# kluonj/HelFEM

Measured on AMD Instinct MI355X. Metric: scf_iteration_wall_time_fock_plus_geneig_nbf4230, lower is better.
Workload: dtype f64; 1 GPU; diatomic Z1=7 Z2=7 R=2.068 PBE, nelem=5 nnodes=15 nquad=75 lmmax=[20,20] (Nbf=4230, Nang=61, Nrad=70), XC grid 92x13, symmetry blocks [1380, 1470, 1380]: J+XC Fock build + eig_gsym_sub + density per step; parallelism=shard1, density=occupied orbitals of the core Hamiltonian

## Files before the change

### helfem_amd/__init__.py

```python
import ctypes
import os

import numpy as np

_HERE = os.path.dirname(os.path.abspath(__file__))
_LIB_PATH = os.environ.get("HELFEM_AMD_LIB") or os.path.join(_HERE, "lib", "libhelfem_amd.so")
_lib = None

c_double_p = ctypes.POINTER(ctypes.c_double)
c_int_p = ctypes.POINTER(ctypes.c_int)
c_i64_p = ctypes.POINTER(ctypes.c_int64)


class hfg_diatomic_desc(ctypes.Structure):
    _fields_ = [("Z1", ctypes.c_int), ("Z2", ctypes.c_int), ("Rhalf", ctypes.c_double), ("primbas", ctypes.c_int),
                ("nnodes", ctypes.c_int), ("nquad", ctypes.c_int), ("bval", c_double_p), ("nbval", ctypes.c_int),
                ("lval", c_int_p), ("mval", c_int_p), ("nang", ctypes.c_int), ("lpad", ctypes.c_int)]


class hfg_model_pot(ctypes.Structure):
    _fields_ = [("kind", ctypes.c_int), ("Z", ctypes.c_int), ("d", ctypes.c_double), ("H", ctypes.c_double)]


class hfg_atomic_desc(ctypes.Structure):
# ... 53 lines not shown
        L.hfg_last_error.restype = ctypes.c_char_p
        L.hfg_version.restype = ctypes.c_char_p
        L.hfg_gaunt_coefficient.restype = ctypes.c_double
        L.hfg_gaunt_coefficient.argtypes = [ctypes.c_int] * 6
        L.hfg_modified_gaunt_coefficient.restype = ctypes.c_double
        L.hfg_modified_gaunt_coefficient.argtypes = [ctypes.c_int] * 6
        L.hfg_theta_lm.restype = ctypes.c_double
        L.hfg_theta_lm.argtypes = [ctypes.c_int, ctypes.c_int, ctypes.c_double]
        L.hfg_legendre_PQ.restype = None
        L.hfg_legendre_PQ.argtypes = [ctypes.c_int, ctypes.c_int, ctypes.c_double, c_double_p, c_double_p]
        for nm in ("hfg_bessel_il", "hfg_bessel_kl"):
            getattr(L, nm).restype = ctypes.c_double
            getattr(L, nm).argtypes = [ctypes.c_double, ctypes.c_int]
        L.hfg_erfc_phi.restype = ctypes.c_double
        L.hfg_erfc_phi.argtypes = [ctypes.c_int, ctypes.c_double, ctypes.c_double]
        L.hfg_compute_rs_tei.argtypes = [ctypes.c_void_p, ctypes.c_int, ctypes.c_double]
        L.hfg_compute_rs_tei_dev.argtypes = [ctypes.c_void_p, ctypes.c_void_p, ctypes.c_int, ctypes.c_double]
        L.hfg_rs_special_dev.argtypes = [ctypes.c_void_p, ctypes.c_int, ctypes.c_int, c_double_p, c_double_p, ctypes.c_int64, c_double_p]
        L.hfg_set_erfc_binomial_mode.restype = None
        L.hfg_set_erfc_binomial_mode.argtypes = [ctypes.c_int]
        L.hfg_model_potential.argtypes = [ctypes.c_void_p, ctypes.c_void_p, ctypes.POINTER(hfg_model_pot),
                                          ctypes.POINTER(hfg_model_pot), c_double_p]
        L.hfg_chebyshev_rule.restype = None
        L.hfg_chebyshev_rule.argtypes = [ctypes.c_int, c_double_p, c_double_p]
        L.hfg_lobatto_nodes.restype = None
        L.hfg_lobatto_nodes.argtypes = [ctypes.c_int, c_double_p]
        L.hfg_radial_grid.argtypes = [ctypes.c_double, ctypes.c_int, ctypes.c_int, ctypes.c_double, c_double_p]
        L.hfg_basis_confinement.argtypes = [ctypes.c_void_p, ctypes.c_int, ctypes.c_int, ctypes.c_double, ctypes.c_double,
                                            ctypes.c_double, c_double_p]
        L.hfg_atomic_grid.argtypes = [ctypes.c_int, ctypes.c_double, ctypes.c_int, ctypes.c_double, ctypes.c_int, ctypes.c_double,
                                      ctypes.c_int, ctypes.c_int, ctypes.c_double, ctypes.c_int, ctypes.c_int, ctypes.c_int,
                                      ctypes.c_double, ctypes.c_int, ctypes.c_double, c_double_p, c_int_p]
        L.hfg_scf_options_check_ex.argtypes = [ctypes.POINTER(hfg_scf_options), ctypes.POINTER(hfg_scf_atomic_extras)]
        L.hfg_scf_run_ex.argtypes = [ctypes.c_void_p, ctypes.POINTER(hfg_scf_options), ctypes.POINTER(hfg_scf_atomic_extras),
                                     ctypes.POINTER(hfg_scf_result), c_double_p, c_double_p]
        L.hfg_ctx_create.argtypes = [ctypes.POINTER(ctypes.c_void_p), ctypes.c_int, ctypes.c_void_p]
        L.hfg_xc_fock.argtypes = [ctypes.c_void_p, ctypes.c_void_p, ctypes.c_int, ctypes.c_int, c_double_p, c_double_p,
                                  c_double_p, c_double_p, c_double_p, ctypes.c_double]
        L.hfg_xc_fock_pol.argtypes = [ctypes.c_void_p, ctypes.c_void_p, ctypes.c_int, ctypes.c_int, c_double_p, c_double_p,
                                      c_double_p, c_double_p, c_double_p, c_double_p, c_double_p, ctypes.c_double]
        L.hfg_xc_fock_dev.argtypes = [ctypes.c_void_p, ctypes.c_void_p, ctypes.c_int, ctypes.c_int, ctypes.c_void_p,
                                      ctypes.c_void_p, ctypes.c_void_p, ctypes.c_double]
        L.hfg_coulomb_batch.argtypes = [ctypes.c_void_p, ctypes.c_void_p, ctypes.c_int64, c_double_p, c_double_p]
        L.hfg_coulomb_energy_matrix.argtypes = [ctypes.c_void_p, ctypes.c_void_p, ctypes.c_int64, c_double_p, c_double_p]
        L.hfg_coulomb_batch_devptr.argtypes = [ctypes.c_void_p, ctypes.c_void_p, ctypes.c_int64, ctypes.c_void_p, ctypes.c_void_p]
        for name in ("hfg_exchange_batch", "hfg_rs_exchange_batch"):
            getattr(L, name).argtypes = [ctypes.c_void_p, ctypes.c_void_p, ctypes.c_int64, c_double_p, c_double_p]
        for name in ("hfg_exchange_batch_devptr", "hfg_rs_exchange_batch_devptr"):
            getattr(L, name).argtypes = [ctypes.c_void_p, ctypes.c_void_p, ctypes.c_int64, ctypes.c_void_p, ctypes.c_void_p]
        L.hfg_exchange_occ_batch_devptr.argtypes = [ctypes.c_void_p, ctypes.c_void_p, ctypes.c_int64, ctypes.c_void_p, ctypes.c_void_p,
                                                    c_i64_p, ctypes.c_int64, ctypes.c_void_p]
        L.hfg_exchange_batch_plan.argtypes = [ctypes.c_int64, c_int_p, ctypes.c_int, c_int_p, c_int_p]
        L.hfg_fock_compact_pol_size.restype = ctypes.c_int64
        L.hfg_fock_compact_pol_size.argtypes = [ctypes.c_void_p]
        L.hfg_fock_compact_pol_devptr.argtypes = [ctypes.c_void_p, ctypes.c_void_p, ctypes.c_int, ctypes.c_int, ctypes.c_void_p,
                                                  ctypes.c_void_p, ctypes.c_void_p, ctypes.c_void_p, ctypes.c_double]
        L.hfg_fock_finish_pol_devptr.argtypes = [ctypes.c_void_p] * 7
        L.hfg_eig_gsym_sub_pair_devptr.argtypes = [ctypes.c_void_p, ctypes.c_int64, ctypes.c_void_p, ctypes.c_void_p, ctypes.c_void_p,
                                                   ctypes.c_int, c_i64_p, c_i64_p] + [ctypes.c_void_p] * 4
        L.hfg_profile_get.argtypes = [ctypes.c_void_p, ctypes.c_char_p, c_double_p, c_i64_p]
        L.hfg_measure_kernel.argtypes = [ctypes.c_void_p, ctypes.c_char_p, c_double_p, c_i64_p]
        L.hfg_profile_names.argtypes = [ctypes.c_void_p, ctypes.c_char_p, ctypes.c_size_t]
        L.hfg_diis_create.argtypes = [ctypes.c_void_p, ctypes.c_int64, ctypes.c_int, ctypes.c_int, ctypes.c_double, ctypes.c_double,
                                      ctypes.c_int, ctypes.POINTER(ctypes.c_void_p)]
        L.hfg_diis_destroy.argtypes = [ctypes.c_void_p]
        L.hfg_diis_set_metric_devptr.argtypes = [ctypes.c_void_p, ctypes.c_void_p, ctypes.c_void_p, ctypes.c_int64]
        L.hfg_diis_set_blocks.argtypes = [ctypes.c_void_p, ctypes.c_int, c_i64_p, c_i64_p]
        L.hfg_diis_update_devptr.argtypes = [ctypes.c_void_p, ctypes.c_double, ctypes.c_void_p, ctypes.c_void_p, ctypes.c_void_p,
                                             ctypes.c_int64, ctypes.c_void_p, ctypes.c_void_p, ctypes.c_void_p, ctypes.c_int64,
                                             c_double_p]
        L.hfg_diis_solve_devptr.argtypes = [ctypes.c_void_p, ctypes.c_void_p, ctypes.c_void_p, c_int_p]
        L.hfg_diis_size.argtypes = [ctypes.c_void_p]
        L.hfg_diis_get.argtypes = [ctypes.c_void_p, ctypes.c_int, c_double_p, ctypes.c_int64]
        L.hfg_coulomb_dev.argtypes = [ctypes.c_void_p] * 4
        L.hfg_fock_compact_size.restype = ctypes.c_int64
        L.hfg_eig_block_buf_size.restype = ctypes.c_int64
        L.hfg_fock_compact_dev.argtypes = [ctypes.c_void_p, ctypes.c_void_p, ctypes.c_int, ctypes.c_int, ctypes.c_void_p,
                                           ctypes.c_void_p, ctypes.c_void_p, ctypes.c_double]
        for name in ("hfg_exchange_dev", "hfg_rs_exchange_dev", "hfg_mix_exchange_devptr"):
            getattr(L, name).argtypes = [ctypes.c_void_p] * 4
        for name in ("hfg_exchange_occ_dev", "hfg_mix_exchange_occ_devptr"):
            getattr(L, name).argtypes = [ctypes.c_void_p] * 4 + [ctypes.c_int64, ctypes.c_void_p]
        L.hfg_mix_exchange_occ_batch_devptr.argtypes = L.hfg_exchange_occ_batch_devptr.argtypes
        _lib = L
    return _lib


def _check(rc):
    if rc != 0:
        raise RuntimeError(lib().hfg_last_error().decode())


def _f(a):
    return np.asfortranarray(a, dtype=np.float64)


def _p(a):
    return a.ctypes.data_as(c_double_p)


def device_count():
    return int(lib().hfg_device_count())


class Context(object):

    def __init__(self, device=0, stream=None):
        h = ctypes.c_void_p()
        if stream is None:
            sp = None
        elif int(stream) == 0:
            sp = ctypes.c_void_p(-1)
        else:
            sp = ctypes.c_void_p(int(stream))
        _check(lib().hfg_ctx_create(ctypes.byref(h), int(device), sp))
        self.h = h
        self.device = device

    def close(self):
        if self.h:
            lib().hfg_ctx_destroy(self.h)
            self.h = None

    def __del__(self):
        try:
            self.close()
        except Exception:
            pass

    def synchronize(self):
        _check(lib().hfg_ctx_synchronize(self.h))

    def set_shard(self, rank, nranks):
        _check(lib().hfg_ctx_set_shard(self.h, int(rank), int(nranks)))

    def set_fock_blocks(self, basis, blockid_ptr):
        f = lib().hfg_ctx_set_fock_blocks
        f.argtypes = [ctypes.c_void_p, ctypes.c_void_p, ctypes.c_void_p]
        _check(f(self.h, basis.h, ctypes.c_void_p(blockid_ptr or 0)))

    def fix_sinvh(self, device_ptr):
        _check(lib().hfg_ctx_fix_sinvh(self.h, ctypes.c_void_p(device_ptr or 0)))

    FOCK_BAND_STATES = ("none", "declared", "refused")

    def declare_fock_band(self, basis, H0_ptr=None, blockid_ptr=None):
        f = lib().hfg_ctx_declare_fock_band
        f.argtypes = [ctypes.c_void_p, ctypes.c_void_p, ctypes.c_void_p, ctypes.c_void_p, c_int_p]
        st = ctypes.c_int()
        _check(f(self.h, basis.h, ctypes.c_void_p(H0_ptr or 0), ctypes.c_void_p(blockid_ptr or 0), ctypes.byref(st)))
        return self.FOCK_BAND_STATES[st.value]

    def fock_band_state(self):
        f = lib().hfg_ctx_fock_band_state
        f.argtypes = [ctypes.c_void_p, c_int_p]
        st = ctypes.c_int()
        _check(f(self.h, ctypes.byref(st)))
        return self.FOCK_BAND_STATES[st.value]

    def profile(self, on=True):
        _check(lib().hfg_profile_enable(self.h, 1 if on else 0))

    def profile_reset(self):
        _check(lib().hfg_profile_reset(self.h))

    def measure_kernel(self, name):
# ... 973 lines not shown
            return [("hfg_mix_exchange_occ_batch_devptr", "K")]
        return [("hfg_mix_exchange_occ_devptr" if have_C else "hfg_mix_exchange_devptr", "K")]
    plain, occ, screened = (("hfg_exchange_batch_devptr", "hfg_exchange_occ_batch_devptr", "hfg_rs_exchange_batch_devptr") if batch
                            else ("hfg_exchange_dev", "hfg_exchange_occ_dev", "hfg_rs_exchange_dev"))
    route = []
    if kfrac != 0.0:
        route.append((occ if have_C else plain, "K"))
    if kshort != 0.0:
        route.append((screened, "Krs"))
    return route


class DeviceSCFStep(object):

    def __init__(self, basis, x_func, c_func, ldft, mdft, nocc, symmetry=1, device=0, rank=0, nranks=1,
                 dens_thr=1e-12, kfrac=0.0, device_tei=False, fock_shard="auto", kshort=0.0, omega=0.0, rs_kind=None):
        self.nocc = int(nocc)
        self._setup(basis, x_func, c_func, ldft, mdft, symmetry, device, rank, nranks, dens_thr, kfrac, device_tei, fock_shard,
                    kshort, omega, rs_kind)
        f64 = dict(dtype=self.torch.float64, device=self.dev)
        L, N = lib(), self.N
        self.Fc = self.torch.zeros(int(L.hfg_fock_compact_size(basis.h)), **f64)
        self.scal = self.torch.zeros(3, **f64)
        self.F = self.torch.zeros(N * N, **f64)
        self.E = self.torch.zeros(N, **f64)
        self.C = self.torch.zeros(N * N, **f64)
        self.P = self.torch.zeros(N * N, **f64)
        nb = int(L.hfg_eig_block_buf_size(len(self.blocks), self.blk_ptr.ctypes.data_as(c_i64_p)))
        self.blockbuf = self.torch.zeros(nb, **f64)
        if self.anyK:
            self.K = self.torch.zeros(N * N, **f64)
            self.Pa = self.torch.zeros(N * N, **f64)

    def _setup(self, basis, x_func, c_func, ldft, mdft, symmetry, device, rank, nranks, dens_thr, kfrac, device_tei, fock_shard,
               kshort=0.0, omega=0.0, rs_kind=None):
        self.kshort, self.omega = float(kshort), float(omega)
        self.rs_kind = 0
        self.mix = False
        self.Krs = None
        if self.kshort != 0.0:
            if not isinstance(basis, AtomicTwoDBasis):
                raise RuntimeError("Range separated functionals are not supported.")
            self.rs_kind = xc_rs_kind(x_func) if rs_kind is None else int(rs_kind)
            if self.rs_kind not in (1, 2) or self.omega == 0.0:
                raise ValueError("kshort != 0 needs a screened kernel (rs_kind 1 Yukawa or 2 erfc, from the exchange functional "
                                 "when None) and its range omega != 0")
        import torch
        self.torch = torch
        self.basis = basis
        self.x_func, self.c_func, self.thr = int(x_func), int(c_func), float(dens_thr)
        self.dev = torch.device("cuda", device)
        torch.cuda.set_device(self.dev)
        self.ctx = Context(device, stream=torch.cuda.current_stream(self.dev).cuda_stream)
        self.ctx.set_shard(rank, nranks)
        self.rank, self.nranks = int(rank), int(nranks)
        self.fock_shard = os.environ.get("HELFEM_FOCK_SHARD", fock_shard)
        if device_tei:
            basis.compute_tei(float(kfrac) != 0.0 or self.kshort != 0.0, device=True, ctx=self.ctx)
        if self.kshort != 0.0:
            switches = {r["name"]: r["value"] for r in tuning_table()}
            on_device = bool(device_tei) or switches["HELFEM_RS_TEI"] == "dev"
            basis._compute_rs(self.rs_kind, self.omega, on_device, self.ctx)
        basis.upload(ldft, mdft, ctx=self.ctx)
        if self.kshort != 0.0:
            want = int(switches["HELFEM_EXL_MIX"])
            if want > 0 or (want < 0 and MIX_BY_DEFAULT[self.rs_kind]):
                self.mix = basis.mix_exchange_tables(float(kfrac), self.kshort, ctx=self.ctx)
        N = basis.Nbf()
        self.N = N
        self.blocks = basis.get_sym_idx(symmetry)
        self.blk_ptr, self.blk_idx = scf._blocks(self.blocks)
        blockid = np.zeros(N, dtype=np.int32)
        for ib, b in enumerate(self.blocks):
            blockid[b] = ib
        self.blockid = torch.from_numpy(blockid).to(self.dev)
        self.ctx.set_fock_blocks(basis, self.blockid.data_ptr())
        self.H0 = None
        self.Sinvh = None
        self.kfrac = float(kfrac)
        self.anyK = self.kfrac != 0.0 or self.kshort != 0.0
        self.kscale = self.kfrac if self.kshort == 0.0 else 1.0
        self.have_C = False
        self.have_density = False
        if self.kshort != 0.0 and not self.mix:
            self.Krs = torch.zeros(N * N, dtype=torch.float64, device=self.dev)

    def _ptr(self, t):
        return ctypes.c_void_p(t.data_ptr())

    def set_matrices(self, H0, Sinvh):
        t = self.torch
        self.H0 = t.from_numpy(np.asfortranarray(H0).ravel(order="F").copy()).to(self.dev)
        self.ctx.fix_sinvh(None)
        self.Sinvh = t.from_numpy(np.asfortranarray(Sinvh).ravel(order="F").copy()).to(self.dev)
        self.ctx.fix_sinvh(self.Sinvh.data_ptr())
        if not self.anyK and not self._applies_cuhf:
            self.ctx.declare_fock_band(self.basis, self.H0.data_ptr(), self.blockid.data_ptr())

    def set_density(self, P, C=None):
        self.P.copy_(self.torch.from_numpy(np.asfortranarray(P).ravel(order="F").copy()))
        self.have_density = True
        self.have_C = C is not None
        if C is not None:
            self.C[:self.N * self.nocc].copy_(self.torch.from_numpy(np.asfortranarray(C[:, :self.nocc]).ravel(order="F").copy()))

    def exchange(self):
        self.torch.mul(self.P, 0.5, out=self.Pa)
        self._build_K(self.Pa, self.C, ctypes.c_int64(self.nocc), self.K)

    def _build_K(self, P, C, nocc, K, batch=0):
        L = lib()
        head = (self.ctx.h, self.basis.h, batch) if batch else (self.ctx.h, self.basis.h)
        for name, dest in _exchange_route(self.mix, self.kfrac, self.kshort, self.have_C, bool(batch)):
            args = [self._ptr(P)]
            if "_occ_" in name:
                args += [self._ptr(C), nocc] if self.have_C else [None, None]
                if batch:
                    args.append(self.N)
            _check(getattr(L, name)(*head, *args, self._ptr(K if dest == "K" else self.Krs)))
        if self.kshort != 0.0 and not self.mix:
            if self.kfrac != 0.0:
                K.mul_(self.kfrac).add_(self.Krs, alpha=self.kshort)
            else:
                self.torch.mul(self.Krs, self.kshort, out=K)

    def fock_partial(self):
        _check(lib().hfg_fock_compact_dev(self.ctx.h, self.basis.h, self.x_func, self.c_func, self._ptr(self.P),
                                          self._ptr(self.Fc), self._ptr(self.scal), self.thr))

    def fock_finish(self):
        _check(lib().hfg_fock_finish_dev(self.ctx.h, self.basis.h, self._ptr(self.Fc), self._ptr(self.H0),
                                         self._ptr(self.blockid), self._ptr(self.F)))

    def _spins(self):
        return ((self.P, self.F, self.E, self.C, self.nocc),)

    def _blockbufs(self):
        return (self.blockbuf,)

    def _spin_K(self):
        return (self.K,)

    def eig_partial(self):
        for (_, F, _, _, _), buf in zip(self._spins(), self._blockbufs()):
            _check(lib().hfg_eig_blocks_dev(self.ctx.h, ctypes.c_int64(self.N), self._ptr(F), self._ptr(self.Sinvh),
                                            len(self.blocks), self.blk_ptr.ctypes.data_as(c_i64_p),
                                            self.blk_idx.ctypes.data_as(c_i64_p), self._ptr(buf)))

    def eig_finish(self):
        for (_, _, E, C, _), buf in zip(self._spins(), self._blockbufs()):
            _check(lib().hfg_eig_assemble_dev(self.ctx.h, ctypes.c_int64(self.N), len(self.blocks),
                                              self.blk_ptr.ctypes.data_as(c_i64_p), self.blk_idx.ctypes.data_as(c_i64_p),
                                              self._ptr(buf), self._ptr(E), self._ptr(C)))

    def eig_whole(self):
        _check(lib().hfg_eig_gsym_sub_dev(self.ctx.h, ctypes.c_int64(self.N), self._ptr(self.F), self._ptr(self.Sinvh),
                                          len(self.blocks), self.blk_ptr.ctypes.data_as(c_i64_p),
                                          self.blk_idx.ctypes.data_as(c_i64_p), self._ptr(self.E), self._ptr(self.C)))

    def density(self):
        for P, _, _, C, nocc in self._spins():
            if nocc == 0:
                P.zero_()
                continue
            _check(lib().hfg_form_density_dev(self.ctx.h, ctypes.c_int64(self.N), ctypes.c_int64(self.N), self._ptr(C),
                                              ctypes.c_int64(nocc), self._ptr(P)))
        self.have_density = True

    def step(self, allreduce=None, exchange_blocks=None):
        self._fock_stage(allreduce)
        self._constrain()
        self._eig_stage(allreduce, exchange_blocks)
        self.density()
        self.have_C = True

    def _whole_shard(self, fn):
        if self.nranks > 1:
            self.ctx.set_shard(0, 1)
        try:
            fn()
        finally:
            if self.nranks > 1:
                self.ctx.set_shard(self.rank, self.nranks)

    def _fock_stage(self, allreduce):
        shard_fock = self.nranks > 1 and self.fock_shard == "always"
        if shard_fock or self.nranks == 1:
            self.fock_partial()
            if allreduce is not None:
                allreduce(self.Fc)
                allreduce(self.scal)
        else:
            self._whole_shard(self.fock_partial)
        self.fock_finish()
        if self.anyK:
            self.exchange()
            if allreduce is not None:
                allreduce(self.K)
            self._add_exchange()

    def _add_exchange(self):
        for (_, F, _, _, _), K in zip(self._spins(), self._spin_K()):
            F.add_(K, alpha=self.kscale)

    def _eig_in_one_call(self, allreduce, exchange_blocks):
        return self.nranks == 1 and allreduce is None and exchange_blocks is None

    def _eig_stage(self, allreduce, exchange_blocks):
        if self._eig_in_one_call(allreduce, exchange_blocks):
            self.eig_whole()
            return
        self.eig_partial()
        for buf in self._blockbufs():
            if exchange_blocks is not None:
                exchange_blocks(buf, len(self.blocks))
            elif allreduce is not None:
                allreduce(buf)
        self.eig_finish()

    def _nn_buffer(self, name):
        buf = getattr(self, name, None)
        if buf is None:
            buf = self.torch.zeros(self.N * self.N, dtype=self.torch.float64, device=self.dev)
            setattr(self, name, buf)
        return buf

    def _coulomb_energy_matrix(self, P):
        J = self._nn_buffer("J")
        self._whole_shard(lambda: _check(lib().hfg_coulomb_dev(self.ctx.h, self.basis.h, self._ptr(P), self._ptr(J))))
        return J

    def _energy_terms(self):
        t = self.torch
        J = self._coulomb_energy_matrix(self.P)
        terms = [t.dot(self.P, self.H0), t.dot(self.P, J)]
        terms.append(t.dot(self.Pa, self.K) if self.anyK else t.zeros((), dtype=t.float64, device=self.dev))
        return terms

    def energy(self, Enucr=0.0):
        t = self.torch
        v = t.stack(self._energy_terms() + [self.scal[0]]).cpu().numpy()
        r = dict(E1=float(v[0]), Ecoul=0.5 * float(v[1]), Exx=self._exx_factor() * float(v[2]), Exc=float(v[3]), Enucr=float(Enucr))
        r["Etot"] = r["E1"] + r["Ecoul"] + r["Exx"] + r["Exc"] + r["Enucr"]
        return r

    def _exx_factor(self):
        return self.kscale

    def _nspin(self):
        return 1

    def _density_stage(self):
        self.density()
        self.P.mul_(2.0)
        self.have_C = True

    def _core_guess(self, allreduce, exchange_blocks):
        for _, F, _, _, _ in self._spins():
            F.copy_(self.H0)
        self._eig_stage(allreduce, exchange_blocks)
        self._density_stage()

    def _diis_update(self, diis, E):
        Pa = self.torch.mul(self.P, 0.5, out=self._nn_buffer("Pa"))
        if self.have_C:
            return diis.update(E, self.F, Pa, self.C, self.nocc)
        return diis.update(E, self.F, Pa)

    def _diis_solve(self, diis):
        diis.solve(self.F)

    _applies_cuhf = False

    def _constraint_begin(self, S):
        pass

    def _constrain(self):
        pass

    def run(self, S, maxit=50, convthr=1e-7, Enucr=0.0, allreduce=None, exchange_blocks=None, diis=None, callback=None,
            rohf=False, cuhf=False, readocc=None, maverage=False, dampfock=1.0):
        _refuse_out_of_scope(type(self).__name__, rohf and not self._applies_cuhf, cuhf and not self._applies_cuhf, readocc, maverage,
                             dampfock)
        if self.H0 is None:
            raise RuntimeError("run: set_matrices first")
        self._constraint_begin(S)
        t = self.torch
        if diis is None:
            diis = DeviceDIIS(self.ctx, self.N, self._nspin())
            dS = t.from_numpy(np.asfortranarray(S, dtype=np.float64).ravel(order="F").copy()).to(self.dev)
            diis.set_metric(dS, self.Sinvh)
            if len(self.blocks) > 1:
                diis.set_blocks(self.blocks)
        if not self.have_density:
            self._core_guess(allreduce, exchange_blocks)
        trace, Eold, res, converged, it = [], 0.0, None, False, 0
        for it in range(1, int(maxit) + 1):
            self._fock_stage(allreduce)
            res = self.energy(Enucr)
            self._constrain()
            maxerr = self._diis_update(diis, res["Etot"])
            dE = res["Etot"] - Eold
            Eold = res["Etot"]
            trace.append((res["Etot"], maxerr))
            if callback is not None:
                callback(it, res["Etot"], maxerr)
            if maxerr < convthr and abs(dE) < convthr:
                converged = True
                break
            self._diis_solve(diis)
            self._eig_stage(allreduce, exchange_blocks)
            self._density_stage()
        res = dict(res or {})
        res.update(iterations=it, converged=converged, trace=trace)
        return res

    def numpy(self, t, shape):
        return t.cpu().numpy().reshape(shape, order="F")


class DeviceUSCFStep(DeviceSCFStep):

    def __init__(self, basis, x_func, c_func, ldft, mdft, nocc, symmetry=1, device=0, rank=0, nranks=1,
                 dens_thr=1e-12, kfrac=0.0, device_tei=False, fock_shard="auto", kshort=0.0, omega=0.0, rs_kind=None):
        self.nela, self.nelb = int(nocc[0]), int(nocc[1])
        if self.nela < 1 or self.nelb < 0:
            raise ValueError("DeviceUSCFStep: nocc = (nela >= 1, nelb >= 0)")
        self._setup(basis, x_func, c_func, ldft, mdft, symmetry, device, rank, nranks, dens_thr, kfrac, device_tei, fock_shard,
                    kshort, omega, rs_kind)
        t, N, L = self.torch, self.N, lib()
        f64 = dict(dtype=t.float64, device=self.dev)
        self.nc = int(L.hfg_fock_compact_size(basis.h))
        self.Fc = t.zeros(int(L.hfg_fock_compact_pol_size(basis.h)), **f64)
        self.scal = t.zeros(3, **f64)
        for name in ("Pa", "Pb", "Fa", "Fb", "Ca", "Cb"):
            setattr(self, name, t.zeros(N * N, **f64))
        self.Ea, self.Eb = t.zeros(N, **f64), t.zeros(N, **f64)
        if self.nranks > 1:
            nb = int(L.hfg_eig_block_buf_size(len(self.blocks), self.blk_ptr.ctypes.data_as(c_i64_p)))
            self.blockbuf_a, self.blockbuf_b = t.zeros(nb, **f64), t.zeros(nb, **f64)
        self.kbatch = False
        if self.anyK:
            self.K = t.zeros(2 * N * N, **f64)
            self.Ka, self.Kb = self.K[:N * N], self.K[N * N:]
            self.kbatch = {r["name"]: r["value"] for r in tuning_table()}["HELFEM_USCF_KBATCH"] == "on"
            if self.kbatch:
                self.Pab, self.Cab = t.zeros(2 * N * N, **f64), t.zeros(2 * N * N, **f64)
                self._nocc = np.array([self.nela, self.nelb], dtype=np.int64)
                if self.Krs is not None:
                    self.Krs = t.zeros(2 * N * N, **f64)

    def _spins(self):
        return ((self.Pa, self.Fa, self.Ea, self.Ca, self.nela), (self.Pb, self.Fb, self.Eb, self.Cb, self.nelb))

    def _blockbufs(self):
        return (self.blockbuf_a, self.blockbuf_b)

    def _spin_K(self):
        return (self.Ka, self.Kb)

    def set_density(self, Pa, Pb, Ca=None, Cb=None):
        as_dev = lambda M: self.torch.from_numpy(np.asfortranarray(M).ravel(order="F").copy())
        self.Pa.copy_(as_dev(Pa))
        self.Pb.copy_(as_dev(Pb))
        self.have_density = True
        self.have_C = Ca is not None and (Cb is not None or self.nelb == 0)
        if self.have_C:
            self.Ca[:self.N * self.nela].copy_(as_dev(Ca[:, :self.nela]))
            if self.nelb:
                self.Cb[:self.N * self.nelb].copy_(as_dev(Cb[:, :self.nelb]))

    def exchange(self):
        if self.kbatch:
            N2 = self.N * self.N
            self.Pab[:N2].copy_(self.Pa)
            self.Pab[N2:].copy_(self.Pb)
            if self.have_C:
                self.Cab[:N2].copy_(self.Ca)
                self.Cab[N2:].copy_(self.Cb)
            self._build_K(self.Pab, self.Cab, self._nocc.ctypes.data_as(c_i64_p), self.K, batch=2)
            return
        for (P, _, _, C, nocc), K in zip(self._spins(), self._spin_K()):
            if nocc == 0:
                K.zero_()
            else:
                self._build_K(P, C, ctypes.c_int64(nocc), K)

    def fock_partial(self):
        _check(lib().hfg_fock_compact_pol_devptr(self.ctx.h, self.basis.h, self.x_func, self.c_func, self._ptr(self.Pa),
                                                 self._ptr(self.Pb), self._ptr(self.Fc), self._ptr(self.scal), self.thr))

    def fock_finish(self):
        _check(lib().hfg_fock_finish_pol_devptr(self.ctx.h, self.basis.h, self._ptr(self.Fc), self._ptr(self.H0),
                                                self._ptr(self.blockid), self._ptr(self.Fa), self._ptr(self.Fb)))

    def eig_pair(self):
        _check(lib().hfg_eig_gsym_sub_pair_devptr(self.ctx.h, ctypes.c_int64(self.N), self._ptr(self.Fa), self._ptr(self.Fb),
                                                  self._ptr(self.Sinvh), len(self.blocks), self.blk_ptr.ctypes.data_as(c_i64_p),
                                                  self.blk_idx.ctypes.data_as(c_i64_p), self._ptr(self.Ea), self._ptr(self.Ca),
                                                  self._ptr(self.Eb), self._ptr(self.Cb)))

    eig_whole = eig_pair

    def _eig_in_one_call(self, allreduce, exchange_blocks):
        return self.nranks == 1

    def _energy_terms(self):
        t = self.torch
        Pt = t.add(self.Pa, self.Pb, out=self._nn_buffer("Pt"))
        J = self._coulomb_energy_matrix(Pt)
        terms = [t.dot(Pt, self.H0), t.dot(Pt, J)]
        terms.append(t.dot(self.Pa, self.Ka) + t.dot(self.Pb, self.Kb) if self.anyK
                     else t.zeros((), dtype=t.float64, device=self.dev))
        return terms

    def _exx_factor(self):
        return 0.5 * self.kscale

    def _nspin(self):
        return 2

    def _density_stage(self):
        self.density()
        self.have_C = True

    def _diis_update(self, diis, E):
        if self.have_C:
            return diis.update(E, self.Fa, self.Pa, self.Ca, self.nela, self.Fb, self.Pb, self.Cb if self.nelb else None, self.nelb)
        return diis.update(E, self.Fa, self.Pa, Fb=self.Fb, Pb=self.Pb)

    def _diis_solve(self, diis):
        diis.solve(self.Fa, self.Fb)


class DeviceROHFStep(DeviceUSCFStep):

    _applies_cuhf = True

    def __init__(self, *args, **kw):
        super(DeviceROHFStep, self).__init__(*args, **kw)
        self.S = None

    def set_overlap(self, S):
        S = np.asfortranarray(S, dtype=np.float64)
        if S.shape != (self.N, self.N):
            raise ValueError("DeviceROHFStep.set_overlap: S is N x N")
        self.S = self.torch.from_numpy(S.ravel(order="F").copy()).to(self.dev)

    def _constraint_begin(self, S):
        if S is not None:
            self.set_overlap(S)

    def _constrain(self):
        if self.S is None:
            raise RuntimeError("DeviceROHFStep: set_overlap first")
        if not self.have_C:
            raise RuntimeError("DeviceROHFStep: the constraint needs the orbitals the densities were formed from "
                               "(set_density with Ca and Cb, or start from the core guess)")
        self.ctx.cuhf_update(self.S, self.Ca, self.nela, self.Cb, self.nelb, self.Fa, self.Fb)
```

### helfem_amd/csrc/hip/capi.cpp

```cpp
#include "internal.h"
#include "../host/checkpoint.h"
#include "../host/diis.h"
#include "../host/dftfuncs.h"
#include "../host/exchange_batch_plan.h"
#include "../host/eig_band_plan.h"
#include "../host/fock_need.h"
#include <cstring>
#include <memory>
#include <mutex>

namespace hfg {
static thread_local std::string g_err;
void set_error(const std::string &msg) { g_err = msg; }

}

using namespace hfg;

#define HFG_TRY try {
#define HFG_CATCH                       \
  }                                     \
  catch (const std::logic_error &e) {   \
    hfg::set_error(e.what());           \
    return 1;                           \
// ... 807 lines not shown
int hfg_exchange_batch_plan(int64_t nP, const int *ranks, int max_members, int *chunk_of, int *nchunks) {
  HFG_TRY
  if (nP < 0) throw std::logic_error("hfg_exchange_batch_plan: negative number of densities\n");
  if (nP > 0 && (!ranks || !chunk_of)) throw std::logic_error("hfg_exchange_batch_plan: null pointer\n");
  if (max_members < 0) throw std::logic_error("hfg_exchange_batch_plan: negative chunk size\n");
  const int n = helfem::exchange_batch_plan((long)nP, ranks, max_members ? max_members : helfem::tuning_live().exchange_batch_chunk, chunk_of);
  if (nchunks) *nchunks = n;
  HFG_CATCH
}
int hfg_xc_fock_dev(hfg_ctx *ctx, hfg_basis *b, int x_func, int c_func, const double *dP, double *dH, double *dScal,
                    double thr) {
  HFG_TRY xc_fock_dev(ctx, b, x_func, c_func, dP, dH, dScal, thr);
  HFG_CATCH
}
int hfg_xc_fock_pol_dev(hfg_ctx *ctx, hfg_basis *b, int x_func, int c_func, const double *dPa, const double *dPb,
                        double *dHa, double *dHb, double *dScal, double thr) {
  HFG_TRY xc_fock_pol_dev(ctx, b, x_func, c_func, dPa, dPb, dHa, dHb, dScal, thr);
  HFG_CATCH
}
int hfg_eig_gsym_sub_dev(hfg_ctx *ctx, int64_t N, const double *dF, const double *dS, int nblk, const int64_t *blk_ptr,
                         const int64_t *blk_idx, double *dE, double *dC) {
  HFG_TRY eig_gsym_sub_dev(ctx, (int)N, dF, dS, nblk, blk_ptr, blk_idx, dE, dC);
  HFG_CATCH
}
int64_t hfg_eig_block_buf_size(int nblk, const int64_t *blk_ptr) { return (int64_t)eig_block_buf_size(nblk, blk_ptr); }
int hfg_eig_blocks_dev(hfg_ctx *ctx, int64_t N, const double *dF, const double *dS, int nblk, const int64_t *blk_ptr,
                       const int64_t *blk_idx, double *dBlockBuf) {
  HFG_TRY eig_blocks_dev(ctx, (int)N, dF, dS, nblk, blk_ptr, blk_idx, dBlockBuf);
  HFG_CATCH
}
int hfg_eig_assemble_dev(hfg_ctx *ctx, int64_t N, int nblk, const int64_t *blk_ptr, const int64_t *blk_idx,
                         const double *dBlockBuf, double *dE, double *dC) {
  HFG_TRY eig_assemble_dev(ctx, (int)N, nblk, blk_ptr, blk_idx, dBlockBuf, dE, dC);
  HFG_CATCH
}
int hfg_form_density_dev(hfg_ctx *ctx, int64_t N, int64_t ncols, const double *dC, int64_t nocc, double *dP) {
  HFG_TRY form_density_dev(ctx, (int)N, (int)ncols, dC, (int)nocc, dP);
  HFG_CATCH
}
int hfg_gemm_dev(hfg_ctx *ctx, int tA, int tB, int64_t m, int64_t n, int64_t k, const double *dA, int64_t lda,
                 const double *dB, int64_t ldb, double *dC, int64_t ldc) {
  HFG_TRY gemm_dev(ctx, tA != 0, tB != 0, (int)m, (int)n, (int)k, 1.0, dA, (int)lda, dB, (int)ldb, 0.0, dC, (int)ldc);
  HFG_CATCH
}

int64_t hfg_fock_compact_size(hfg_basis *b) { return (int64_t)fock_compact_size(b); }
int hfg_fock_compact_dev(hfg_ctx *ctx, hfg_basis *b, int x_func, int c_func, const double *dP, double *dFc,
                         double *dScal, double thr) {
  HFG_TRY fock_compact_dev(ctx, b, x_func, c_func, dP, dFc, dScal, thr);
  HFG_CATCH
}
int hfg_fock_finish_dev(hfg_ctx *ctx, hfg_basis *b, const double *dFc, const double *dH0, const int *dBlockId,
                        double *dF) {
  HFG_TRY fock_finish_dev(ctx, b, dFc, dH0, dBlockId, dF);
  HFG_CATCH
}
int64_t hfg_fock_compact_pol_size(hfg_basis *b) { return 2 * (int64_t)fock_compact_size(b); }
int hfg_fock_compact_pol_devptr(hfg_ctx *ctx, hfg_basis *b, int x_func, int c_func, const double *dPa, const double *dPb,
                                double *dFc, double *dScal, double thr) {
  HFG_TRY
  if (!ctx || !b) throw std::logic_error("hfg_fock_compact_pol_devptr: null context or basis\n");
  if (!dPa || !dPb || !dFc || !dScal) throw std::logic_error("hfg_fock_compact_pol_devptr: null device pointer\n");
  fock_compact_pol_dev(ctx, b, x_func, c_func, dPa, dPb, dFc, dScal, thr);
  HFG_CATCH
}
int hfg_fock_finish_pol_devptr(hfg_ctx *ctx, hfg_basis *b, const double *dFc, const double *dH0, const int *dBlockId,
                               double *dFa, double *dFb) {
  HFG_TRY
  if (!ctx || !b) throw std::logic_error("hfg_fock_finish_pol_devptr: null context or basis\n");
  if (!dFc || !dFa || !dFb) throw std::logic_error("hfg_fock_finish_pol_devptr: null device pointer\n");
  fock_finish_pol_dev(ctx, b, dFc, dH0, dBlockId, dFa, dFb);
  HFG_CATCH
}
int hfg_eig_gsym_sub_pair_devptr(hfg_ctx *ctx, int64_t N, const double *dFa, const double *dFb, const double *dSinvh, int nblk,
                                 const int64_t *blk_ptr, const int64_t *blk_idx, double *dEa, double *dCa, double *dEb,
                                 double *dCb) {
  HFG_TRY
  if (!ctx) throw std::logic_error("hfg_eig_gsym_sub_pair_devptr: null context\n");
  if (!dFa || !dFb || !dSinvh || !blk_ptr || !blk_idx || !dEa || !dCa || !dEb || !dCb)
    throw std::logic_error("hfg_eig_gsym_sub_pair_devptr: null pointer\n");
  eig_gsym_sub_pair_dev(ctx, (int)N, dFa, dFb, dSinvh, nblk, blk_ptr, blk_idx, dEa, dCa, dEb, dCb);
  HFG_CATCH
}
int hfg_ctx_set_fock_blocks(hfg_ctx *ctx, hfg_basis *b, const int *blockid_dev) {
  HFG_TRY
  if (!ctx || !b) throw std::logic_error("hfg_ctx_set_fock_blocks: null context or basis");
  set_fock_blocks(ctx, b, blockid_dev);
  HFG_CATCH
}
int hfg_fock_need_pairs(int nshell, const int *nfunc, const int *blockid, int *need) {
  HFG_TRY
  if (nshell < 0 || !nfunc || !blockid || !need) throw std::logic_error("hfg_fock_need_pairs: invalid arguments");
  helfem::fock_need_pairs(nshell, nfunc, blockid, need);
  HFG_CATCH
}

namespace {
struct FullShard {
  hfg_ctx *c;
  int r, n;
  explicit FullShard(hfg_ctx *ctx) : c(ctx), r(ctx->shard_rank), n(ctx->shard_n) {
    c->shard_rank = 0;
    c->shard_n = 1;
  }
  ~FullShard() {
    c->shard_rank = r;
    c->shard_n = n;
  }
};
}
int hfg_coulomb(hfg_ctx *ctx, hfg_basis *b, const double *P, double *J) {
  HFG_TRY
  FullShard full(ctx);
  size_t N = b->Nbf();
  Stage st(ctx);
  double *dP = st.up(P, N * N), *dJ = st.alloc(N * N);
  coulomb_dev(ctx, b, dP, dJ);
  st.down(J, dJ, N * N);
  st.sync();
  HFG_CATCH
}
int hfg_coulomb_batch(hfg_ctx *ctx, hfg_basis *b, int64_t nP, const double *P, double *J) {
  HFG_TRY
  if (!coulomb_batch_args("hfg_coulomb_batch", ctx, b, nP, P, J)) return 0;
  FullShard full(ctx);
  size_t n = b->Nbf() * b->Nbf() * (size_t)nP;
  Stage st(ctx);
  double *dP = st.up(P, n), *dJ = st.alloc(n);
  coulomb_batch_dev(ctx, b, nP, dP, dJ);
  st.down(J, dJ, n);
  st.sync();
  HFG_CATCH
}
int hfg_coulomb_energy_matrix(hfg_ctx *ctx, hfg_basis *b, int64_t nP, const double *P, double *W) {
  HFG_TRY
  if (!coulomb_batch_args("hfg_coulomb_energy_matrix", ctx, b, nP, P, W)) return 0;
  FullShard full(ctx);
  Stage st(ctx);
  double *dP = st.up(P, b->Nbf() * b->Nbf() * (size_t)nP), *dW = st.alloc((size_t)nP * nP);
  coulomb_energy_matrix_dev(ctx, b, nP, dP, dW);
  st.down(W, dW, (size_t)nP * nP);
  st.sync();
  HFG_CATCH
}
int hfg_exchange(hfg_ctx *ctx, hfg_basis *b, const double *P, double *K) {
  HFG_TRY
  FullShard full(ctx);
  size_t N = b->Nbf();
  Stage st(ctx);
  double *dP = st.up(P, N * N), *dK = st.alloc(N * N);
  exchange_dev(ctx, b, dP, dK);
  st.down(K, dK, N * N);
  st.sync();
  HFG_CATCH
}
int hfg_rs_exchange(hfg_ctx *ctx, hfg_basis *b, const double *P, double *K) {
  HFG_TRY
  FullShard full(ctx);
  size_t N = b->Nbf();
  Stage st(ctx);
  double *dP = st.up(P, N * N), *dK = st.alloc(N * N);
  exchange_dev(ctx, b, dP, dK, ExTables::screened);
  st.down(K, dK, N * N);
  st.sync();
  HFG_CATCH
}
// ... 366 lines not shown
```

### helfem_amd/csrc/hip/common.h

```cpp
#pragma once
#include <hip/hip_runtime.h>
#include <cstdint>
#include <cstring>
#include <map>
#include <stdexcept>
#include <string>
#include <vector>

#include "../../../include/helfem_gpu.h"
#include "../host/atomic_basis.h"
#include "../host/diatomic_basis.h"
#include "../host/tuning.h"
#include "workspace_owner.h"

namespace hfg {
using helfem::TrdMode, helfem::tuning;

void set_error(const std::string &msg);

#define HFG_HIP_CHECK(expr)                                                                          \
  do {                                                                                               \
    hipError_t _e = (expr);                                                                          \
    if (_e != hipSuccess)                                                                            \
      throw std::runtime_error(std::string("HIP error: ") + hipGetErrorString(_e) + " in " + #expr + \
                               " (" + __FILE__ + ":" + std::to_string(__LINE__) + ")");              \
  } while (0)

template <typename T>
struct DevBuf {
  T *p = nullptr;
  size_t n = 0;
  DevBuf() {}
  DevBuf(const DevBuf &) = delete;
  DevBuf &operator=(const DevBuf &) = delete;
  ~DevBuf() { release(); }
  void release() {
    if (p) (void)hipFree(p);
    p = nullptr;
    n = 0;
  }
  void resize(size_t count) {
    if (count <= n) return;
    release();
    HFG_HIP_CHECK(hipMalloc((void **)&p, count * sizeof(T)));
    n = count;
  }
  void upload(const std::vector<T> &h, hipStream_t s) {
    resize(h.size() ? h.size() : 1);
    if (h.size()) HFG_HIP_CHECK(hipMemcpyAsync(p, h.data(), h.size() * sizeof(T), hipMemcpyHostToDevice, s));
  }
};

template <typename T>
bool upload_cached(DevBuf<T> &buf, std::vector<T> &cache, const std::vector<T> &h, hipStream_t s) {
  if (buf.p && cache.size() == h.size() && buf.n >= h.size() &&
      (h.empty() || memcmp((const void *)cache.data(), (const void *)h.data(), h.size() * sizeof(T)) == 0))
    return false;
  HFG_HIP_CHECK(hipStreamSynchronize(s));
  cache = h;
  buf.upload(cache, s);
  return true;
}

struct ProfEntry {
  double ms = 0.0;
  int64_t launches = 0;
  std::vector<std::pair<hipEvent_t, hipEvent_t> > pending;
};

}

struct hfg_dev_tables;

struct hfg_ctx {
  int device = 0;
  hipStream_t stream = nullptr;
  bool own_stream = false;
  hipStream_t side_stream = nullptr;
  hipEvent_t side_ev[2] = {nullptr, nullptr};
  hipStream_t side();
  bool avoid_side = false;
  void drop_side();
  int shard_rank = 0, shard_n = 1;
  const double *fixed_sinvh = nullptr;
  unsigned long fixed_gen = 0;
  void fix_sinvh(const double *p) {
    fixed_sinvh = p;
    fixed_gen++;
    band_node.clear();
    band_state = 0;
  }
  std::vector<int> band_node;
  int band_pm = 0, band_E = 0;
  int band_state = 0;
  hfg::DevBuf<int> fock_need, fock_gneed;
  const hfg_dev_tables *fock_need_tables = nullptr;
  int fock_need_A = 0, fock_need_G = 0;
  bool profiling = false;
  std::map<std::string, hfg::ProfEntry> prof;
  std::vector<hipEvent_t> event_pool;
  hfg::DevBuf<double> ws[8];
  double *pinned = nullptr;
  size_t pinned_bytes = 0;
  hfg::WorkspaceOwner<hfg::WS_CTX_SLOTS> work;

  void *pinned_buf(size_t bytes);
  hipEvent_t get_event();
  void prof_begin(const char *name);
  void prof_end(const char *name);
  void prof_collect();
};

struct hfg_basis {
  int kind = 0;
  helfem::diatomic::TwoDBasis b;
  helfem::atomic::TwoDBasis ab;
  hfg_dev_tables *dev = nullptr;
  hfg_dev_tables *dev_rs = nullptr;
  hfg_dev_tables *dev_mix = nullptr;
  double mix_alpha = 0.0, mix_beta = 0.0, mix_omega = 0.0;
  int mix_kind = 0;
  int dev_device = -1;
  hfg::DevBuf<double> dev_tei;
  bool tei_on_device = false;
  hfg::DevBuf<double> dev_rs_tei, dev_rs_disj;
  bool rs_on_device = false;

  size_t Nbf() const { return kind ? ab.Nbf() : b.Nbf(); }
  size_t Ndummy() const { return kind ? ab.Nbf() : b.Ndummy(); }
  size_t Nrad() const { return kind ? ab.Nrad() : b.Nrad(); }
  size_t Nang() const { return kind ? ab.Nang() : b.Nang(); }
  size_t Nel() const { return kind ? ab.Nel() : b.Nel(); }
  size_t max_Nprim() const { return kind ? ab.max_Nprim() : b.max_Nprim(); }
  bool have_tei() const { return tei_on_device || (kind ? ab.have_tei : b.have_tei); }
};

namespace hfg {
struct GemmTask {
  const double *A;
  const double *B;
  double *C;
  int M, N, K, lda, ldb, ldc;
  int tA = 0, tB = 0;
  double alpha = 1.0, beta = 0.0;
  int sym = 0;
  int over = 0;
  const int *amap = nullptr, *cmap = nullptr;
  const int64_t *rmap = nullptr;
  const int *kstart = nullptr;
  int nk = 0;
  int kpad = 0;
};
static_assert(sizeof(GemmTask) == 120, "GemmTask is compared bytewise: keep it free of padding");

struct ProfScope {
  hfg_ctx *c;
  const char *n;
  ProfScope(hfg_ctx *ctx, const char *name) : c(ctx), n(name) {
    if (c->profiling) c->prof_begin(n);
  }
  ~ProfScope() {
    if (c->profiling) c->prof_end(n);
  }
};
}
```

### helfem_amd/csrc/hip/eig.hip

```cpp
#include "internal.h"
#include "wave.h"
#include "../host/eigsel_count.h"
#include "../host/eig_band_plan.h"
#include <cstdlib>
#include <cstring>
#include <functional>

namespace hfg {

constexpr int MAXB = 8;
struct EigBatch {
  int nblk;
  int n[MAXB];
  double *A[MAXB];
  double *d[MAXB];
  double *e[MAXB];
  double *tau[MAXB];
  double *v[MAXB];
  double *pp[MAXB];
  double *dots[MAXB];
  double *Z[MAXB];
  int nz[MAXB];
  double *rot[MAXB];
  int *sweeps[MAXB];
// ... 512 lines not shown
  __shared__ double sT[BT_KB][BT_KB + 1];
  __shared__ double sG[BT_KB][BT_KB + 1];
  __shared__ double sg[BT_KB];
  const int blk = blockIdx.y, p = blockIdx.x;
  const int n = b.n[blk];
  const int j0 = p * BT_KB;
  if (j0 > n - 3) return;
  const int kb = min(BT_KB, n - 2 - j0);
  double *Tp = T[blk] + (size_t)p * BT_KB * BT_KB;
  const int t = threadIdx.x;
  for (int c0 = 0; c0 < BT_KB; c0 += 16) {
    double g[16];
#pragma unroll
    for (int u = 0; u < 16; u++) g[u] = 0.0;
#pragma unroll
    for (int sl = 0; sl < BT_GS; sl++) {
      const double *src = G[blk] + ((size_t)sl * P + p) * BT_KB * BT_KB + (size_t)c0 * BT_KB + t;
#pragma unroll
      for (int u = 0; u < 16; u++) g[u] += src[(size_t)u * BT_KB];
    }
#pragma unroll
    for (int u = 0; u < 16; u++) {
      sG[c0 + u][t] = g[u];
      sT[t][c0 + u] = 0.0;
    }
  }
  __shared__ double stau[BT_KB];
  stau[t] = (t < kb) ? b.tau[blk][j0 + t] : 0.0;
  __syncthreads();
  for (int i = 0; i < kb; i++) {
    const double ti = stau[i];
    sg[t] = (t < i) ? sG[i][t] : 0.0;
    __syncthreads();
    if (t < i) {
      double acc0 = 0.0, acc1 = 0.0, acc2 = 0.0, acc3 = 0.0;
#pragma unroll
      for (int k = 0; k < BT_KB; k += 4) {
        acc0 += sT[t][k] * sg[k];
        acc1 += sT[t][k + 1] * sg[k + 1];
        acc2 += sT[t][k + 2] * sg[k + 2];
        acc3 += sT[t][k + 3] * sg[k + 3];
      }
      sT[t][i] = -ti * ((acc0 + acc1) + (acc2 + acc3));
    }
    if (t == i) sT[i][i] = ti;
    __syncthreads();
  }
  for (int c = 0; c < BT_KB; c++) Tp[(size_t)c * BT_KB + t] = sT[t][c];
}

struct EigWork : Workspace {
  GemmHow full_how;
  std::vector<int64_t> asm_rows;
  DevBuf<long long> asm_rows_dev;
  bool folded = false;
  DevBuf<double> Y[MAXB];
  DevBuf<GemmTask> btslabR, btupdR;
  std::vector<GemmTask> h_btslabR, h_btupdR;
  DevBuf<double> A[MAXB], d[MAXB], e[MAXB], tau[MAXB], v[MAXB], pp[MAXB], dots[MAXB], Z[MAXB], rot[MAXB];
  DevBuf<double> Zs[MAXB], Ws[MAXB];
  DevBuf<int> selrank;
  DevBuf<int> sweeps[MAXB];
  DevBuf<int> ibuf1, ibuf2;
  DevBuf<GemmTask> gtasks, bttasks, btslab, btgram, btcpl, btupd;
  std::vector<GemmTask> h_gtasks, h_bttasks, h_btslab, h_btgram, h_btcpl, h_btupd;
  std::vector<double *> h_btptr;
  DevBuf<double> Vx[MAXB], G[MAXB], T[MAXB], VT[MAXB], Wb[MAXB], Wp[MAXB], Cc[MAXB];
  DevBuf<double *> btptr;
  bool used_dc = true;
  DevBuf<double> idx;
  const double *sup_S = nullptr;
  unsigned long sup_gen = 0;
  int sup_N = 0;
  std::vector<int64_t> sup_ptr, sup_idx;
  DevBuf<double> Xc;
  std::vector<char> xc_have;
  std::vector<int64_t> band_rows, band_pos;
  std::vector<int> band_ks, band_koff, band_toff;
  bool band_any = false;
  DevBuf<long long> band_rows_dev, band_pos_dev;
  DevBuf<int> band_ks_dev, band_iota_dev;
  DevBuf<GemmTask> fxtasks;
  std::vector<GemmTask> h_fxtasks;
  int *h_status = nullptr;
  hipEvent_t status_ev = nullptr;
  ~EigWork() {
    if (h_status) (void)hipHostFree(h_status);
    if (status_ev) (void)hipEventDestroy(status_ev);
  }
};
static EigWork &work_for(hfg_ctx *ctx) { return ctx->work.get<EigWork>(WS_EIG); }

struct CopySlices {
  const double *src[16];
  double *dst[16];
  int n[16];
};
__global__ void k_copy_slices(CopySlices c) {
  const int q = blockIdx.y;
  for (int i = blockIdx.x * blockDim.x + threadIdx.x; i < c.n[q]; i += gridDim.x * blockDim.x) c.dst[q][i] = c.src[q][i];
}
static void copy_slices(hipStream_t s, const std::vector<const double *> &src, const std::vector<double *> &dst, const std::vector<int> &n) {
  for (size_t q0 = 0; q0 < src.size(); q0 += 16) {
    CopySlices c{};
    const int m = (int)std::min<size_t>(16, src.size() - q0);
    int nmax = 0;
    for (int q = 0; q < m; q++) {
      c.src[q] = src[q0 + q];
      c.dst[q] = dst[q0 + q];
      c.n[q] = n[q0 + q];
      nmax = std::max(nmax, n[q0 + q]);
    }
    if (nmax > 0) hipLaunchKernelGGL(k_copy_slices, dim3((nmax + 255) / 256, m), dim3(256), 0, s, c);
  }
}

struct TrPtrs {
  const double *src[MAXB];
  double *dst[MAXB];
  int n[MAXB];
};
__global__ __launch_bounds__(256) void k_transpose_batch(TrPtrs t) {
  __shared__ double tile[64][65];
  const int blk = blockIdx.z, n = t.n[blk];
  const int bi = blockIdx.x * 64, bj = blockIdx.y * 64;
  if (bi >= n || bj >= n) return;
  const int tx = threadIdx.x & 63, ty = threadIdx.x >> 6;
  for (int c = ty; c < 64; c += 4) {
    const int gm = bi + tx, gn = bj + c;
    tile[c][tx] = (gm < n && gn < n) ? t.src[blk][(size_t)gn * n + gm] : 0.0;
  }
  __syncthreads();
  for (int c = ty; c < 64; c += 4) {
    const int gm = bj + tx, gn = bi + c;
    if (gm < n && gn < n) t.dst[blk][(size_t)gn * n + gm] = tile[tx][c];
  }
}

static void bt_wy_setup(hfg_ctx *ctx, EigWork &w, const EigBatch &b, int nblk, const int *ns, int nmax, bool fold = false) {
  hipStream_t s = ctx->stream;
  const int P = (nmax - 3) / BT_KB + 1;
  const int NP = (P + 1) / 2;
  constexpr int BT_S = 6;
  std::vector<double *> ptrs(6 * (size_t)nblk);
  for (int k = 0; k < nblk; k++) {
    const int n = ns[k];
    w.Vx[k].resize((size_t)n * n);
    w.G[k].resize((size_t)BT_GS * P * BT_KB * BT_KB);
    w.T[k].resize((size_t)P * BT_KB * BT_KB);
    w.VT[k].resize((size_t)n * P * BT_KB);
    w.Wb[k].resize((size_t)BT_PW * n);
    w.Wp[k].resize((size_t)BT_S * BT_PW * n);
    w.Cc[k].resize((size_t)BT_GS * NP * BT_KB * BT_KB);
    ptrs[k] = w.Vx[k].p;
    ptrs[nblk + k] = w.G[k].p;
    ptrs[2 * nblk + k] = w.T[k].p;
    ptrs[3 * nblk + k] = w.Wp[k].p;
    ptrs[4 * nblk + k] = w.Wb[k].p;
    ptrs[5 * nblk + k] = w.Cc[k].p;
  }
  upload_cached(w.btptr, w.h_btptr, ptrs, s);
  GemmTask none;
  none.A = none.B = nullptr;
  none.C = nullptr;
  none.M = none.N = none.K = 0;
  none.lda = none.ldb = none.ldc = 1;
// ... 359 lines not shown
      if (shb > 64 * 1024)
        HFG_HIP_CHECK(
            hipFuncSetAttribute((const void *)k_backtransform_lds, hipFuncAttributeMaxDynamicSharedMemorySize, (int)shb));
      hipLaunchKernelGGL(k_backtransform_lds, grid, dim3(256), shb, s, bz);
    }
    }
  }
  HFG_HIP_CHECK(hipGetLastError());
}

static void check_status(hfg_ctx *ctx, EigWork &w, int nblk) {
  if (w.used_dc) {
    if (dc_status(ctx) != 0) throw std::logic_error("Eigendecomposition failed!\n");
    trdp_check_status(ctx);
    return;
  }
  for (int i = 0; i < nblk; i++) {
    int st[2];
    HFG_HIP_CHECK(hipMemcpyAsync(st, w.sweeps[i].p, 2 * sizeof(int), hipMemcpyDeviceToHost, ctx->stream));
    HFG_HIP_CHECK(hipStreamSynchronize(ctx->stream));
    if (st[1] != 0) throw std::logic_error("Eigendecomposition failed!\n");
  }
}

void eig_sym_dev(hfg_ctx *ctx, int n, const double *dA, double *dE, double *dC) {
  EigWork &w = work_for(ctx);
  w.A[0].resize((size_t)n * n + 2);
  HFG_HIP_CHECK(hipMemcpyAsync(w.A[0].p, dA, sizeof(double) * n * n, hipMemcpyDeviceToDevice, ctx->stream));
  eig_sym_batch(ctx, w, 1, &n);
  DevBuf<int> &rank = w.ibuf1;
  rank.resize(n + 8);
  launch_rank(ctx, w.d[0].p, n, rank.p);
  hipLaunchKernelGGL(k_scatter_cols, dim3((n + 255) / 256, n), dim3(256), 0, ctx->stream, w.Z[0].p, n, n,
                     (const int64_t *)nullptr, rank.p, 0, w.d[0].p, n, dC, dE);
  check_status(ctx, w, 1);
}

void eig_sym_sel_dev(hfg_ctx *ctx, int n, const double *dA, int nev, double *dE, double *dC) {
  if (nev < 1) throw std::logic_error("eig_sym_sel: nev must be at least 1\n");
  if (n < 1) throw std::logic_error("eig_sym_sel: empty matrix\n");
  nev = std::min(nev, n);
  EigWork &w = work_for(ctx);
  w.A[0].resize((size_t)n * n + 2);
  HFG_HIP_CHECK(hipMemcpyAsync(w.A[0].p, dA, sizeof(double) * n * n, hipMemcpyDeviceToDevice, ctx->stream));
  eig_sym_batch(ctx, w, 1, &n, nullptr, &nev);
  HFG_HIP_CHECK(hipMemcpyAsync(dC, w.Zs[0].p, sizeof(double) * (size_t)n * nev, hipMemcpyDeviceToDevice, ctx->stream));
  HFG_HIP_CHECK(hipMemcpyAsync(dE, w.Ws[0].p, sizeof(double) * nev, hipMemcpyDeviceToDevice, ctx->stream));
  check_status(ctx, w, 1);
}

void eig_gsym_dev(hfg_ctx *ctx, int N, int n, const double *dF, const double *dS, double *dE, double *dC) {
  EigWork &w = work_for(ctx);
  w.A[0].resize((size_t)n * n + 2);
  DevBuf<double> &T1 = ctx->ws[0];
  DevBuf<double> &Ctmp = ctx->ws[1];
  T1.resize((size_t)N * n);
  Ctmp.resize((size_t)N * n);
  {
    ProfScope ps(ctx, "eig_reduce");
    gemm_dev(ctx, false, false, N, n, N, 1.0, dF, N, dS, N, 0.0, T1.p, N);
    gemm_dev(ctx, true, false, n, n, N, 1.0, dS, N, T1.p, N, 0.0, w.A[0].p, n);
  }
  eig_sym_batch(ctx, w, 1, &n);
  {
    ProfScope ps(ctx, "eig_backtransform");
    gemm_dev(ctx, false, false, N, n, n, 1.0, dS, N, w.Z[0].p, n, 0.0, Ctmp.p, N);
  }
  DevBuf<int> &rank = w.ibuf1;
  rank.resize(n + 8);
  launch_rank(ctx, w.d[0].p, n, rank.p);
  hipLaunchKernelGGL(k_scatter_cols, dim3((N + 255) / 256, n), dim3(256), 0, ctx->stream, Ctmp.p, N, n,
                     (const int64_t *)nullptr, rank.p, 0, w.d[0].p, N, dC, dE);
  check_status(ctx, w, 1);
}

size_t eig_block_buf_size(int nblk, const int64_t *blk_ptr) {
  size_t nmax = 0;
  for (int ib = 0; ib < nblk; ib++) nmax = std::max<size_t>(nmax, blk_ptr[ib + 1] - blk_ptr[ib]);
  return (size_t)nblk * (nmax * nmax + nmax);
}

static void eig_blocks_multi_dev(hfg_ctx *ctx, int N, int nF, const double *const *dFs, const double *dS, int nblk, const int64_t *blk_ptr,
                                 const int64_t *blk_idx, double *const *dBlockBufs, int nev = 0, double *const *dEs = nullptr,
                                 double *const *dCs = nullptr);
static int eig_num_cus(hfg_ctx *ctx) {
  static const int ncu = [&] {
    hipDeviceProp_t prop;
    return (hipGetDeviceProperties(&prop, ctx->device) == hipSuccess && prop.multiProcessorCount > 0) ? prop.multiProcessorCount : 256;
  }();
  return ncu;
}
void eig_blocks_dev(hfg_ctx *ctx, int N, const double *dF, const double *dS, int nblk, const int64_t *blk_ptr,
                    const int64_t *blk_idx, double *dBlockBuf) {
  eig_blocks_multi_dev(ctx, N, 1, &dF, dS, nblk, blk_ptr, blk_idx, &dBlockBuf);
}
static void eig_blocks_multi_dev(hfg_ctx *ctx, int N, int nF, const double *const *dFs, const double *dS, int nblk, const int64_t *blk_ptr,
                                 const int64_t *blk_idx, double *const *dBlockBufs, int nev, double *const *dEs, double *const *dCs) {
  EigWork &w = work_for(ctx);
  hipStream_t s = ctx->stream;
  const bool direct = dEs != nullptr;
  if (direct && (ctx->shard_n != 1 || nF * nblk > MAXB)) throw std::logic_error("eig_blocks_multi_dev: direct path needs one rank and one batch\n");
  if (blk_ptr[nblk] != N) throw std::logic_error("Symmetry mismatch in eig_gsym_sub\n");
  DevBuf<double> &idxbuf = w.idx;
  idxbuf.resize(2 * (size_t)N + 16);
  int64_t *drows = (int64_t *)idxbuf.p;
  int64_t *dcols = drows + N;
  for (int ib = 0; ib < nblk; ib++)
    if (blk_ptr[ib + 1] == blk_ptr[ib]) throw std::logic_error("eig_gsym_sub: empty symmetry block\n");
  const bool want_band = ctx->fixed_sinvh && ctx->fixed_sinvh == dS && ctx->band_state == 1 && ctx->band_node.size() == (size_t)N &&
                         helfem::tuning_live().eig_band;
  const bool cached = ctx->fixed_sinvh && ctx->fixed_sinvh == dS && w.sup_S == dS && w.sup_gen == ctx->fixed_gen &&
                      w.sup_N == N && want_band == !w.band_rows.empty() &&
                      w.sup_ptr.size() == (size_t)nblk + 1 && std::equal(w.sup_ptr.begin(), w.sup_ptr.end(), blk_ptr) &&
                      w.sup_idx.size() == (size_t)N && std::equal(w.sup_idx.begin(), w.sup_idx.end(), blk_idx);
  if (!cached) {
    w.sup_S = nullptr;
    w.xc_have.clear();
    HFG_HIP_CHECK(hipStreamSynchronize(s));
    w.band_rows.clear();
    w.band_pos.clear();
    w.band_ks.clear();
    w.band_koff.assign(1, 0);
    w.band_toff.assign(1, 0);
    w.band_any = false;
    if (want_band) {
      w.band_rows.resize(N);
      w.band_pos.resize(N);
      std::vector<int> nd, ks, toff;
      int64_t nbig = 0;
      for (int ib = 0; ib < nblk; ib++) {
        const int64_t o = blk_ptr[ib], n = blk_ptr[ib + 1] - o;
        nbig = std::max(nbig, n);
        nd.resize(n);
        for (int64_t i = 0; i < n; i++) {
          if (blk_idx[o + i] < 0 || blk_idx[o + i] >= N) throw std::logic_error("eig_gsym_sub: block index out of range\n");
          nd[i] = ctx->band_node[blk_idx[o + i]];
        }
        helfem::eig_band_order(n, nd.data(), w.band_pos.data() + o);
        for (int64_t i = 0; i < n; i++) w.band_rows[o + i] = blk_idx[o + w.band_pos[o + i]];
        if (helfem::eig_band_plan(n, nd.data(), w.band_pos.data() + o, ctx->band_pm, ctx->band_E, ks, toff)) w.band_any = true;
        for (size_t t = 0; t + 1 < toff.size(); t++) w.band_koff.push_back((int)w.band_ks.size() + toff[t + 1]);
        w.band_ks.insert(w.band_ks.end(), ks.begin(), ks.end());
        w.band_toff.push_back((int)w.band_koff.size() - 1);
      }
      std::vector<int> iota(nbig);
      for (int64_t i = 0; i < nbig; i++) iota[i] = (int)i;
      w.band_rows_dev.resize(N);
      w.band_pos_dev.resize(N);
      w.band_ks_dev.resize(w.band_ks.size() + 1);
      w.band_iota_dev.resize(nbig);
      HFG_HIP_CHECK(hipMemcpyAsync(w.band_rows_dev.p, w.band_rows.data(), sizeof(int64_t) * N, hipMemcpyHostToDevice, s));
      HFG_HIP_CHECK(hipMemcpyAsync(w.band_pos_dev.p, w.band_pos.data(), sizeof(int64_t) * N, hipMemcpyHostToDevice, s));
      HFG_HIP_CHECK(hipMemcpyAsync(w.band_ks_dev.p, w.band_ks.data(), sizeof(int) * w.band_ks.size(), hipMemcpyHostToDevice, s));
      HFG_HIP_CHECK(hipMemcpyAsync(w.band_iota_dev.p, iota.data(), sizeof(int) * nbig, hipMemcpyHostToDevice, s));
      HFG_HIP_CHECK(hipStreamSynchronize(s));
    }
    HFG_HIP_CHECK(hipMemcpyAsync(drows, blk_idx, sizeof(int64_t) * N, hipMemcpyHostToDevice, s));
    DevBuf<int> &flag = w.ibuf2;
    flag.resize((size_t)N * nblk + 8);
    for (int ib = 0; ib < nblk; ib++) {
      int n = (int)(blk_ptr[ib + 1] - blk_ptr[ib]);
      hipLaunchKernelGGL(k_col_support, dim3(N), dim3(256), 0, s, dS, N, drows + blk_ptr[ib], n, flag.p + (size_t)ib * N);
    }
    std::vector<int> hflag((size_t)N * nblk);
    HFG_HIP_CHECK(hipMemcpyAsync(hflag.data(), flag.p, sizeof(int) * hflag.size(), hipMemcpyDeviceToHost, s));
    HFG_HIP_CHECK(hipStreamSynchronize(s));
    std::vector<int64_t> allcols;
    for (int ib = 0; ib < nblk; ib++) {
      int cnt = 0;
      for (int c = 0; c < N; c++)
        if (hflag[(size_t)ib * N + c]) {
          allcols.push_back(c);
          cnt++;
        }
      if (cnt != (int)(blk_ptr[ib + 1] - blk_ptr[ib]))
        throw std::logic_error("eig_gsym_sub: Sinvh is not block structured (columns with support != block size)\n");
    }
    HFG_HIP_CHECK(hipMemcpyAsync(dcols, allcols.data(), sizeof(int64_t) * N, hipMemcpyHostToDevice, s));
    HFG_HIP_CHECK(hipStreamSynchronize(s));
    if (ctx->fixed_sinvh == dS) {
      w.sup_S = dS;
      w.sup_gen = ctx->fixed_gen;
      w.sup_N = N;
      w.sup_ptr.assign(blk_ptr, blk_ptr + nblk + 1);
      w.sup_idx.assign(blk_idx, blk_idx + N);
    }
  }

  size_t nmax = 0;
  for (int ib = 0; ib < nblk; ib++) nmax = std::max<size_t>(nmax, blk_ptr[ib + 1] - blk_ptr[ib]);
  const size_t slot = nmax * nmax + nmax;
  if (!direct && ctx->shard_n > 1)
    for (int f = 0; f < nF; f++) HFG_HIP_CHECK(hipMemsetAsync(dBlockBufs[f], 0, sizeof(double) * slot * nblk, s));
  const bool keep_x = w.sup_S == dS && w.sup_S != nullptr;
  std::vector<size_t> xoff(nblk + 1, 0);
  for (int ib = 0; ib < nblk; ib++) xoff[ib + 1] = xoff[ib] + (size_t)(blk_ptr[ib + 1] - blk_ptr[ib]) * (size_t)(blk_ptr[ib + 1] - blk_ptr[ib]);
  if (keep_x) {
    if (w.xc_have.size() != (size_t)nblk || w.Xc.n < xoff[nblk]) {
      w.Xc.resize(xoff[nblk]);
      w.xc_have.assign(nblk, 0);
    }
  }
  std::vector<int64_t> koff(nblk + 1, 0);
  for (int ib = 0; ib < nblk; ib++) {
    const int64_t n = blk_ptr[ib + 1] - blk_ptr[ib];
    koff[ib + 1] = koff[ib] + (nev > 0 ? std::min<int64_t>(nev, n) : n);
  }
  const int K = (int)koff[nblk];
  DevBuf<int> &rank = w.ibuf1;
  DevBuf<double> &Etmp = ctx->ws[3];
  if (direct) {
    rank.resize((size_t)nF * (N + 8));
    Etmp.resize((size_t)nF * N);
  }

  std::vector<int> mine;
  for (int f = 0; f < nF; f++)
    for (int ib = 0; ib < nblk; ib++)
      if (ib % ctx->shard_n == ctx->shard_rank) mine.push_back(f * nblk + ib);
  DevBuf<double> &Fb = ctx->ws[5];
  DevBuf<double> &T1 = ctx->ws[0];
  DevBuf<double> &Xall = ctx->ws[4];
  Fb.resize(nmax * nmax * MAXB);
  T1.resize(nmax * nmax * MAXB);
  Xall.resize(nmax * nmax * MAXB);
  for (size_t c0 = 0; c0 < mine.size(); c0 += MAXB) {
    int nb = (int)std::min<size_t>(MAXB, mine.size() - c0);
    std::vector<int> ns(nb), nevs(nb);
    std::vector<GemmTask> gt(4 * (size_t)nb);
    const double *Xptr[MAXB];
    int nm = 0;
    for (int k = 0; k < nb; k++) {
      const int ib = mine[c0 + k] % nblk;
      double *dBlockBuf = direct ? nullptr : dBlockBufs[mine[c0 + k] / nblk];
      int n = (int)(blk_ptr[ib + 1] - blk_ptr[ib]);
      ns[k] = n;
      nevs[k] = nev > 0 ? std::min(nev, n) : n;
      nm = std::max(nm, n);
      w.A[k].resize((size_t)n * n + 2);
      if (nev > 0) w.Zs[k].resize((size_t)n * nevs[k]);
      else w.Z[k].resize((size_t)n * n);
      w.Y[k].resize((size_t)n * n);
      double *Xb = keep_x ? w.Xc.p + xoff[ib] : Xall.p + (size_t)k * nmax * nmax;
      double *Fk = Fb.p + (size_t)k * nmax * nmax, *Tk = T1.p + (size_t)k * nmax * nmax;
      Xptr[k] = Xb;
      GemmTask g;
      g.M = g.N = g.K = n;
      g.lda = g.ldb = g.ldc = n;
      g.A = Fk;
      g.B = Xb;
      g.C = Tk;
      gt[k] = g;
      g.A = Xb;
      g.tA = 1;
      g.B = Tk;
      g.C = w.A[k].p;
      g.sym = 1;
      gt[nb + k] = g;
      g.sym = 0;
      g.tA = 0;
      g.A = Xb;
      g.B = nev > 0 ? w.Zs[k].p : w.Z[k].p;
      g.N = nevs[k];
      if (direct) {
        const int f = mine[c0 + k] / nblk;
        g.C = dCs[f];
        g.ldc = N;
        g.rmap = drows + blk_ptr[ib];
        g.cmap = rank.p + (size_t)f * (N + 8) + koff[ib];
      } else
        g.C = dBlockBuf + (size_t)ib * slot;
      gt[2 * nb + k] = g;
      g.A = w.Y[k].p;
      g.tA = 1;
      gt[3 * nb + k] = g;
    }
    upload_cached(w.gtasks, w.h_gtasks, gt, s);
    std::vector<GemmTask> fx;
    if (w.band_any && !w.band_rows.empty()) {
      for (int k = 0; k < nb; k++) {
        const int ib = mine[c0 + k] % nblk;
        const int n = ns[k], nt = w.band_toff[ib + 1] - w.band_toff[ib];
        for (int t = 0; t < nt; t++) {
          const int i0 = t * helfem::EIG_BAND_TILE, q = w.band_toff[ib] + t;
          GemmTask g = gt[k];
          g.A = gt[k].A + i0;
          g.M = std::min(helfem::EIG_BAND_TILE, n - i0);
          g.rmap = (const int64_t *)w.band_pos_dev.p + blk_ptr[ib] + i0;
          g.cmap = w.band_iota_dev.p;
          g.kstart = w.band_ks_dev.p + w.band_koff[q];
          g.nk = w.band_koff[q + 1] - w.band_koff[q];
          fx.push_back(g);
        }
      }
      std::stable_sort(fx.begin(), fx.end(), [](const GemmTask &a, const GemmTask &b) { return a.nk > b.nk; });
      upload_cached(w.fxtasks, w.h_fxtasks, fx, s);
    }
    {
      ProfScope ps(ctx, "eig_reduce");
      const int force_split = tuning().gemm_splitk;
      long full_tiles = 0, low_tiles = 0;
      for (int k = 0; k < nb; k++) {
        const long t1 = (ns[k] + 127) / 128;
        full_tiles += t1 * t1;
        low_tiles += t1 * (t1 + 1) / 2;
      }
      const bool band_fx = !fx.empty() && force_split < 0 && !gemm_prefers_128(ctx, full_tiles) && !tuning().mfma_4x4x4;
      for (int k = 0; k < nb; k++) {
        const int ib = mine[c0 + k] % nblk;
        const double *dF = dFs[mine[c0 + k] / nblk];
        int n = ns[k];
        double *Fk = Fb.p + (size_t)k * nmax * nmax;
        if (!(keep_x && w.xc_have[ib]))
          hipLaunchKernelGGL(k_gather_block, dim3((n + 255) / 256, n), dim3(256), 0, s, dF, dS, N, drows + blk_ptr[ib],
                             dcols + blk_ptr[ib], n, Fk, const_cast<double *>(Xptr[k]));
        else if (!band_fx)
          hipLaunchKernelGGL(k_gather_f, dim3((n + 255) / 256, n), dim3(256), 0, s, dF, N, drows + blk_ptr[ib], n, Fk);
        if (band_fx)
          hipLaunchKernelGGL(k_gather_f2, dim3((n + 255) / 256, n), dim3(256), 0, s, dF, N, (const int64_t *)w.band_rows_dev.p + blk_ptr[ib],
                             drows + blk_ptr[ib], n, Fk);
        if (keep_x) w.xc_have[ib] = 1;
      }
      const int slots = 2 * eig_num_cus(ctx);
      const bool split_full = force_split >= 0 ? force_split != 0 : (full_tiles < slots && nm >= 256);
      const bool split_low = force_split >= 0 ? force_split != 0 : (low_tiles < slots && nm >= 256);
      ProfScope pp3(ctx, "eig_products");
      const bool tile64 = force_split < 0 && !gemm_prefers_128(ctx, full_tiles);
      GemmHow full, low;
      if (tile64) full.tile = low.tile = GemmTile::T64;
      else {
        if (split_full) full.tile = GemmTile::T128, full.split2 = true;
        else if (tuning().gemm_rect) full.tile = GemmTile::T128x64;
        if (split_low) low.tile = GemmTile::T128, low.split2 = true;
      }
      w.full_how = full;
      if (full.split2)
        for (int k = 0; k < nb; k++) HFG_HIP_CHECK(hipMemsetAsync(T1.p + (size_t)k * nmax * nmax, 0, sizeof(double) * (size_t)ns[k] * ns[k], s));
      if (band_fx) {
        GemmHow how;
        how.tile = GemmTile::T64;
        how.scatter = how.klist = true;
        gemm_tasklist_dev(ctx, w.fxtasks.p, (int)fx.size(), helfem::EIG_BAND_TILE, nm, how);
      } else
        gemm_tasklist_dev(ctx, w.gtasks.p, nb, nm, nm, full);
      if (low.split2)
        for (int k = 0; k < nb; k++) HFG_HIP_CHECK(hipMemsetAsync(w.A[k].p, 0, sizeof(double) * (size_t)ns[k] * ns[k], s));
      gemm_tasklist_dev(ctx, w.gtasks.p + nb, nb, nm, nm, low);
      gemm_mirror_lower_dev(ctx, w.gtasks.p + nb, nb, nm);
    }
    std::function<void()> after_solve;
    if (direct)
      after_solve = [&] {
        if (w.used_dc) {
          if (!w.h_status) HFG_HIP_CHECK(hipHostMalloc((void **)&w.h_status, sizeof(int), hipHostMallocDefault));
          if (!w.status_ev) HFG_HIP_CHECK(hipEventCreateWithFlags(&w.status_ev, hipEventDisableTiming));
          HFG_HIP_CHECK(hipMemcpyAsync(w.h_status, dc_status_word(ctx), sizeof(int), hipMemcpyDeviceToHost, s));
          HFG_HIP_CHECK(hipEventRecord(w.status_ev, s));
        }
        ProfScope ps(ctx, "scatter");
        std::vector<const double *> csrc;
        std::vector<double *> cdst;
        std::vector<int> cn;
        for (int k = 0; k < nb; k++) {
          const int ib = mine[c0 + k] % nblk, f = mine[c0 + k] / nblk;
          csrc.push_back(nev > 0 ? w.Ws[k].p : w.d[k].p);
          cdst.push_back(Etmp.p + (size_t)f * N + koff[ib]);
          cn.push_back(nevs[k]);
        }
        copy_slices(s, csrc, cdst, cn);
        for (int f = 0; f < nF; f++) {
          int *rk = rank.p + (size_t)f * (N + 8);
          launch_rank(ctx, Etmp.p + (size_t)f * N, K, rk);
          hipLaunchKernelGGL(k_place_values, dim3((K + 255) / 256), dim3(256), 0, s, Etmp.p + (size_t)f * N, K, rk, dEs[f]);
          HFG_HIP_CHECK(hipMemsetAsync(dCs[f], 0, sizeof(double) * (size_t)N * K, s));
        }
      };
    eig_sym_batch(ctx, w, nb, ns.data(), Xptr, nev > 0 ? nevs.data() : nullptr, after_solve);
    {
      ProfScope ps(ctx, "eig_backtransform");
      if (!direct) {
        std::vector<const double *> csrc;
        std::vector<double *> cdst;
        std::vector<int> cn;
        for (int k = 0; k < nb; k++) {
          const int ib = mine[c0 + k] % nblk;
          double *slotp = dBlockBufs[mine[c0 + k] / nblk] + (size_t)ib * slot;
          csrc.push_back(nev > 0 ? w.Ws[k].p : w.d[k].p);
          cdst.push_back(slotp + nmax * nmax);
          cn.push_back(nevs[k]);
          if (nev <= 0 && w.full_how.split2 && ctx->shard_n == 1)
            HFG_HIP_CHECK(hipMemsetAsync(slotp, 0, sizeof(double) * (size_t)ns[k] * ns[k], s));
        }
        copy_slices(s, csrc, cdst, cn);
      }
      {
        ProfScope pp3(ctx, "eig_products");
        const GemmTask *last = w.gtasks.p + (w.folded ? 3 : 2) * (size_t)nb;
        GemmHow how = nev > 0 ? GemmHow{GemmTile::T64} : w.full_how;
        how.scatter = direct;
        gemm_tasklist_dev(ctx, last, nb, nm, nev > 0 ? *std::max_element(nevs.begin(), nevs.end()) : nm, how);
      }
    }
    if (direct && w.used_dc) {
      HFG_HIP_CHECK(hipEventSynchronize(w.status_ev));
      if (*w.h_status != 0) throw std::logic_error("Eigendecomposition failed!\n");
      trdp_check_status(ctx);
    } else
    check_status(ctx, w, nb);
  }
  HFG_HIP_CHECK(hipGetLastError());
}

static void eig_assemble_sel_dev(hfg_ctx *ctx, int N, int nblk, const int64_t *blk_ptr, const int64_t *blk_idx, const double *dBlockBuf,
                                 double *dE, double *dC, int nev);
void eig_assemble_dev(hfg_ctx *ctx, int N, int nblk, const int64_t *blk_ptr, const int64_t *blk_idx,
                      const double *dBlockBuf, double *dE, double *dC) {
  eig_assemble_sel_dev(ctx, N, nblk, blk_ptr, blk_idx, dBlockBuf, dE, dC, 0);
}
int64_t eig_sel_count(int nblk, const int64_t *blk_ptr, int64_t nev) { return helfem::eig_sel_count(nblk, blk_ptr, nev); }
static void eig_assemble_sel_dev(hfg_ctx *ctx, int N, int nblk, const int64_t *blk_ptr, const int64_t *blk_idx, const double *dBlockBuf,
                                 double *dE, double *dC, int nev) {
  EigWork &w = work_for(ctx);
  hipStream_t s = ctx->stream;
  ProfScope ps(ctx, "scatter");
  if (w.asm_rows.size() != (size_t)N || !std::equal(w.asm_rows.begin(), w.asm_rows.end(), blk_idx)) {
    w.asm_rows.assign(blk_idx, blk_idx + N);
    w.asm_rows_dev.resize((size_t)N + 2);
    HFG_HIP_CHECK(hipMemcpyAsync(w.asm_rows_dev.p, w.asm_rows.data(), sizeof(int64_t) * N, hipMemcpyHostToDevice, s));
  }
  int64_t *drows = (int64_t *)w.asm_rows_dev.p;
  size_t nmax = 0;
  for (int ib = 0; ib < nblk; ib++) nmax = std::max<size_t>(nmax, blk_ptr[ib + 1] - blk_ptr[ib]);
  const size_t slot = nmax * nmax + nmax;
  DevBuf<double> &Etmp = ctx->ws[3];
  Etmp.resize(N);
  std::vector<int64_t> koff(nblk + 1, 0);
  for (int ib = 0; ib < nblk; ib++) {
    const int64_t n = blk_ptr[ib + 1] - blk_ptr[ib];
    koff[ib + 1] = koff[ib] + (nev > 0 ? std::min<int64_t>(nev, n) : n);
  }
  const int K = (int)koff[nblk];
  {
    std::vector<const double *> csrc;
    std::vector<double *> cdst;
    std::vector<int> cn;
    for (int ib = 0; ib < nblk; ib++) {
      csrc.push_back(dBlockBuf + (size_t)ib * slot + nmax * nmax);
      cdst.push_back(Etmp.p + koff[ib]);
      cn.push_back((int)(koff[ib + 1] - koff[ib]));
    }
    copy_slices(s, csrc, cdst, cn);
  }
  DevBuf<int> &rank = w.ibuf1;
  rank.resize(N + 8);
  HFG_HIP_CHECK(hipMemsetAsync(dC, 0, sizeof(double) * (size_t)N * K, s));
  launch_rank(ctx, Etmp.p, K, rank.p);
  for (int ib = 0; ib < nblk; ib++) {
    int n = (int)(blk_ptr[ib + 1] - blk_ptr[ib]), nc = (int)(koff[ib + 1] - koff[ib]);
    hipLaunchKernelGGL(k_scatter_cols, dim3((n + 255) / 256, nc), dim3(256), 0, s, dBlockBuf + (size_t)ib * slot, n, nc,
                       drows + blk_ptr[ib], rank.p, (int)koff[ib], Etmp.p + koff[ib], N, dC, dE);
  }
  HFG_HIP_CHECK(hipGetLastError());
}

static void eig_gsym_sub_multi_dev(hfg_ctx *ctx, int N, int nF, const double *const *dFs, const double *dS, int nblk, const int64_t *blk_ptr,
                                   const int64_t *blk_idx, int nev, double *const *dEs, double *const *dCs) {
  int save_rank = ctx->shard_rank, save_n = ctx->shard_n;
  ctx->shard_rank = 0;
  ctx->shard_n = 1;
  try {
    if (helfem::tuning_live().eig_direct && nF * nblk <= MAXB) {
      eig_blocks_multi_dev(ctx, N, nF, dFs, dS, nblk, blk_ptr, blk_idx, nullptr, nev, dEs, dCs);
    } else {
      const size_t sz = eig_block_buf_size(nblk, blk_ptr);
      DevBuf<double> &buf = ctx->ws[6];
      buf.resize(nF * sz);
      double *bufs[MAXB];
      if (nF > MAXB) throw std::logic_error("eig_gsym_sub: too many matrices in one call\n");
      for (int f = 0; f < nF; f++) bufs[f] = buf.p + f * sz;
      eig_blocks_multi_dev(ctx, N, nF, dFs, dS, nblk, blk_ptr, blk_idx, bufs, nev);
      for (int f = 0; f < nF; f++) eig_assemble_sel_dev(ctx, N, nblk, blk_ptr, blk_idx, bufs[f], dEs[f], dCs[f], nev);
    }
  } catch (...) {
    ctx->shard_rank = save_rank;
    ctx->shard_n = save_n;
    throw;
  }
  ctx->shard_rank = save_rank;
  ctx->shard_n = save_n;
}

void eig_gsym_sub_dev(hfg_ctx *ctx, int N, const double *dF, const double *dS, int nblk, const int64_t *blk_ptr,
                      const int64_t *blk_idx, double *dE, double *dC) {
  eig_gsym_sub_multi_dev(ctx, N, 1, &dF, dS, nblk, blk_ptr, blk_idx, 0, &dE, &dC);
}

void eig_gsym_sub_sel_dev(hfg_ctx *ctx, int N, const double *dF, const double *dS, int nblk, const int64_t *blk_ptr,
                          const int64_t *blk_idx, int nev, double *dE, double *dC) {
  if (nev < 1) throw std::logic_error("eig_gsym_sub_sel: nev must be at least 1\n");
  eig_gsym_sub_multi_dev(ctx, N, 1, &dF, dS, nblk, blk_ptr, blk_idx, nev, &dE, &dC);
}

void eig_block_supports(hfg_ctx *ctx, int N, const double *dS, int nblk, const int64_t *blk_ptr, const int64_t *blk_idx,
                        std::vector<int64_t> &cols) {
  hipStream_t s = ctx->stream;
  DevBuf<int64_t> drows;
  DevBuf<int> flag;
  drows.resize(N);
  flag.resize((size_t)N * nblk + 8);
  HFG_HIP_CHECK(hipMemcpyAsync(drows.p, blk_idx, sizeof(int64_t) * N, hipMemcpyHostToDevice, s));
  for (int ib = 0; ib < nblk; ib++) {
    const int n = (int)(blk_ptr[ib + 1] - blk_ptr[ib]);
    hipLaunchKernelGGL(k_col_support, dim3(N), dim3(256), 0, s, dS, N, drows.p + blk_ptr[ib], n, flag.p + (size_t)ib * N);
  }
  std::vector<int> hflag((size_t)N * nblk);
  HFG_HIP_CHECK(hipMemcpyAsync(hflag.data(), flag.p, sizeof(int) * hflag.size(), hipMemcpyDeviceToHost, s));
  HFG_HIP_CHECK(hipStreamSynchronize(s));
  cols.clear();
  for (int ib = 0; ib < nblk; ib++) {
    int cnt = 0;
    for (int c = 0; c < N; c++)
      if (hflag[(size_t)ib * N + c]) {
        cols.push_back(c);
        cnt++;
      }
    if (cnt != (int)(blk_ptr[ib + 1] - blk_ptr[ib]))
      throw std::logic_error("eig_gsym_sub: Sinvh is not block structured (columns with support != block size)\n");
  }
}

__global__ void k_band_outside(const double *__restrict__ H, int N, const int *__restrict__ node, const int *__restrict__ blockid,
                               int pm, int E, int *__restrict__ flag) {
  const int row = blockIdx.x * blockDim.x + threadIdx.x, col = blockIdx.y;
  int bad = 0;
  if (row < N && (!blockid || blockid[row] == blockid[col]) && !helfem::eig_band_share(node[row], node[col], pm, E))
    bad = H[(size_t)col * N + row] != 0.0;
  bad = __syncthreads_or(bad);
  if (bad && threadIdx.x == 0) atomicOr(flag, 1);
}

int eig_declare_band(hfg_ctx *ctx, int N, const int *node, int pm, int E, const double *dH0, const int *dBlockId) {
  if (!ctx->fixed_sinvh) throw std::logic_error("hfg_ctx_declare_fock_band: no Sinvh is declared fixed (hfg_ctx_fix_sinvh)\n");
  if (N < 1 || pm < 1 || E < 1 || !node) throw std::logic_error("hfg_ctx_declare_fock_band: invalid pattern\n");
  for (int i = 0; i < N; i++)
    if (node[i] < 0 || node[i] > pm * E) throw std::logic_error("hfg_ctx_declare_fock_band: radial node outside the elements\n");
  ctx->band_node.clear();
  ctx->band_state = 0;
  EigWork &w = work_for(ctx);
  w.sup_S = nullptr;
  if (dH0) {
    hipStream_t s = ctx->stream;
    DevBuf<int> &buf = w.ibuf2;
    buf.resize((size_t)N + 8);
    int flag = 0;
    HFG_HIP_CHECK(hipMemcpyAsync(buf.p + 1, node, sizeof(int) * N, hipMemcpyHostToDevice, s));
    HFG_HIP_CHECK(hipMemsetAsync(buf.p, 0, sizeof(int), s));
    hipLaunchKernelGGL(k_band_outside, dim3((N + 255) / 256, N), dim3(256), 0, s, dH0, N, buf.p + 1, dBlockId, pm, E, buf.p);
    HFG_HIP_CHECK(hipMemcpyAsync(&flag, buf.p, sizeof(int), hipMemcpyDeviceToHost, s));
    HFG_HIP_CHECK(hipStreamSynchronize(s));
    if (flag) {
      ctx->band_state = 2;
      return 2;
    }
  }
  ctx->band_node.assign(node, node + N);
  ctx->band_pm = pm;
  ctx->band_E = E;
  ctx->band_state = 1;
  return 1;
}

void eig_gsym_sub_pair_dev(hfg_ctx *ctx, int N, const double *dFa, const double *dFb, const double *dS, int nblk, const int64_t *blk_ptr,
                           const int64_t *blk_idx, double *dEa, double *dCa, double *dEb, double *dCb) {
  const double *Fs[2] = {dFa, dFb};
  double *Es[2] = {dEa, dEb}, *Cs[2] = {dCa, dCb};
  eig_gsym_sub_multi_dev(ctx, N, 2, Fs, dS, nblk, blk_ptr, blk_idx, 0, Es, Cs);
}
// ... 3 lines not shown
```

### helfem_amd/csrc/hip/fock.hip

```cpp
#include "internal.h"
#include "xc_device.h"
#include "../host/dftfuncs.h"
#include "../host/fock_need.h"
#include <algorithm>
#include <cstring>

namespace hfg {

__global__ void k_gather_compact(const double *__restrict__ P, int N, int A, int R, int E, int p,
                                 const int *__restrict__ shell_off, const int *__restrict__ shell_skip,
                                 double *__restrict__ Xc, int *__restrict__ on) {
  int blk = blockIdx.x;
  int e = blk % E;
  int xy = blk / E;
  int y = xy % A, x = xy / A;
  int pp = p * p;
  int live = 0;
  for (int t = threadIdx.x; t < pp; t += blockDim.x) {
    int i = t % p, j = t / p;
    int ni = e * (p - 1) + i, nj = e * (p - 1) + j;
    double v = 0.0;
    bool ok = (ni < R) && (nj < R) && !(shell_skip[x] && ni == 0) && !(shell_skip[y] && nj == 0);
    if (ok) v = P[(size_t)(shell_off[y] + nj) * N + (shell_off[x] + ni)];
    Xc[(size_t)blk * pp + t] = v;
// ... 86 lines not shown
  size_t stride = (size_t)gridDim.x * blockDim.x;
  for (; i < n; i += stride) a[i] += b[i];
}

__global__ void k_gather_compact_pol(const double *__restrict__ Pa, const double *__restrict__ Pb, int N, int A, int R, int E,
                                     int p, const int *__restrict__ shell_off, const int *__restrict__ shell_skip,
                                     double *__restrict__ Xa, double *__restrict__ Xb, double *__restrict__ Xt,
                                     int *__restrict__ on) {
  int blk = blockIdx.x;
  int e = blk % E;
  int xy = blk / E;
  int y = xy % A, x = xy / A;
  int pp = p * p;
  int live = 0;
  for (int t = threadIdx.x; t < pp; t += blockDim.x) {
    int i = t % p, j = t / p;
    int ni = e * (p - 1) + i, nj = e * (p - 1) + j;
    double va = 0.0, vb = 0.0;
    bool ok = (ni < R) && (nj < R) && !(shell_skip[x] && ni == 0) && !(shell_skip[y] && nj == 0);
    if (ok) {
      size_t o = (size_t)(shell_off[y] + nj) * N + (shell_off[x] + ni);
      va = Pa[o];
      vb = Pb[o];
    }
    size_t c = (size_t)blk * pp + t;
    Xa[c] = va;
    Xb[c] = vb;
    Xt[c] = va + vb;
    live |= (va != 0.0) | (vb != 0.0);
  }
  if (on) {
    live = __syncthreads_or(live);
    if (threadIdx.x == 0) on[blk] = live;
  }
}

__global__ void k_fock_combine_pol(double *__restrict__ Fc, const double *__restrict__ Xa, const double *__restrict__ Xb,
                                   size_t nc) {
  size_t i = (size_t)blockIdx.x * blockDim.x + threadIdx.x;
  size_t stride = (size_t)gridDim.x * blockDim.x;
  for (; i < nc; i += stride) {
    double j = Fc[nc + i];
    Fc[i] = j + Xa[i];
    Fc[nc + i] = j + Xb[i];
  }
}

__global__ void k_fock_finish_pol(const double *__restrict__ Xc, size_t nc, const double *__restrict__ H0,
                                  const int *__restrict__ blockid, int N, int A, int R, int E, int p,
                                  const int *__restrict__ pure_shell, const int *__restrict__ pure_n,
                                  double *__restrict__ outa, double *__restrict__ outb) {
  int row = blockIdx.x * 64 + (threadIdx.x & 63);
  int col = blockIdx.y * 4 + (threadIdx.x >> 6);
  if (row >= N || col >= N) return;
  size_t o = (size_t)col * N + row;
  if (blockid && blockid[row] != blockid[col]) {
    outa[o] = 0.0;
    outb[o] = 0.0;
    return;
  }
  int x = pure_shell[row], n = pure_n[row];
  int y = pure_shell[col], m = pure_n[col];
  int pm = p - 1, pp = p * p;
  int e1 = n / pm, f1 = m / pm;
  double va = H0 ? H0[o] : 0.0, vb = va;
  const double *base = Xc + (size_t)(x * A + y) * E * pp;
  for (int ce = 0; ce < 2; ce++) {
    int e = e1 - ce;
    if (e < 0 || e >= E) continue;
    int i = n - e * pm;
    if (i < 0 || i > pm) continue;
    for (int cf = 0; cf < 2; cf++) {
      int f = f1 - cf;
      if (f != e) continue;
      int j = m - f * pm;
      if (j < 0 || j > pm) continue;
      size_t c = (size_t)e * pp + j * p + i;
      va += base[c];
      vb += base[nc + c];
    }
  }
  outa[o] = va;
  outb[o] = vb;
}

__global__ void k_coulomb_ket(const double *__restrict__ Pc, int A, int E, int pp, const int *__restrict__ lm_off,
                              const int *__restrict__ lm_x, const int *__restrict__ lm_y,
                              const double *__restrict__ lm_c0, const double *__restrict__ lm_c2, int NLM,
                              const int *__restrict__ LM_ilm, int rank, int nranks, double *__restrict__ Paux,
                              const int *__restrict__ on, int *__restrict__ chan) {
  int iLM = blockIdx.x, e = blockIdx.y;
  if (LM_ilm[iLM] % nranks != rank) return;
  int beg = lm_off[iLM], end = lm_off[iLM + 1];
  if (on) {
    int live = 0;
    for (int k = beg + threadIdx.x; k < end; k += blockDim.x) live |= on[((size_t)lm_x[k] * A + lm_y[k]) * E + e];
    live = __syncthreads_or(live);
    if (threadIdx.x == 0) chan[(size_t)iLM * E + e] = live;
    if (!live) {
      for (int t = threadIdx.x; t < pp; t += blockDim.x) {
        Paux[((size_t)(0 * NLM + iLM) * E + e) * pp + t] = 0.0;
        Paux[((size_t)(1 * NLM + iLM) * E + e) * pp + t] = 0.0;
      }
      return;
    }
  }
  for (int t = threadIdx.x; t < pp; t += blockDim.x) {
    double a0 = 0.0, a2 = 0.0;
    int k = beg;
    for (; k + 8 <= end; k += 8) {
      double v[8];
#pragma unroll
      for (int u = 0; u < 8; u++) v[u] = Pc[((size_t)(lm_x[k + u] * A + lm_y[k + u]) * E + e) * pp + t];
#pragma unroll
      for (int u = 0; u < 8; u++) {
        a0 += lm_c0[k + u] * v[u];
        a2 += lm_c2[k + u] * v[u];
      }
    }
    for (; k < end; k++) {
      double v = Pc[((size_t)(lm_x[k] * A + lm_y[k]) * E + e) * pp + t];
      a0 += lm_c0[k] * v;
      a2 += lm_c2[k] * v;
    }
    Paux[((size_t)(0 * NLM + iLM) * E + e) * pp + t] = a0;
    Paux[((size_t)(1 * NLM + iLM) * E + e) * pp + t] = a2;
  }
}

__global__ void k_coulomb_tei(const double *__restrict__ tei, const double *__restrict__ Paux, int Ntab, int NLM,
                              int E, int pp, const int *__restrict__ lmpos ,
                              const int *__restrict__ lm_tab, int rank, int nranks, double *__restrict__ Y,
                              const int *__restrict__ chan) {
  extern __shared__ double sh[];
  int ilm = blockIdx.x / E, e = blockIdx.x % E;
  if (ilm % nranks != rank) return;
  int tt = blockIdx.y;
  int iLMp = lmpos[2 * ilm], iLMm = lmpos[2 * ilm + 1];
  if (chan && !(iLMp >= 0 && chan[(size_t)iLMp * E + e]) && !(iLMm >= 0 && chan[(size_t)iLMm * E + e])) {
    for (int r = threadIdx.x; r < pp; r += blockDim.x) {
      if (iLMp >= 0) Y[((size_t)(tt * NLM + iLMp) * E + e) * pp + r] = 0.0;
      if (iLMm >= 0) Y[((size_t)(tt * NLM + iLMm) * E + e) * pp + r] = 0.0;
    }
    return;
  }
  int which = (tt & 1);
  double *xp = sh, *xm = sh + pp;
  for (int t = threadIdx.x; t < pp; t += blockDim.x) {
    xp[t] = (iLMp >= 0) ? Paux[((size_t)(which * NLM + iLMp) * E + e) * pp + t] : 0.0;
    xm[t] = (iLMm >= 0) ? Paux[((size_t)(which * NLM + iLMm) * E + e) * pp + t] : 0.0;
  }
  __syncthreads();
  const double *T = tei + (((size_t)tt * Ntab + lm_tab[ilm]) * E + e) * (size_t)pp * pp;
  for (int r = threadIdx.x; r < pp; r += blockDim.x) {
    double yp = 0.0, ym = 0.0;
#pragma unroll 5
    for (int c = 0; c < pp; c++) {
      double v = T[(size_t)c * pp + r];
      yp += v * xp[c];
      ym += v * xm[c];
    }
    if (iLMp >= 0) Y[((size_t)(tt * NLM + iLMp) * E + e) * pp + r] = yp;
    if (iLMm >= 0) Y[((size_t)(tt * NLM + iLMm) * E + e) * pp + r] = ym;
  }
}

// ... 1157 lines not shown
__global__ void k_mp_fill(const double *__restrict__ rad_w, const double *__restrict__ rad_sh,
                          const double *__restrict__ th_c, const double *__restrict__ th_s,
                          const double *__restrict__ th_w, int G, int nth, int nphi, double Rh, int geom, DevModelPot p1,
                          DevModelPot p2, double *__restrict__ Fo) {
  const size_t Q = blockIdx.x;
  const double shm = rad_sh[Q], wr = rad_w[Q];
  const double dphi = 2.0 * HFG_PI / nphi;
  for (int t = threadIdx.x; t < G * G * nth; t += blockDim.x) {
    const int i = t % nth, gab = t / nth, ga = gab / G, gb = gab % G;
    double f = 0.0;
    if (ga == gb) {
      const double sth = th_s[i], cth = th_c[i];
      double w, v;
      if (geom == 0) {
        const double chm = sqrt(1.0 + shm * shm);
        w = th_w[i] * dphi * wr * Rh * Rh * Rh * shm * (shm * shm + sth * sth);
        v = mp_potential(p1, Rh * (chm + cth)) + mp_potential(p2, Rh * (chm - cth));
      } else {
        w = th_w[i] * dphi * wr * shm * shm;
        v = mp_potential(p1, shm);
      }
      f = 0.5 * nphi * w * v;
    }
    Fo[((Q * G + ga) * G + gb) * nth + i] = f;
  }
}

static int round_up64(int n) { return ((n + 63) / 64) * 64; }
static size_t xc_fock_radial_lds(int p, int nq, int do_lapl = 0) {
  const size_t shb = (size_t)(4 * nq + (do_lapl ? 6 : 4) * nq * p) * sizeof(double);
  if (shb > 150 * 1024) throw std::runtime_error("radial quadrature too large for the XC Fock kernel's LDS tables");
  if (shb > 64 * 1024)
    HFG_HIP_CHECK(hipFuncSetAttribute((const void *)k_xc_fock_radial, hipFuncAttributeMaxDynamicSharedMemorySize, (int)shb));
  return shb;
}
static size_t xc_fock_theta_lds(int nth, int maxgrp, int do_lapl) {
  size_t shb = (size_t)((do_lapl ? 6 : 5) * nth + 4 * nth * maxgrp) * sizeof(double);
  if (shb > 160 * 1024) throw std::runtime_error("angular grid too large for the XC Fock kernel's LDS tables");
  if (shb > 64 * 1024)
    HFG_HIP_CHECK(hipFuncSetAttribute((const void *)k_xc_fock_theta, hipFuncAttributeMaxDynamicSharedMemorySize, (int)shb));
  return shb;
}
static void launch_xc_fock_theta(hfg_ctx *ctx, size_t NQ, int G, int nth, int maxgrp, const double *Fo, const double *Th, const double *dTh,
                                 int A, const int *grp_off, const int *grp_shell, int do_grad, int do_tau, int rank, int nranks,
                                 double *GA, double *GB, double *GC, int do_lapl = 0, double *GL = nullptr, const int *gneed = nullptr) {
  const int nf = do_lapl ? 6 : 5;
  const size_t need = (size_t)(nf * nth + 4 * nth * maxgrp) * sizeof(double);
  if (need <= tuning().xc_lds_limit) {
    hipLaunchKernelGGL(k_xc_fock_theta, dim3((unsigned)NQ, G * G), dim3(256), xc_fock_theta_lds(nth, maxgrp, do_lapl), ctx->stream, Fo, Th, dTh, A,
                       nth, G, grp_off, grp_shell, do_grad, do_tau, do_lapl, NQ, rank, nranks, GA, GB, GC, GL, gneed);
    return;
  }
  if (maxgrp * maxgrp > XC_FT_MAXPP * 256) throw std::runtime_error("angular basis too large for the XC Fock kernels (more than 64 shells of one m)");
  int nthc = (int)(tuning().xc_lds_limit / sizeof(double) / (nf + 4 * maxgrp));
  if (nthc < 4) throw std::runtime_error("angular basis too large for the XC Fock kernels' LDS tables");
  nthc = std::min(nthc, nth);
  const size_t shb = (size_t)(nf * nthc + 4 * nthc * maxgrp) * sizeof(double);
  if (do_lapl) {
    if (shb > 64 * 1024)
      HFG_HIP_CHECK(hipFuncSetAttribute((const void *)k_xc_fock_theta_chunked<true>, hipFuncAttributeMaxDynamicSharedMemorySize, (int)shb));
    hipLaunchKernelGGL(k_xc_fock_theta_chunked<true>, dim3((unsigned)NQ, G * G), dim3(256), shb, ctx->stream, Fo, Th, dTh, A, nth, G, grp_off,
                       grp_shell, do_grad, do_tau, NQ, rank, nranks, GA, GB, GC, GL, nthc, gneed);
    return;
  }
  if (shb > 64 * 1024)
    HFG_HIP_CHECK(hipFuncSetAttribute((const void *)k_xc_fock_theta_chunked<false>, hipFuncAttributeMaxDynamicSharedMemorySize, (int)shb));
  hipLaunchKernelGGL(k_xc_fock_theta_chunked<false>, dim3((unsigned)NQ, G * G), dim3(256), shb, ctx->stream, Fo, Th, dTh, A, nth, G, grp_off,
                     grp_shell, do_grad, do_tau, NQ, rank, nranks, GA, GB, GC, (double *)nullptr, nthc, gneed);
}

static size_t xc_density_radial_lds(int p, int nq, int do_lapl = 0) {
  const int NJ = (256 / nq > 0) ? std::min(256 / nq, p) : 1;
  size_t shb = (size_t)(p * p + 2 * p * nq + 3 * NJ * nq + (do_lapl ? NJ * nq + p * nq : 0)) * sizeof(double);
  if (shb > 150 * 1024) throw std::runtime_error("radial quadrature too large for the XC density kernel's LDS tables");
  if (shb > 64 * 1024)
    HFG_HIP_CHECK(hipFuncSetAttribute((const void *)k_xc_density_radial, hipFuncAttributeMaxDynamicSharedMemorySize, (int)shb));
  return shb;
}

struct FockAux : Workspace {
  DevBuf<int> pure_shell, pure_n, lmpos;
  DevBuf<double> Pc, Jc, Pc2, Jc2, Pc3, Paux, Y, Jaux, D0, D1, D2, D3, V, Fo, GA, GB, GC, GL, partial, scal;
  DevBuf<int> on, gon, chan;
};

struct FockSkip {
  const int *on = nullptr, *gon = nullptr;
  int *chan = nullptr;
  const int *need = nullptr, *gneed = nullptr;
};

static void aux_setup(hfg_ctx *ctx, const hfg_dev_tables *t, FockAux *a) {
  std::vector<int> ps(t->N), pn(t->N);
  {
    size_t k = 0;
    for (int s = 0; s < t->A; s++)
      for (int n = (t->h_shell_skip[s] ? 1 : 0); n < t->R; n++, k++) {
        ps[k] = s;
        pn[k] = n;
      }
  }
  a->pure_shell.upload(ps, ctx->stream);
  a->pure_n.upload(pn, ctx->stream);
  std::vector<int> lmpos(2 * t->Nlm, -1);
  for (int i = 0; i < t->NLM; i++) {
    int M = t->h_LM_M[i];
    int ilm = t->h_LM_ilm[i];
    if (M >= 0) lmpos[2 * ilm] = i;
    if (M < 0) lmpos[2 * ilm + 1] = i;
  }
  a->lmpos.upload(lmpos, ctx->stream);
  HFG_HIP_CHECK(hipStreamSynchronize(ctx->stream));
}
static FockAux &aux_for(hfg_ctx *ctx, hfg_basis *basis) {
  hfg_dev_tables *t = basis->dev;
  return t->work.get<FockAux>(WS_FOCK, [&](FockAux &a) { aux_setup(ctx, t, &a); });
}

static hfg_dev_tables *tables_of(hfg_ctx *ctx, hfg_basis *basis) {
  if (!basis->dev || !basis->dev->have_tei) throw std::logic_error("Primitive teis have not been computed!\n");
  if (basis->dev_device != ctx->device) throw std::logic_error("basis tables live on a different device\n");
  return basis->dev;
}

static void gather_compact(hfg_ctx *ctx, hfg_basis *basis, const double *dP, double *dPc) {
  hfg_dev_tables *t = basis->dev;
  hipLaunchKernelGGL(k_gather_compact, dim3(t->A * t->A * t->E), dim3(256), 0, ctx->stream, dP, t->N, t->A, t->R, t->E,
                     t->p, t->shell_off.p, t->shell_skip.p, dPc, (int *)nullptr);
}

static void skip_flags_behind_on(hfg_ctx *ctx, hfg_dev_tables *t, FockAux &a, bool with_need, FockSkip &sk) {
  sk.on = a.on.p;
  sk.chan = a.chan.p;
  if (t->have_xc) {
    a.gon.resize((size_t)t->E * t->G * t->G);
    hipLaunchKernelGGL(k_skip_groups, dim3(t->E, t->G * t->G), dim3(256), 0, ctx->stream, a.on.p, t->A, t->E, t->G, t->grp_off.p,
                       t->grp_shell.p, a.gon.p);
    sk.gon = a.gon.p;
  }
  if (with_need && ctx->fock_need_tables == t && ctx->fock_need_A == t->A) {
    sk.need = ctx->fock_need.p;
    if (t->have_xc && ctx->fock_need_G == t->G) sk.gneed = ctx->fock_gneed.p;
  }
}

static FockSkip gather_compact_flagged(hfg_ctx *ctx, hfg_basis *basis, const double *dP, double *dPc, bool with_need) {
  hfg_dev_tables *t = basis->dev;
  FockSkip sk;
  if (!helfem::tuning_live().fock_skip) {
    gather_compact(ctx, basis, dP, dPc);
    return sk;
  }
  FockAux &a = aux_for(ctx, basis);
  a.on.resize((size_t)t->A * t->A * t->E);
  a.chan.resize((size_t)t->NLM * t->E);
  hipLaunchKernelGGL(k_gather_compact, dim3(t->A * t->A * t->E), dim3(256), 0, ctx->stream, dP, t->N, t->A, t->R, t->E,
                     t->p, t->shell_off.p, t->shell_skip.p, dPc, a.on.p);
  skip_flags_behind_on(ctx, t, a, with_need, sk);
  return sk;
}

static FockSkip gather_compact_pol_flagged(hfg_ctx *ctx, hfg_basis *basis, const double *dPa, const double *dPb, bool with_need) {
  hfg_dev_tables *t = basis->dev;
  FockAux &a = aux_for(ctx, basis);
  FockSkip sk;
  const bool skip = helfem::tuning_live().fock_skip;
// ... 368 lines not shown
  const FockSkip sk = gather_compact_flagged(ctx, basis, dP, a.Pc.p, false);
  xc_compact(ctx, basis, x_func, c_func, a.Pc.p, a.Jc.p, dScal, thr, sk);
  scatter_dense(ctx, basis, a.Jc.p, dH);
  HFG_HIP_CHECK(hipGetLastError());
}

static size_t xc_grid_pol_lds(const hfg_dev_tables *t, const XCPlan &pl, int *rowc) {
  const int npot2 = pl.do_lapl ? 12 : (pl.do_tau ? 10 : 8);
  *rowc = t->ntheta;
  while ((size_t)(npot2 * *rowc * t->nphi + 3 * 4) * sizeof(double) > tuning().xc_lds_limit && *rowc > 1) *rowc = (*rowc + 1) / 2;
  const size_t shb = (size_t)(npot2 * *rowc * t->nphi + 3 * 4) * sizeof(double);
  if (shb > 150 * 1024) throw std::runtime_error("XC angular grid too large for the polarised grid kernel's LDS tile");
  return shb;
}

static void xc_compact_pol(hfg_ctx *ctx, hfg_basis *basis, int x_func, int c_func, const double *dPca, const double *dPcb,
                           double *dHca, double *dHcb, double *dScal, double thr, const FockSkip &sk = FockSkip()) {
  hfg_dev_tables *t = tables_of(ctx, basis);
  const XCPlan pl = xc_plan(t, x_func, c_func, thr);
  FockAux &a = aux_for(ctx, basis);
  const int npl = pl.do_lapl ? 6 : (pl.do_tau ? 5 : 3);
  xc_buffers(a, pl, 2 * npl);
  for (int sp = 0; sp < 2; sp++) xc_density_stage(ctx, t, a, pl, sp ? dPcb : dPca, a.V.p + (size_t)sp * npl * pl.nv, sk);
  int rowc;
  const size_t shb = xc_grid_pol_lds(t, pl, &rowc);
  launch_xc_grid(ctx, t, a, pl, k_xc_grid_pol<true>, k_xc_grid_pol<false>, shb, x_func, c_func, rowc);
  for (int sp = 0; sp < 2; sp++) xc_fock_stage(ctx, t, a, pl, a.Fo.p + (size_t)sp * npl * pl.nv, sp ? dHcb : dHca, sk);
  hipLaunchKernelGGL(k_xc_sum_partials, dim3(1), dim3(64), 0, ctx->stream, a.partial.p, pl.NQ, dScal);
  HFG_HIP_CHECK(hipGetLastError());
}

void xc_fock_pol_dev(hfg_ctx *ctx, hfg_basis *basis, int x_func, int c_func, const double *dPa, const double *dPb,
                     double *dHa, double *dHb, double *dScal, double thr) {
  hfg_dev_tables *t = tables_of(ctx, basis);
  FockAux &a = aux_for(ctx, basis);
  const size_t nc = (size_t)t->A * t->A * t->E * t->p * t->p;
  a.Pc.resize(nc);
  a.Jc.resize(nc);
  a.Pc2.resize(nc);
  a.Jc2.resize(nc);
  ProfScope ps(ctx, "xc");
  gather_compact(ctx, basis, dPa, a.Pc.p);
  gather_compact(ctx, basis, dPb, a.Pc2.p);
  xc_compact_pol(ctx, basis, x_func, c_func, a.Pc.p, a.Pc2.p, a.Jc.p, a.Jc2.p, dScal, thr);
  scatter_dense(ctx, basis, a.Jc.p, dHa);
  scatter_dense(ctx, basis, a.Jc2.p, dHb);
  HFG_HIP_CHECK(hipGetLastError());
}

void model_potential_dev(hfg_ctx *ctx, hfg_basis *basis, int kind1, int Z1, double d1, double H1, int kind2, int Z2,
                         double d2, double H2, double *dH) {
  hfg_dev_tables *t = tables_of(ctx, basis);
  if (!t->have_xc) throw std::runtime_error("XC grid tables were not uploaded (hfg_basis_upload with ldft,mdft > 0)\n");
  for (int k : {kind1, kind2})
    if (k != 0 && k != 1 && k != 3) throw std::logic_error("Unsupported guess\n");
  if ((kind1 == 1 && !(d1 > 0.0)) || (kind2 == 1 && !(d2 > 0.0)))
    throw std::logic_error("GSZ guess: the screening length d_Z must be given\n");
  FockAux &a = aux_for(ctx, basis);
  const int A = t->A, E = t->E, p = t->p, nq = t->nq, G = t->G, nth = t->ntheta, nphi = t->nphi;
  const size_t NQ = (size_t)E * nq, AA = (size_t)A * A;
  const size_t nc = (size_t)A * A * E * p * p;
  a.Jc.resize(nc);
  a.GA.resize(NQ * AA);
  a.GB.resize(NQ * AA);
  a.Fo.resize(5 * NQ * G * G * nth);
  int maxgrp = 0;
  for (int g = 0; g < G; g++) maxgrp = std::max(maxgrp, t->h_grp_off[g + 1] - t->h_grp_off[g]);
  DevModelPot p1{kind1, Z1, d1, H1}, p2{kind2, Z2, d2, H2};
  hipLaunchKernelGGL(k_mp_fill, dim3((unsigned)NQ), dim3(256), 0, ctx->stream, t->rad_w.p, t->rad_sh.p, t->th_c.p, t->th_s.p,
                     t->th_w.p, G, nth, nphi, t->Rhalf, t->geom, p1, p2, a.Fo.p);
  launch_xc_fock_theta(ctx, NQ, G, nth, maxgrp, a.Fo.p, t->Th.p, t->dTh.p, A, t->grp_off.p, t->grp_shell.p, 0, 0, 0, 1, a.GA.p, a.GB.p,
                       (double *)nullptr);
  hipLaunchKernelGGL(k_xc_fock_radial, dim3(A * A, E), dim3(std::min(256, round_up64(p * p))),
                     xc_fock_radial_lds(p, nq), ctx->stream, a.GA.p, a.GB.p, (const double *)nullptr, (const double *)nullptr, t->rad_B.p,
                     t->rad_dB.p, (const double *)nullptr, t->shell_l.p, t->rad_sh.p, A, E, p, nq, 0, 0, 0, 0, 1, a.Jc.p, (const int *)nullptr);
  scatter_dense(ctx, basis, a.Jc.p, dH);
  HFG_HIP_CHECK(hipGetLastError());
}

size_t fock_compact_size(hfg_basis *basis) {
  return (size_t)basis->Nang() * basis->Nang() * basis->Nel() * basis->max_Nprim() * basis->max_Nprim();
}

void set_fock_blocks(hfg_ctx *ctx, hfg_basis *basis, const int *dBlockId) {
  ctx->fock_need_tables = nullptr;
  if (!dBlockId) return;
  if (!basis->dev || basis->dev_device != ctx->device) throw std::logic_error("hfg_ctx_set_fock_blocks: the basis tables are not on this context's device\n");
  const hfg_dev_tables *t = basis->dev;
  const int A = t->A;
  std::vector<int> blockid(t->N), nfunc(A), need((size_t)A * A);
  HFG_HIP_CHECK(hipDeviceSynchronize());
  HFG_HIP_CHECK(hipMemcpy(blockid.data(), dBlockId, sizeof(int) * t->N, hipMemcpyDeviceToHost));
  for (int x = 0; x < A; x++) nfunc[x] = t->R - (t->h_shell_skip[x] ? 1 : 0);
  helfem::fock_need_pairs(A, nfunc.data(), blockid.data(), need.data());
  ctx->fock_need.upload(need, ctx->stream);
  ctx->fock_need_A = A;
  ctx->fock_need_G = 0;
  if (t->have_xc) {
    std::vector<int> ms(t->h_shell_m.begin(), t->h_shell_m.begin() + A);
    std::sort(ms.begin(), ms.end());
    ms.erase(std::unique(ms.begin(), ms.end()), ms.end());
    const int G = (int)ms.size();
    if (G != t->G) throw std::logic_error("hfg_ctx_set_fock_blocks: m groups do not match the XC tables\n");
    std::vector<int> gneed((size_t)G * G, 0);
    auto grp = [&](int x) { return (int)(std::lower_bound(ms.begin(), ms.end(), t->h_shell_m[x]) - ms.begin()); };
    for (int x = 0; x < A; x++)
      for (int y = 0; y < A; y++)
        if (need[(size_t)x * A + y]) gneed[(size_t)grp(x) * G + grp(y)] = 1;
    ctx->fock_gneed.upload(gneed, ctx->stream);
    ctx->fock_need_G = G;
  }
  HFG_HIP_CHECK(hipStreamSynchronize(ctx->stream));
  ctx->fock_need_tables = t;
}

void fock_compact_dev(hfg_ctx *ctx, hfg_basis *basis, int x_func, int c_func, const double *dP, double *dFc,
                      double *dScal, double thr) {
  hfg_dev_tables *t = tables_of(ctx, basis);
  FockAux &a = aux_for(ctx, basis);
  const size_t nc = fock_compact_size(basis);
  a.Pc.resize(nc);
  a.Jc.resize(nc);
  if ((x_func > 0 || c_func > 0) && tuning().fock_overlap && !ctx->avoid_side) {
    hipStream_t main = ctx->stream, q = ctx->side();
    const FockSkip sk = gather_compact_flagged(ctx, basis, dP, a.Pc.p, true);
    HFG_HIP_CHECK(hipEventRecord(ctx->side_ev[0], main));
    HFG_HIP_CHECK(hipStreamWaitEvent(q, ctx->side_ev[0], 0));
    ctx->stream = q;
    try {
      ProfScope ps(ctx, "coulomb");
      coulomb_compact(ctx, basis, a.Pc.p, dFc, sk);
    } catch (...) {
      ctx->stream = main;
      throw;
    }
    ctx->stream = main;
    HFG_HIP_CHECK(hipEventRecord(ctx->side_ev[1], q));
    ProfScope ps(ctx, "xc");
    xc_compact(ctx, basis, x_func, c_func, a.Pc.p, a.Jc.p, dScal, thr, sk);
    HFG_HIP_CHECK(hipStreamWaitEvent(main, ctx->side_ev[1], 0));
    hipLaunchKernelGGL(k_add_inplace, dim3(2048), dim3(256), 0, ctx->stream, dFc, a.Jc.p, nc);
    HFG_HIP_CHECK(hipGetLastError());
    return;
  }
  FockSkip sk;
  {
    ProfScope ps(ctx, "coulomb");
    sk = gather_compact_flagged(ctx, basis, dP, a.Pc.p, true);
    coulomb_compact(ctx, basis, a.Pc.p, dFc, sk);
  }
  if (x_func > 0 || c_func > 0) {
    ProfScope ps(ctx, "xc");
    xc_compact(ctx, basis, x_func, c_func, a.Pc.p, a.Jc.p, dScal, thr, sk);
    hipLaunchKernelGGL(k_add_inplace, dim3(2048), dim3(256), 0, ctx->stream, dFc, a.Jc.p, nc);
  } else {
    HFG_HIP_CHECK(hipMemsetAsync(dScal, 0, 3 * sizeof(double), ctx->stream));
  }
  (void)t;
  HFG_HIP_CHECK(hipGetLastError());
}

void fock_finish_dev(hfg_ctx *ctx, hfg_basis *basis, const double *dFc, const double *dH0, const int *dBlockId,
                     double *dF) {
  hfg_dev_tables *t = tables_of(ctx, basis);
  FockAux &a = aux_for(ctx, basis);
  ProfScope ps(ctx, "scatter");
  dim3 grid((t->N + 63) / 64, (t->N + 3) / 4);
  hipLaunchKernelGGL(k_fock_finish, grid, dim3(256), 0, ctx->stream, dFc, dH0, dBlockId, t->N, t->A, t->R, t->E, t->p,
                     a.pure_shell.p, a.pure_n.p, dF);
  HFG_HIP_CHECK(hipGetLastError());
}

void fock_compact_pol_dev(hfg_ctx *ctx, hfg_basis *basis, int x_func, int c_func, const double *dPa, const double *dPb,
                          double *dFc, double *dScal, double thr) {
  hfg_dev_tables *t = tables_of(ctx, basis);
  const bool with_xc = x_func > 0 || c_func > 0;
  if (with_xc) {
    int rowc;
    (void)xc_grid_pol_lds(t, xc_plan(t, x_func, c_func, thr), &rowc);
  }
  FockAux &a = aux_for(ctx, basis);
  const size_t nc = fock_compact_size(basis);
  a.Pc.resize(nc);
  a.Pc2.resize(nc);
  a.Pc3.resize(nc);
  double *dJc = dFc + nc;
  if (!with_xc) {
    ProfScope ps(ctx, "coulomb");
    const FockSkip sk = gather_compact_pol_flagged(ctx, basis, dPa, dPb, true);
    coulomb_compact(ctx, basis, a.Pc3.p, dJc, sk);
    HFG_HIP_CHECK(hipMemcpyAsync(dFc, dJc, nc * sizeof(double), hipMemcpyDeviceToDevice, ctx->stream));
    HFG_HIP_CHECK(hipMemsetAsync(dScal, 0, 3 * sizeof(double), ctx->stream));
    return;
  }
  a.Jc.resize(nc);
  a.Jc2.resize(nc);
  if (tuning().fock_overlap && !ctx->avoid_side) {
    hipStream_t main = ctx->stream, q = ctx->side();
    const FockSkip sk = gather_compact_pol_flagged(ctx, basis, dPa, dPb, true);
    HFG_HIP_CHECK(hipEventRecord(ctx->side_ev[0], main));
    HFG_HIP_CHECK(hipStreamWaitEvent(q, ctx->side_ev[0], 0));
    ctx->stream = q;
    try {
      ProfScope ps(ctx, "coulomb");
      coulomb_compact(ctx, basis, a.Pc3.p, dJc, sk);
    } catch (...) {
      ctx->stream = main;
      throw;
    }
    ctx->stream = main;
    HFG_HIP_CHECK(hipEventRecord(ctx->side_ev[1], q));
    ProfScope ps(ctx, "xc");
    try {
      xc_compact_pol(ctx, basis, x_func, c_func, a.Pc.p, a.Pc2.p, a.Jc.p, a.Jc2.p, dScal, thr, sk);
    } catch (...) {
      (void)hipStreamWaitEvent(main, ctx->side_ev[1], 0);
      throw;
    }
    HFG_HIP_CHECK(hipStreamWaitEvent(main, ctx->side_ev[1], 0));
    hipLaunchKernelGGL(k_fock_combine_pol, dim3(2048), dim3(256), 0, ctx->stream, dFc, a.Jc.p, a.Jc2.p, nc);
    HFG_HIP_CHECK(hipGetLastError());
    return;
  }
  FockSkip sk;
  {
    ProfScope ps(ctx, "coulomb");
    sk = gather_compact_pol_flagged(ctx, basis, dPa, dPb, true);
    coulomb_compact(ctx, basis, a.Pc3.p, dJc, sk);
  }
  ProfScope ps(ctx, "xc");
  xc_compact_pol(ctx, basis, x_func, c_func, a.Pc.p, a.Pc2.p, a.Jc.p, a.Jc2.p, dScal, thr, sk);
  hipLaunchKernelGGL(k_fock_combine_pol, dim3(2048), dim3(256), 0, ctx->stream, dFc, a.Jc.p, a.Jc2.p, nc);
  HFG_HIP_CHECK(hipGetLastError());
}

void fock_finish_pol_dev(hfg_ctx *ctx, hfg_basis *basis, const double *dFc, const double *dH0, const int *dBlockId,
                         double *dFa, double *dFb) {
  hfg_dev_tables *t = tables_of(ctx, basis);
  FockAux &a = aux_for(ctx, basis);
  ProfScope ps(ctx, "scatter");
  dim3 grid((t->N + 63) / 64, (t->N + 3) / 4);
  hipLaunchKernelGGL(k_fock_finish_pol, grid, dim3(256), 0, ctx->stream, dFc, fock_compact_size(basis), dH0, dBlockId, t->N, t->A,
                     t->R, t->E, t->p, a.pure_shell.p, a.pure_n.p, dFa, dFb);
  HFG_HIP_CHECK(hipGetLastError());
}

}
```

### helfem_amd/csrc/hip/internal.h

```cpp
#pragma once
#include "common.h"
#include "tables.h"
#include "../host/scf.h"

namespace hfg {

enum class GemmTile { Auto, T64, T128, T128x64 };
struct GemmHow {
  GemmTile tile = GemmTile::Auto;
  bool acc = false, split2 = false, map = false, scatter = false, klist = false;
};
void gemm_tasklist_dev(hfg_ctx *ctx, const GemmTask *dtasks, int ntasks, int maxM, int maxN, GemmHow how = {});
void gemm_worklist_dev(hfg_ctx *ctx, const GemmTask *dtasks, const int2 *dwl, int nwg, GemmTile tile, bool split2 = false);
void gemm_worklist(const std::vector<GemmTask> &tasks, GemmTile tile, bool split2, std::vector<int2> &out);
void gemm_mirror_lower_dev(hfg_ctx *ctx, const GemmTask *dtasks, int ntasks, int maxN);
bool gemm_prefers_128(hfg_ctx *ctx, long tiles128);
void gemm_dev(hfg_ctx *ctx, bool tA, bool tB, int M, int N, int K, double alpha, const double *A, int lda, const double *B, int ldb,
              double beta, double *C, int ldc);

void coulomb_dev(hfg_ctx *ctx, hfg_basis *basis, const double *dP, double *dJ);
void coulomb_batch_dev(hfg_ctx *ctx, hfg_basis *basis, int64_t nP, const double *dP, double *dJ);
void coulomb_energy_matrix_dev(hfg_ctx *ctx, hfg_basis *basis, int64_t nP, const double *dP, double *dW);
void set_xc_params(hfg_ctx *ctx, int x_func, const double *x_pars, int nx, int c_func, const double *c_pars, int nc);
void xc_eval_host(int id, int nspin, size_t np, const double *rho, const double *sigma, const double *lapl, const double *tau,
                  double *exc, double *vrho, double *vsigma, double *vlapl, double *vtau, double thr);
void xc_eval_host_ext(int id, const double *pars, int npars, int nspin, size_t np, const double *rho, const double *sigma,
                      const double *lapl, const double *tau, double *exc, double *vrho, double *vsigma, double *vlapl, double *vtau,
                      double thr);
void xc_fock_dev(hfg_ctx *ctx, hfg_basis *basis, int x_func, int c_func, const double *dP, double *dH, double *dScal,
                 double thr);
void xc_fock_pol_dev(hfg_ctx *ctx, hfg_basis *basis, int x_func, int c_func, const double *dPa, const double *dPb, double *dHa,
                     double *dHb, double *dScal, double thr);
void model_potential_dev(hfg_ctx *ctx, hfg_basis *basis, int kind1, int Z1, double d1, double H1, int kind2, int Z2, double d2,
                         double H2, double *dH);
void set_fock_blocks(hfg_ctx *ctx, hfg_basis *basis, const int *dBlockId);
size_t fock_compact_size(hfg_basis *basis);
void fock_compact_dev(hfg_ctx *ctx, hfg_basis *basis, int x_func, int c_func, const double *dP, double *dFc, double *dScal,
                      double thr);
void fock_finish_dev(hfg_ctx *ctx, hfg_basis *basis, const double *dFc, const double *dH0, const int *dBlockId,
                     double *dF);
void fock_compact_pol_dev(hfg_ctx *ctx, hfg_basis *basis, int x_func, int c_func, const double *dPa, const double *dPb,
                          double *dFc, double *dScal, double thr);
void fock_finish_pol_dev(hfg_ctx *ctx, hfg_basis *basis, const double *dFc, const double *dH0, const int *dBlockId,
                         double *dFa, double *dFb);

enum class ExTables { coulomb, screened, mix };
hfg_dev_tables *exchange_tables(hfg_basis *basis, ExTables which);
void exchange_dev(hfg_ctx *ctx, hfg_basis *basis, const double *dP, double *dK, ExTables which = ExTables::coulomb,
                  const double *Lknown = nullptr, int rknown = 0);
bool exchange_lowrank_dev(hfg_ctx *ctx, hfg_dev_tables *t, const double *dP, double *dK, const double *Lknown,
                          int rknown);
void exchange_batch_dev(hfg_ctx *ctx, hfg_basis *basis, int64_t nP, const double *dP, double *dK, ExTables which = ExTables::coulomb,
                        const double *dC = nullptr, const int64_t *nocc = nullptr, int64_t ldc = 0);

constexpr double EXL_PAIR_MAX_BYTES = 32e9;
int mix_exchange_tables_dev(hfg_ctx *ctx, hfg_basis *basis, double alpha, double beta);

void compute_tei_dev(hfg_ctx *ctx, hfg_basis *basis);

void compute_rs_tei_dev(hfg_ctx *ctx, hfg_basis *basis, int rs_kind, double omega);
void rs_special_dev(hfg_ctx *ctx, int which, int L, const double *a, const double *b, size_t n, double *out);

void eig_sym_dev(hfg_ctx *ctx, int n, const double *dA, double *dE, double *dC);
void eig_gsym_dev(hfg_ctx *ctx, int N, int n, const double *dF, const double *dS, double *dE, double *dC);
void eig_gsym_sub_dev(hfg_ctx *ctx, int N, const double *dF, const double *dS, int nblk, const int64_t *blk_ptr,
                      const int64_t *blk_idx, double *dE, double *dC);
void eig_gsym_sub_pair_dev(hfg_ctx *ctx, int N, const double *dFa, const double *dFb, const double *dS, int nblk,
                           const int64_t *blk_ptr, const int64_t *blk_idx, double *dEa, double *dCa, double *dEb,
                           double *dCb);
size_t eig_block_buf_size(int nblk, const int64_t *blk_ptr);
void eig_blocks_dev(hfg_ctx *ctx, int N, const double *dF, const double *dS, int nblk, const int64_t *blk_ptr,
                    const int64_t *blk_idx, double *dBlockBuf);
void eig_assemble_dev(hfg_ctx *ctx, int N, int nblk, const int64_t *blk_ptr, const int64_t *blk_idx, const double *dBlockBuf,
                      double *dE, double *dC);
void eig_block_supports(hfg_ctx *ctx, int N, const double *dS, int nblk, const int64_t *blk_ptr, const int64_t *blk_idx,
                        std::vector<int64_t> &cols);
int64_t eig_sel_count(int nblk, const int64_t *blk_ptr, int64_t nev);
void eig_sym_sel_dev(hfg_ctx *ctx, int n, const double *dA, int nev, double *dE, double *dC);
void eig_gsym_sub_sel_dev(hfg_ctx *ctx, int N, const double *dF, const double *dS, int nblk, const int64_t *blk_ptr,
                          const int64_t *blk_idx, int nev, double *dE, double *dC);

int eig_declare_band(hfg_ctx *ctx, int N, const int *node, int pm, int E, const double *dH0, const int *dBlockId);

void tridiag_dc_batch(hfg_ctx *ctx, int nblk, const int *ns, double *const *d, double *const *e, double *const *Z);
int dc_status(hfg_ctx *ctx);
int *dc_status_word(hfg_ctx *ctx);
void tridiag_sel_batch(hfg_ctx *ctx, int nblk, const int *ns, const int *nev, double *const *d, double *const *e, double *const *W,
                       double *const *Z);
void tridiagonalize_batch(hfg_ctx *ctx, int nblk, const int *ns, double *const *A, double *const *d, double *const *e,
                          double *const *tau);
void trd_measure_gemv(hfg_ctx *ctx, double *ms, int64_t *launches);
bool tridiagonalize_takes_chain(int nblk, const int *ns);
void tridiagonalize_persistent(hfg_ctx *ctx, int nblk, const int *ns, double *const *A, double *const *d, double *const *e,
                               double *const *tau, std::vector<char> &done);
void trdp_check_status(hfg_ctx *ctx);

void form_sinvh_dev(hfg_ctx *ctx, int N, const double *dS, bool chol, int nblk, const int64_t *blk_ptr, const int64_t *blk_idx,
                    double *dSinvh);
void form_density_dev(hfg_ctx *ctx, int N, int ncols, const double *dC, int nocc, double *dP);

constexpr int DIIS_LR_MAXCOLS = 64;
constexpr int DIIS_HIST_CHUNK = 8;
struct DiisErrTask {
  const double *A, *B;
  double *out;
  int n, k, ld, ldo;
};
struct DiisHistory {
  const double *E[DIIS_HIST_CHUNK], *P[DIIS_HIST_CHUNK], *F[DIIS_HIST_CHUNK];
  int n;
};
struct DiisComb {
  const double *F[16];
  double w[16];
  int n;
};
size_t diis_lowrank_partials(int ntasks, int nmax);
void diis_lowrank_error_dev(hfg_ctx *ctx, const DiisErrTask *dtasks, int ntasks, int nmax, double *dPartialMax,
                            double *dMax);
void diis_history_dev(hfg_ctx *ctx, const DiisHistory &h, int j0, int nhtot, const double *dEnew, size_t elen, const double *dPnew,
                      const double *dFnew, size_t flen, bool want_max, double *dPartial, double *dRes);
void diis_extrapolate_dev(hfg_ctx *ctx, const DiisComb &c, size_t NN, int nspin, double *dFa, double *dFb);

constexpr int CUHF_LR_MAXCOLS = 128;
void cuhf_lowrank_dev(hfg_ctx *ctx, int N, const double *dS, const double *dCa, int nocca, const double *dCb, int noccb, double *dFa,
                      double *dFb);
void cuhf_dense_dev(hfg_ctx *ctx, int N, int n, const double *dP, const double *dSh, const double *dSinvh, int nocca, int noccb,
                    double *dFa, double *dFb);

helfem::scf::Result scf_device_loop(hfg_ctx *ctx, hfg_basis *hb, const helfem::scf::Options &opt, int nel, double Enucr, int symm,
                                    const std::vector<std::vector<size_t> > &dsym, int ldft, int mdft,
                                    const std::vector<std::vector<std::vector<size_t> > > &avg_idx =
                                        std::vector<std::vector<std::vector<size_t> > >());

}
```

### helfem_amd/csrc/host/tuning.h

```cpp
#pragma once
#include <string>

namespace helfem {
constexpr int EXL_GMAX = 16;
enum class TrdMode { persistent, chain, twokernel, unblocked };
enum class EigSel { crossover, stein, dc };
enum class RsTei { host, dev };
#define HELFEM_TUNING(X) \
  X(scf_host, bool, false, "HELFEM_SCF", true, "=host", !strcmp(e, "host"), "SCF loop driven from the host through the per-stage entry points (checker of the device-resident loop)") \
  X(tei_host, bool, false, "HELFEM_TEI", false, "=host", !strcmp(e, "host"), "in-element tables built by the threaded host code and uploaded (checker of tei_dev.hip)") \
  X(rs_tei, RsTei, RsTei::host, "HELFEM_RS_TEI", false, "word", !strcmp(e, "dev") ? RsTei::dev : RsTei::host, "range-separated exchange tables of the SCF drivers: dev = built on the device (rs_tei_dev.hip); unset or any other word = built by the threaded host code and uploaded") \
  X(exchange_general, bool, false, "HELFEM_EXCHANGE", true, "=general", !strcmp(e, "general"), "general exchange kernels always, not only where the low-rank fast path declines") \
  X(exl_rb, int, 0, "HELFEM_EXL_RB", false, "int", atoi(e), "RB kernel of the low-rank exchange: 4 the 4 x 4 vector kernel, 1 the one-pair vector kernel (checkers), else the matrix-core kernel k_exl_RBm") \
  X(exl_mgroups, bool, true, "HELFEM_EXL_MGROUPS", false, "off if 0", atoi(e) != 0, "cross-element products by blocks of equal m; off: the full products") \
  X(exl_rect, int, -1, "HELFEM_EXL_RECT", false, "int", atoi(e), "tiles of the element GEMM: 0 / 1 / 2 = 128 x 128 / 128 x 64 / 64 x 64 always; negative: 64 x 64 when the tasks average fewer than 1500 pairs, else 128 x 128") \
  X(exl_wl, bool, true, "HELFEM_EXL_WL", false, "off if 0", atoi(e) != 0, "XCD-contiguous workgroup lists for the element GEMM and the cross products; off: plain task-list grids") \
  X(exl_splitk, bool, true, "HELFEM_EXL_SPLITK", false, "off if 0", atoi(e) != 0, "two half-K workgroups per tile for the cross products; off: one workgroup per tile") \
  X(exl_crect, bool, true, "HELFEM_EXL_CRECT", false, "off if 0", atoi(e) != 0, "128 x 64 tiles for the split cross products; off: 128 x 128") \
  X(exl_groups, int, 4, "HELFEM_EXL_GROUPS", false, "int", std::max(1, std::min(EXL_GMAX, atoi(e))), "groups of 64 factors tried before the general kernels take over, clamped to 1 ... 16") \
  X(exl_hint, bool, true, "HELFEM_EXL_HINT", false, "off if 0", atoi(e) != 0, "the SCF loop's occupied orbitals taken as the factors of P; off: always factorise and verify P (checker)") \
  X(exl_pair, bool, true, "HELFEM_EXL_PAIR", false, "off if 0", atoi(e) != 0, "low-rank fast path for the pair (erfc) tables; off: general kernels") \
  X(exl_mix, int, -1, "HELFEM_EXL_MIX", true, "int", atoi(e), "range-separated hybrids in the step objects: 0 = K from two builds, hfg_exchange_occ_dev and hfg_rs_exchange_dev, added on the device (checker); other non-negative = one build on the mixed-kernel table set (hfg_mix_exchange_tables); negative: by kernel kind as measured, the mixed set for both Yukawa and erfc") \
  X(fock_overlap, bool, true, "HELFEM_FOCK_OVERLAP", false, "off if 0", atoi(e) != 0, "Coulomb kernels on the side stream beside the XC kernels; off: one after the other on the main stream") \
  X(fock_skip, bool, true, "HELFEM_FOCK_SKIP", true, "off if 0", atoi(e) != 0, "Fock build skips shell pairs whose density block is zero and, after hfg_ctx_set_fock_blocks, pairs the caller does not read; off: every pair is computed (checker)") \
  X(xc_lds_limit, size_t, 150 * 1024, "HELFEM_XC_LDS_LIMIT", false, "int", (size_t)atol(e), "bytes of LDS the angular XC kernels plan with; smaller forces the chunked kernels (tests)") \
  X(coulomb_batch_chunk, int, 0, "HELFEM_COULOMB_BATCH_CHUNK", true, "int", std::max(0, atoi(e)), "densities per pass over the tables of the batched Coulomb build forced smaller than the LDS rule allows (tests; 0: the rule's own)") \
  X(exchange_batch_chunk, int, 0, "HELFEM_EXCHANGE_BATCH_CHUNK", true, "int", std::max(0, atoi(e)), "densities per pass over the tables of the batched exchange build at most (tests; 0: as many as fit the 64 factor columns of a pass)") \
  X(uscf_kbatch, bool, false, "HELFEM_USCF_KBATCH", true, "=1", atoi(e) == 1, "DeviceUSCFStep: K[Pa] and K[Pb] through one call of hfg_exchange_occ_batch_devptr; off: one call per spin") \
  X(diis_blocks, bool, true, "HELFEM_DIIS_BLOCKS", false, "off if 0", atoi(e) != 0, "DIIS error per symmetry block; off: the four dense N^3 products (checker)") \
  X(diis_lowrank, bool, true, "HELFEM_DIIS_LOWRANK", false, "off if 0", atoi(e) != 0, "blocked DIIS error from the occupied orbitals; off: per-block n^3 products from F and P (checker)") \
  X(cuhf_lowrank, bool, true, "HELFEM_CUHF_LOWRANK", true, "off if 0", atoi(e) != 0, "hfg_cuhf_update_devptr: the constraint from the occupied orbitals (rank na + nb, up to 128 columns); off: the dense natural-orbital sequence always (checker)") \
  X(eig_pair, bool, true, "HELFEM_EIG_PAIR", false, "off if 0", atoi(e) != 0, "both spins' Fock matrices in one batched eigensolve; off: two calls") \
  X(eig_direct, bool, true, "HELFEM_EIG_DIRECT", true, "off if 0", atoi(e) != 0, "one-call blocked eigensolve (hfg_eig_gsym_sub_dev, _sel_dev, _pair_devptr) ranks before its last product and stores that product straight into C; off: block slots, then hfg_eig_assemble_dev (checker)") \
  X(eig_band, bool, true, "HELFEM_EIG_BAND", true, "off if 0", atoi(e) != 0, "blocked eigensolve under a declared radial-element pattern of F (hfg_ctx_declare_fock_band): rows of F radial-major, F X as row-tile tasks over the k steps that meet their non-zero columns, bit for bit the dense product; off: the declaration is ignored (checker)") \
  X(trd_mode, TrdMode, TrdMode::persistent, "HELFEM_TRD", false, "word", !strcmp(e, "persistent") ? TrdMode::persistent : !strcmp(e, "twokernel") ? TrdMode::twokernel : !strcmp(e, "unblocked") ? TrdMode::unblocked : TrdMode::chain, "tridiagonalisation: persistent = k_trdp where the batch fits, else the chain; chain (and any unknown word) = one k_trdf launch per column always (checker); twokernel = k_trdb_gemv + k_trdb_w; unblocked = the first-generation kernels") \
  X(trdp_min, int, 256, "HELFEM_TRDP_MIN", false, "int", atoi(e), "smallest order the persistent kernel takes") \
  X(trdp_r, int, 0, "HELFEM_TRDP_R", false, "int", atoi(e), "rows per thread of the persistent kernel forced (0: the first that fits)") \
  X(trdp_u, int, 0, "HELFEM_TRDP_U", false, "int", atoi(e), "column chunks per thread of the persistent kernel forced wider than needed (measurement; 0: narrowest)") \
  X(trdp_limit_ms, long long, 200, "HELFEM_TRDP_LIMIT_MS", false, "int", atoll(e), "wall-clock bound of every spin of the persistent kernel, ms") \
  X(trdp_phases, bool, true, "HELFEM_TRDP_PHASES", false, "off if 0", atoi(e) != 0, "one cooperative launch per phase; off: the whole matrix in one launch (checker)") \
  X(trdp_step, int, 96, "HELFEM_TRDP_STEP", false, "int", std::max(1, atoi(e)), "fewest columns of a phase (at least 1)") \
  X(trdp_coop, bool, true, "HELFEM_TRDP_COOP", false, "off if 0", atoi(e) != 0, "hipLaunchCooperativeKernel for the phases; off: plain launches (A/B of the launch overhead)") \
  X(trdp_stamps, int, 0, "HELFEM_TRDP_STAMPS", false, "int", atoi(e), "non-zero: the stamping kernels, one launch per eigensolve, phase summary on stderr; 2 and more: also per-column stamps of one workgroup") \
  X(trdp_stamps_file, std::string, "", "HELFEM_TRDP_STAMPS_FILE", false, "path", e, "with stamps: file for the stamps of every workgroup over 64 columns (tools/trdp_window.py)") \
  X(trd_tail, int, 2, "HELFEM_TRD_TAIL", false, "int", atoi(e), "last columns of the chain in one launch: 0 none, 1 the LDS-resident kernel (order 128), else the register-resident kernel (order 192)") \
  X(trdf_sym, int, -1, "HELFEM_TRDF_SYM", false, "int", atoi(e), "symmetric sweep of k_trdf: 0 never, other non-negative always, negative by HELFEM_TRDF_SYM_MIN") \
  X(trdf_sym_min, int, 0, "HELFEM_TRDF_SYM_MIN", false, "int", atoi(e), "panels whose full grid has more tiles than this sweep one triangle only") \
  X(trd_band_update, bool, true, "HELFEM_TRD_BAND_UPDATE", false, "off if 0", atoi(e) != 0, "band-limited trailing updates when every sweep is symmetric; off: full updates") \
  X(trdf_nth, int, 0, "HELFEM_TRDF_NTH", false, "int", atoi(e), "512: k_trdf with 512 threads; anything else 1024 (A/B runs)") \
  X(acc_tile, int, 0, "HELFEM_ACC_TILE", false, "int", atoi(e), "128: 128 x 128 tiles for the accumulating updates (and full, not band-limited ones); anything else 64 x 64") \
  X(trdf_dbg, int, 0, "HELFEM_TRDF_DBG", false, "int", atoi(e), "measurement replay of k_trdf only: bits 0-2 go to the kernel's debug field, bit 2 also prints the per-wave stamps (tools/trdf_probe.py)") \
  X(trdf_c, int, -1, "HELFEM_TRDF_C", false, "int", atoi(e), "measurement replay of k_trdf only: column-in-panel index forced for every launch (negative: each launch's own)") \
  X(tridiag_ql, bool, false, "HELFEM_TRIDIAG", false, "=ql", !strcmp(e, "ql"), "one-lane implicit QL for the tridiagonal problem instead of divide and conquer (checker)") \
  X(dc_gemm_small, bool, false, "HELFEM_DC_GEMM", false, "=small", !strcmp(e, "small"), "Q U of the divide-and-conquer merges by the first 64 x 64 kernel instead of the tile engine (checker)") \
  X(dc_levels, bool, false, "HELFEM_DC", false, "=levels", !strcmp(e, "levels"), "divide-and-conquer merges with the gather, scatter and copy-back passes over Q and ten launches per level (checker of the column-mapped product)") \
  X(eigsel, EigSel, EigSel::crossover, "HELFEM_EIGSEL", false, "word", !strcmp(e, "stein") ? EigSel::stein : !strcmp(e, "dc") ? EigSel::dc : EigSel::crossover, "selected eigenpairs (hfg_eig_*_sel): stein = multisection and inverse iteration always; dc = the full divide and conquer, then the lowest columns (checker); unset or any other word = the crossover, which sends every wanted fraction to dc (measured: stein is slower down to 1/64 of the columns)") \
  X(dc_dbg, bool, false, "HELFEM_DC_DBG", false, "present", true, "merge statistics of divide and conquer on stderr") \
  X(bt_column, bool, false, "HELFEM_BT", false, "=column", !strcmp(e, "column"), "back-transformation reflector by reflector instead of compact WY (checker)") \
  X(bt_fold, bool, true, "HELFEM_BT_FOLD", false, "off if 0", atoi(e) != 0, "X Q formed on the side stream beside divide and conquer; off: Z <- Q Z on the main stream behind it") \
  X(bt_side, bool, false, "HELFEM_BT_SIDE", false, "=1", atoi(e) == 1, "without the fold: the compact-WY set-up on the side stream") \
  X(gemm_tile, int, 0, "HELFEM_GEMM_TILE", false, "int", atoi(e), "128: 128 x 128 tiles always; other non-zero: 64 x 64 always; 0: the large tiles where they fill whole rounds of the chip") \
  X(gemm_splitk, int, -1, "HELFEM_GEMM_SPLITK", false, "int", atoi(e), "eigensolve's products: 0 / other non-negative = large tiles without / with two half-K workgroups each; negative: chosen by tile count") \
  X(gemm_rect, bool, false, "HELFEM_GEMM_RECT", false, "on if not 0", atoi(e) != 0, "128 x 64 tiles for the eigensolve's large-tile products") \
  X(mfma_4x4x4, bool, false, "HELFEM_MFMA", false, "=4x4x4", !strcmp(e, "4x4x4"), "v_mfma_f64_4x4x4_4b_f64 in the tile engine instead of v_mfma_f64_16x16x4_f64 (A/B runs)") \
  X(num_threads, int, 0, "HELFEM_NUM_THREADS", true, "int", std::max(0, atoi(e)), "host threads of the set-up code (0: one per core, 64 at most)") \
  X(hdf5_lib, std::string, "", "HELFEM_HDF5_LIB", true, "path", e, "HDF5 library tried before the usual names")

struct Tuning {
#define X(field, type, def, ...) type field = def;
  HELFEM_TUNING(X)
#undef X
};
const Tuning &tuning();
Tuning tuning_live();
std::string tuning_table();
}
```

### include/helfem_gpu.h

```cpp
#ifndef HELFEM_GPU_H
#define HELFEM_GPU_H

#include <stddef.h>
#include <stdint.h>

#ifdef __cplusplus
extern "C" {
#endif

typedef struct hfg_ctx hfg_ctx;
typedef struct hfg_basis hfg_basis;

#define HFG_NULL_STREAM ((void *)(intptr_t)-1)
int hfg_ctx_create(hfg_ctx **ctx, int device, void *stream);
int hfg_ctx_destroy(hfg_ctx *ctx);
int hfg_ctx_synchronize(hfg_ctx *ctx);
const char *hfg_last_error(void);
const char *hfg_version(void);
int hfg_device_count(void);

int hfg_ctx_set_shard(hfg_ctx *ctx, int rank, int nranks);

int hfg_ctx_fix_sinvh(hfg_ctx *ctx, const double *dSinvh);

// ... 102 lines not shown
int hfg_xc_fock_pol(hfg_ctx *ctx, hfg_basis *basis, int x_func, int c_func, const double *Pa, const double *Pb,
                    double *Ha, double *Hb, double *Exc, double *Nel, double *Ekin, double dens_thr);
int hfg_xc_fock_ext(hfg_ctx *ctx, hfg_basis *basis, int x_func, const double *x_pars, int n_x_pars, int c_func,
                    const double *c_pars, int n_c_pars, const double *P, double *H, double *Exc, double *Nel, double *Ekin,
                    double dens_thr);
int hfg_xc_fock_pol_ext(hfg_ctx *ctx, hfg_basis *basis, int x_func, const double *x_pars, int n_x_pars, int c_func,
                        const double *c_pars, int n_c_pars, const double *Pa, const double *Pb, double *Ha, double *Hb,
                        double *Exc, double *Nel, double *Ekin, double dens_thr);
int hfg_xc_eval(int func_id, int nspin, int64_t np, const double *rho, const double *sigma, const double *lapl, const double *tau,
                double *exc, double *vrho, double *vsigma, double *vlapl, double *vtau, double dens_thr);
int hfg_xc_eval_ext(int func_id, const double *pars, int n_pars, int nspin, int64_t np, const double *rho, const double *sigma,
                    const double *lapl, const double *tau, double *exc, double *vrho, double *vsigma, double *vlapl, double *vtau,
                    double dens_thr);
int hfg_xc_func_ids(const char *method, int *x_func, int *c_func);
const char *hfg_xc_func_name(int func_id);
int hfg_xc_exact_exchange(int x_func, double *omega, double *alpha, double *beta);
int hfg_xc_rs_kind(int x_func);
int hfg_xc_func_table(char *buf, size_t cap);
int hfg_basis_radial_table(const hfg_basis *basis, int which, int iel, double *out, int64_t *rows, int64_t *cols);
typedef struct {
  int kind;
  int Z;
  double d, H;
} hfg_model_pot;
int hfg_model_potential(hfg_ctx *ctx, hfg_basis *basis, const hfg_model_pot *p1, const hfg_model_pot *p2, double *H);
int hfg_scf_set_iguess(int iguess);
int hfg_eig_gsym(hfg_ctx *ctx, int64_t N, int64_t n, const double *F, const double *Sinvh, double *E, double *C);
int hfg_eig_gsym_sub(hfg_ctx *ctx, int64_t N, const double *F, const double *Sinvh, int nblk,
                     const int64_t *blk_ptr, const int64_t *blk_idx, double *E, double *C);
int hfg_eig_gsym_sub_pair(hfg_ctx *ctx, int64_t N, const double *Fa, const double *Fb, const double *Sinvh, int nblk,
                          const int64_t *blk_ptr, const int64_t *blk_idx, double *Ea, double *Ca, double *Eb, double *Cb);
int hfg_eig_sym(hfg_ctx *ctx, int64_t n, const double *A, double *E, double *C);
int64_t hfg_eig_sel_count(int nblk, const int64_t *blk_ptr, int64_t nev);
int hfg_eig_sym_sel(hfg_ctx *ctx, int64_t n, const double *A, int64_t nev, double *E, double *C);
int hfg_eig_gsym_sub_sel(hfg_ctx *ctx, int64_t N, const double *F, const double *Sinvh, int nblk, const int64_t *blk_ptr,
                         const int64_t *blk_idx, int64_t nev, double *E , double *C );
int hfg_form_sinvh(hfg_ctx *ctx, int64_t N, const double *S, int chol, int nblk, const int64_t *blk_ptr,
                   const int64_t *blk_idx, double *Sinvh);
int hfg_form_density(hfg_ctx *ctx, int64_t N, int64_t ncols, const double *C, int64_t nocc, double *P);
int hfg_gemm(hfg_ctx *ctx, int transA, int transB, int64_t m, int64_t n, int64_t k, const double *A, int64_t lda,
             const double *B, int64_t ldb, double *C, int64_t ldc);

int hfg_coulomb_dev(hfg_ctx *ctx, hfg_basis *basis, const double *dP, double *dJ);
int hfg_coulomb_batch_devptr(hfg_ctx *ctx, hfg_basis *basis, int64_t nP, const double *dP, double *dJ);
int hfg_exchange_dev(hfg_ctx *ctx, hfg_basis *basis, const double *dP, double *dK);
int hfg_rs_exchange_dev(hfg_ctx *ctx, hfg_basis *basis, const double *dP, double *dK);
int hfg_exchange_occ_dev(hfg_ctx *ctx, hfg_basis *basis, const double *dP, const double *dC, int64_t nocc, double *dK);
int hfg_exchange_batch_devptr(hfg_ctx *ctx, hfg_basis *basis, int64_t nP, const double *dP, double *dK);
int hfg_rs_exchange_batch_devptr(hfg_ctx *ctx, hfg_basis *basis, int64_t nP, const double *dP, double *dK);
int hfg_exchange_occ_batch_devptr(hfg_ctx *ctx, hfg_basis *basis, int64_t nP, const double *dP, const double *dC,
                                  const int64_t *nocc, int64_t ldc_cols, double *dK);
int hfg_mix_exchange_tables(hfg_ctx *ctx, hfg_basis *basis, double alpha, double beta);
int hfg_mix_exchange(hfg_ctx *ctx, hfg_basis *basis, const double *P, double *K);
int hfg_mix_exchange_devptr(hfg_ctx *ctx, hfg_basis *basis, const double *dP, double *dK);
int hfg_mix_exchange_occ_devptr(hfg_ctx *ctx, hfg_basis *basis, const double *dP, const double *dC, int64_t nocc, double *dK);
int hfg_mix_exchange_occ_batch_devptr(hfg_ctx *ctx, hfg_basis *basis, int64_t nP, const double *dP, const double *dC,
                                      const int64_t *nocc, int64_t ldc_cols, double *dK);
int hfg_exchange_batch_plan(int64_t nP, const int *ranks, int max_members, int *chunk_of, int *nchunks);
int hfg_xc_fock_dev(hfg_ctx *ctx, hfg_basis *basis, int x_func, int c_func, const double *dP, double *dH,
                    double *dScal, double dens_thr);
int hfg_xc_fock_pol_dev(hfg_ctx *ctx, hfg_basis *basis, int x_func, int c_func, const double *dPa, const double *dPb,
                        double *dHa, double *dHb, double *dScal , double dens_thr);
int64_t hfg_fock_compact_size(hfg_basis *basis);
int hfg_fock_compact_dev(hfg_ctx *ctx, hfg_basis *basis, int x_func, int c_func, const double *dP, double *dFc,
                         double *dScal, double dens_thr);
int hfg_fock_finish_dev(hfg_ctx *ctx, hfg_basis *basis, const double *dFc, const double *dH0, const int *dBlockId,
                        double *dF);
int64_t hfg_fock_compact_pol_size(hfg_basis *basis);
int hfg_fock_compact_pol_devptr(hfg_ctx *ctx, hfg_basis *basis, int x_func, int c_func, const double *dPa, const double *dPb,
                                double *dFc, double *dScal , double dens_thr);
int hfg_fock_finish_pol_devptr(hfg_ctx *ctx, hfg_basis *basis, const double *dFc, const double *dH0, const int *dBlockId,
                               double *dFa, double *dFb);
int hfg_eig_gsym_sub_pair_devptr(hfg_ctx *ctx, int64_t N, const double *dFa, const double *dFb, const double *dSinvh, int nblk,
                                 const int64_t *blk_ptr, const int64_t *blk_idx, double *dEa, double *dCa, double *dEb,
                                 double *dCb);
int hfg_cuhf_update_devptr(hfg_ctx *ctx, int64_t N, const double *dS, const double *dCa, int64_t nocca, const double *dCb,
                           int64_t noccb, double *dFa, double *dFb);
int hfg_rohf_update(hfg_ctx *ctx, int64_t N, int64_t n, double *Fa, double *Fb, const double *P, const double *Sh,
                    const double *Sinvh, int64_t nocca, int64_t noccb);
int hfg_ctx_set_fock_blocks(hfg_ctx *ctx, hfg_basis *basis, const int *blockid_dev);
int hfg_fock_need_pairs(int nshell, const int *nfunc, const int *blockid, int *need);
int hfg_eig_gsym_sub_dev(hfg_ctx *ctx, int64_t N, const double *dF, const double *dSinvh, int nblk,
                         const int64_t *blk_ptr, const int64_t *blk_idx, double *dE, double *dC);
int hfg_eig_gsym_sub_sel_dev(hfg_ctx *ctx, int64_t N, const double *dF, const double *dSinvh, int nblk, const int64_t *blk_ptr,
                             const int64_t *blk_idx, int64_t nev, double *dE , double *dC );
int64_t hfg_eig_block_buf_size(int nblk, const int64_t *blk_ptr);
int hfg_eig_blocks_dev(hfg_ctx *ctx, int64_t N, const double *dF, const double *dSinvh, int nblk,
                       const int64_t *blk_ptr, const int64_t *blk_idx, double *dBlockBuf);
int hfg_eig_assemble_dev(hfg_ctx *ctx, int64_t N, int nblk, const int64_t *blk_ptr, const int64_t *blk_idx,
                         const double *dBlockBuf, double *dE, double *dC);
int hfg_form_density_dev(hfg_ctx *ctx, int64_t N, int64_t ncols, const double *dC, int64_t nocc, double *dP);
int hfg_gemm_dev(hfg_ctx *ctx, int transA, int transB, int64_t m, int64_t n, int64_t k, const double *dA,
                 int64_t lda, const double *dB, int64_t ldb, double *dC, int64_t ldc);

int hfg_scf_diatomic(hfg_ctx *ctx, int Z1, int Z2, double Rbond, const int *lmmax, int nlm, int nelem, int nnodes,
                     int nquad, double Rmax, int igrid, double zexp, int lpad, const char *method, int ldft, int mdft,
                     int symmetry, int multiplicity, int maxit, double convthr, int verbose, double *out );

#define HFG_MAX_LMMAX 16
typedef struct hfg_scf_options {
  int program;
  int Z1, Z2;
  double Rbond;
  int nela, nelb, Q, M;
  int lmmax[HFG_MAX_LMMAX];
  int nlm;
  int lmax, mmax;
  int lpad;
  double Rmax;
  int grid;
  double zexp;
  int nelem, nnodes, nquad;
  int maxit;
  double convthr;
  int diag;
  char method[128];
  int ldft, mdft;
  double dftthr;
  int restricted;
  int symmetry;
  int primbas;
  double diiseps, diisthr;
  int diisorder;
  int iguess;
  const double *x_pars;
  int n_x_pars;
  const double *c_pars;
  int n_c_pars;
  int maverage;
  double dampfock, dampthr;
  char save[512];
  char load[512];
  double Ez, Qzz, Bz;
  int finitenuc;
  int readocc;
  const int *occs;
  int occ_rows, occ_cols;
  double perturb;
  int iconf;
  int zeroder;
  int verbose;
} hfg_scf_options;

typedef struct hfg_scf_result {
  double Etot, Ekin, Epot, Enucr, Ecoul, Exx, Exc;
  int iterations, converged;
  int nela, nelb;
  int64_t Nbf;
  double tJ, tK, tXC, tdiag;
} hfg_scf_result;

int hfg_scf_options_default(hfg_scf_options *opt, int program);
int hfg_scf_set_occupations(int readocc, int nrows, int ncols, const int *rows);
int hfg_scf_options_check(const hfg_scf_options *opt);
int hfg_scf_run(hfg_ctx *ctx, const hfg_scf_options *opt, hfg_scf_result *res, double *E, double *C);
typedef struct hfg_scf_atomic_extras {
  double Rrms;
  int conf_N;
  double conf_R;
  double conf_barrier;
  double shift_conf;
  int add_conf;
  int Zl, Zr;
  double Rmid;
  int nelem0;
  int grid0;
// ... 47 lines not shown
```

Before: 7.705 ms.

## Fuse Fock finish with symmetry-block scatter into eigensolver operand buffer

Adds a block-aware Fock finish kernel that writes only entries inside the symmetry blocks and, when the eigensolver's cached plan matches, scatters them straight into the eigensolver's per-block operand buffer. The eigensolve then skips its own gather of F into blocks, tracked through a finish counter and Python-side version stamps on F. The goal is to remove the full-square finish pass and the separate gather kernel in each SCF step. In exchange it adds host-side validation, state coupling between the Fock and eig modules, and a risk of stale operands if the invalidation logic misses a write to F.

```diff
diff --git a/helfem_amd/__init__.py b/helfem_amd/__init__.py
--- a/helfem_amd/__init__.py
+++ b/helfem_amd/__init__.py
@@ -159,6 +159,11 @@
         for name in ("hfg_exchange_occ_dev", "hfg_mix_exchange_occ_devptr"):
             getattr(L, name).argtypes = [ctypes.c_void_p] * 4 + [ctypes.c_int64, ctypes.c_void_p]
         L.hfg_mix_exchange_occ_batch_devptr.argtypes = L.hfg_exchange_occ_batch_devptr.argtypes
+        L.hfg_fock_compact_parts_devptr.argtypes = L.hfg_fock_compact_dev.argtypes + [ctypes.POINTER(ctypes.c_void_p)]
+        L.hfg_fock_finish_blocks_devptr.argtypes = [ctypes.c_void_p] * 7
+        L.hfg_fock_finish_blocks_pol_devptr.argtypes = [ctypes.c_void_p] * 8
+        L.hfg_eig_gsym_sub_handoff_devptr.argtypes = [ctypes.c_void_p, ctypes.c_int64, ctypes.c_void_p, ctypes.c_void_p, ctypes.c_int,
+                                                      c_i64_p, c_i64_p, ctypes.c_void_p, ctypes.c_void_p, ctypes.c_int]
         _lib = L
     return _lib
 
@@ -1298,6 +1303,10 @@
         self.kscale = self.kfrac if self.kshort == 0.0 else 1.0
         self.have_C = False
         self.have_density = False
+        self._f_clean = True
+        self._f_from_finish = False
+        self._f_ver = None
+        self._Xc = None
         if self.kshort != 0.0 and not self.mix:
             self.Krs = torch.zeros(N * N, dtype=torch.float64, device=self.dev)
 
@@ -1340,13 +1349,37 @@
             else:
                 self.torch.mul(self.Krs, self.kshort, out=K)
 
-    def fock_partial(self):
+    def fock_partial(self, parts=False):
+        self._Xc = None
+        if parts:
+            xc = ctypes.c_void_p()
+            _check(lib().hfg_fock_compact_parts_devptr(self.ctx.h, self.basis.h, self.x_func, self.c_func, self._ptr(self.P),
+                                                       self._ptr(self.Fc), self._ptr(self.scal), self.thr, ctypes.byref(xc)))
+            self._Xc = xc
+            return
         _check(lib().hfg_fock_compact_dev(self.ctx.h, self.basis.h, self.x_func, self.c_func, self._ptr(self.P),
                                           self._ptr(self.Fc), self._ptr(self.scal), self.thr))
 
-    def fock_finish(self):
+    def fock_finish(self, blocks=False):
+        if blocks:
+            _check(lib().hfg_fock_finish_blocks_devptr(self.ctx.h, self.basis.h, self._ptr(self.Fc), self._Xc, self._ptr(self.H0),
+                                                       self._ptr(self.blockid), self._ptr(self.F)))
+            return
+        if self._Xc is not None and self._Xc.value:
+            raise RuntimeError("fock_finish: the build was split (fock_partial(parts=True)); finish it with blocks=True")
         _check(lib().hfg_fock_finish_dev(self.ctx.h, self.basis.h, self._ptr(self.Fc), self._ptr(self.H0),
                                          self._ptr(self.blockid), self._ptr(self.F)))
+
+    def _f_written(self):
+        self._f_clean = False
+        self._f_from_finish = False
+
+    def _f_versions(self):
+        return tuple(F._version for _, F, _, _, _ in self._spins())
+
+    def _f_untouched(self):
+        ver = self._f_versions()
+        return all(v == 0 for v in ver) if self._f_ver is None else self._f_ver == ver
 
     def _spins(self):
         return ((self.P, self.F, self.E, self.C, self.nocc),)
@@ -1369,10 +1402,11 @@
                                               self.blk_ptr.ctypes.data_as(c_i64_p), self.blk_idx.ctypes.data_as(c_i64_p),
                                               self._ptr(buf), self._ptr(E), self._ptr(C)))
 
-    def eig_whole(self):
-        _check(lib().hfg_eig_gsym_sub_dev(self.ctx.h, ctypes.c_int64(self.N), self._ptr(self.F), self._ptr(self.Sinvh),
-                                          len(self.blocks), self.blk_ptr.ctypes.data_as(c_i64_p),
-                                          self.blk_idx.ctypes.data_as(c_i64_p), self._ptr(self.E), self._ptr(self.C)))
+    def eig_whole(self, f_from_finish=False):
+        _check(lib().hfg_eig_gsym_sub_handoff_devptr(self.ctx.h, ctypes.c_int64(self.N), self._ptr(self.F), self._ptr(self.Sinvh),
+                                                     len(self.blocks), self.blk_ptr.ctypes.data_as(c_i64_p),
+                                                     self.blk_idx.ctypes.data_as(c_i64_p), self._ptr(self.E), self._ptr(self.C),
+                                                     1 if f_from_finish else 0))
 
     def density(self):
         for P, _, _, C, nocc in self._spins():
@@ -1386,7 +1420,8 @@
     def step(self, allreduce=None, exchange_blocks=None):
         self._fock_stage(allreduce)
         self._constrain()
-        self._eig_stage(allreduce, exchange_blocks)
+        self._eig_stage(allreduce, exchange_blocks, self._f_from_finish and self._f_untouched())
+        self._f_from_finish = False
         self.density()
         self.have_C = True
 
@@ -1401,6 +1436,7 @@
 
     def _fock_stage(self, allreduce):
         shard_fock = self.nranks > 1 and self.fock_shard == "always"
+        blocks = self._f_clean and self._f_untouched()
         if shard_fock or self.nranks == 1:
             self.fock_partial()
             if allreduce is not None:
@@ -1408,7 +1444,10 @@
                 allreduce(self.scal)
         else:
             self._whole_shard(self.fock_partial)
-        self.fock_finish()
+        self.fock_finish(blocks=blocks)
+        self._f_clean = True
+        self._f_from_finish = True
+        self._f_ver = self._f_versions()
         if self.anyK:
             self.exchange()
             if allreduce is not None:
@@ -1418,13 +1457,14 @@
     def _add_exchange(self):
         for (_, F, _, _, _), K in zip(self._spins(), self._spin_K()):
             F.add_(K, alpha=self.kscale)
+        self._f_written()
 
     def _eig_in_one_call(self, allreduce, exchange_blocks):
         return self.nranks == 1 and allreduce is None and exchange_blocks is None
 
-    def _eig_stage(self, allreduce, exchange_blocks):
+    def _eig_stage(self, allreduce, exchange_blocks, f_from_finish=False):
         if self._eig_in_one_call(allreduce, exchange_blocks):
-            self.eig_whole()
+            self.eig_whole(f_from_finish)
             return
         self.eig_partial()
         for buf in self._blockbufs():
@@ -1474,6 +1514,7 @@
     def _core_guess(self, allreduce, exchange_blocks):
         for _, F, _, _, _ in self._spins():
             F.copy_(self.H0)
+        self._f_written()
         self._eig_stage(allreduce, exchange_blocks)
         self._density_stage()
 
@@ -1485,6 +1526,7 @@
 
     def _diis_solve(self, diis):
         diis.solve(self.F)
+        self._f_written()
 
     _applies_cuhf = False
 
@@ -1602,15 +1644,19 @@
             else:
                 self._build_K(P, C, ctypes.c_int64(nocc), K)
 
-    def fock_partial(self):
+    def fock_partial(self, parts=False):
         _check(lib().hfg_fock_compact_pol_devptr(self.ctx.h, self.basis.h, self.x_func, self.c_func, self._ptr(self.Pa),
                                                  self._ptr(self.Pb), self._ptr(self.Fc), self._ptr(self.scal), self.thr))
 
-    def fock_finish(self):
+    def fock_finish(self, blocks=False):
+        if blocks:
+            _check(lib().hfg_fock_finish_blocks_pol_devptr(self.ctx.h, self.basis.h, self._ptr(self.Fc), None, self._ptr(self.H0),
+                                                           self._ptr(self.blockid), self._ptr(self.Fa), self._ptr(self.Fb)))
+            return
         _check(lib().hfg_fock_finish_pol_devptr(self.ctx.h, self.basis.h, self._ptr(self.Fc), self._ptr(self.H0),
                                                 self._ptr(self.blockid), self._ptr(self.Fa), self._ptr(self.Fb)))
 
-    def eig_pair(self):
+    def eig_pair(self, f_from_finish=False):
         _check(lib().hfg_eig_gsym_sub_pair_devptr(self.ctx.h, ctypes.c_int64(self.N), self._ptr(self.Fa), self._ptr(self.Fb),
                                                   self._ptr(self.Sinvh), len(self.blocks), self.blk_ptr.ctypes.data_as(c_i64_p),
                                                   self.blk_idx.ctypes.data_as(c_i64_p), self._ptr(self.Ea), self._ptr(self.Ca),
@@ -1647,6 +1693,7 @@
 
     def _diis_solve(self, diis):
         diis.solve(self.Fa, self.Fb)
+        self._f_written()
 
 
 class DeviceROHFStep(DeviceUSCFStep):
@@ -1674,3 +1721,4 @@
             raise RuntimeError("DeviceROHFStep: the constraint needs the orbitals the densities were formed from "
                                "(set_density with Ca and Cb, or start from the core guess)")
         self.ctx.cuhf_update(self.S, self.Ca, self.nela, self.Cb, self.nelb, self.Fa, self.Fb)
+        self._f_written()
diff --git a/helfem_amd/csrc/hip/capi.cpp b/helfem_amd/csrc/hip/capi.cpp
--- a/helfem_amd/csrc/hip/capi.cpp
+++ b/helfem_amd/csrc/hip/capi.cpp
@@ -913,6 +913,38 @@
   eig_gsym_sub_pair_dev(ctx, (int)N, dFa, dFb, dSinvh, nblk, blk_ptr, blk_idx, dEa, dCa, dEb, dCb);
   HFG_CATCH
 }
+int hfg_fock_compact_parts_devptr(hfg_ctx *ctx, hfg_basis *b, int x_func, int c_func, const double *dP, double *dFc, double *dScal,
+                                  double thr, const double **dXc) {
+  HFG_TRY
+  if (!ctx || !b) throw std::logic_error("hfg_fock_compact_parts_devptr: null context or basis\n");
+  if (!dP || !dFc || !dScal || !dXc) throw std::logic_error("hfg_fock_compact_parts_devptr: null pointer\n");
+  fock_compact_dev(ctx, b, x_func, c_func, dP, dFc, dScal, thr, dXc);
+  HFG_CATCH
+}
+int hfg_fock_finish_blocks_devptr(hfg_ctx *ctx, hfg_basis *b, const double *dFc, const double *dJc, const double *dH0,
+                                  const int *dBlockId, double *dF) {
+  HFG_TRY
+  if (!ctx || !b) throw std::logic_error("hfg_fock_finish_blocks_devptr: null context or basis\n");
+  if (!dFc || !dF) throw std::logic_error("hfg_fock_finish_blocks_devptr: null device pointer\n");
+  fock_finish_blocks_dev(ctx, b, dFc, dJc, dH0, dBlockId, dF);
+  HFG_CATCH
+}
+int hfg_fock_finish_blocks_pol_devptr(hfg_ctx *ctx, hfg_basis *b, const double *dFc, const double *dJc, const double *dH0,
+                                      const int *dBlockId, double *dFa, double *dFb) {
+  HFG_TRY
+  if (!ctx || !b) throw std::logic_error("hfg_fock_finish_blocks_pol_devptr: null context or basis\n");
+  if (!dFc || !dFa || !dFb) throw std::logic_error("hfg_fock_finish_blocks_pol_devptr: null device pointer\n");
+  fock_finish_blocks_dev(ctx, b, dFc, dJc, dH0, dBlockId, dFa, dFb);
+  HFG_CATCH
+}
+int hfg_eig_gsym_sub_handoff_devptr(hfg_ctx *ctx, int64_t N, const double *dF, const double *dSinvh, int nblk, const int64_t *blk_ptr,
+                                    const int64_t *blk_idx, double *dE, double *dC, int f_from_finish) {
+  HFG_TRY
+  if (!ctx) throw std::logic_error("hfg_eig_gsym_sub_handoff_devptr: null context\n");
+  if (!dF || !dSinvh || !blk_ptr || !blk_idx || !dE || !dC) throw std::logic_error("hfg_eig_gsym_sub_handoff_devptr: null pointer\n");
+  eig_gsym_sub_dev(ctx, (int)N, dF, dSinvh, nblk, blk_ptr, blk_idx, dE, dC, f_from_finish != 0);
+  HFG_CATCH
+}
 int hfg_ctx_set_fock_blocks(hfg_ctx *ctx, hfg_basis *b, const int *blockid_dev) {
   HFG_TRY
   if (!ctx || !b) throw std::logic_error("hfg_ctx_set_fock_blocks: null context or basis");
diff --git a/helfem_amd/csrc/hip/common.h b/helfem_amd/csrc/hip/common.h
--- a/helfem_amd/csrc/hip/common.h
+++ b/helfem_amd/csrc/hip/common.h
@@ -96,6 +96,7 @@
   hfg::DevBuf<int> fock_need, fock_gneed;
   const hfg_dev_tables *fock_need_tables = nullptr;
   int fock_need_A = 0, fock_need_G = 0;
+  unsigned long finish_count = 0;
   bool profiling = false;
   std::map<std::string, hfg::ProfEntry> prof;
   std::vector<hipEvent_t> event_pool;
diff --git a/helfem_amd/csrc/hip/eig.hip b/helfem_amd/csrc/hip/eig.hip
--- a/helfem_amd/csrc/hip/eig.hip
+++ b/helfem_amd/csrc/hip/eig.hip
@@ -618,6 +618,11 @@
   DevBuf<int> band_ks_dev, band_iota_dev;
   DevBuf<GemmTask> fxtasks;
   std::vector<GemmTask> h_fxtasks;
+  DevBuf<double> Fb;
+  bool fb_plan = false, fb_band = false, fb_src_band = false;
+  size_t fb_nmax = 0;
+  const double *fb_src = nullptr;
+  unsigned long fb_stamp = 0;
   int *h_status = nullptr;
   hipEvent_t status_ev = nullptr;
   ~EigWork() {
@@ -1143,7 +1148,7 @@
 
 static void eig_blocks_multi_dev(hfg_ctx *ctx, int N, int nF, const double *const *dFs, const double *dS, int nblk, const int64_t *blk_ptr,
                                  const int64_t *blk_idx, double *const *dBlockBufs, int nev = 0, double *const *dEs = nullptr,
-                                 double *const *dCs = nullptr);
+                                 double *const *dCs = nullptr, bool f_from_finish = false);
 static int eig_num_cus(hfg_ctx *ctx) {
   static const int ncu = [&] {
     hipDeviceProp_t prop;
@@ -1153,10 +1158,11 @@
 }
 void eig_blocks_dev(hfg_ctx *ctx, int N, const double *dF, const double *dS, int nblk, const int64_t *blk_ptr,
                     const int64_t *blk_idx, double *dBlockBuf) {
-  eig_blocks_multi_dev(ctx, N, 1, &dF, dS, nblk, blk_ptr, blk_idx, &dBlockBuf);
+  eig_blocks_multi_dev(ctx, N, 1, &dF, dS, nblk, blk_ptr, blk_idx, &dBlockBuf, 0, nullptr, nullptr, false);
 }
 static void eig_blocks_multi_dev(hfg_ctx *ctx, int N, int nF, const double *const *dFs, const double *dS, int nblk, const int64_t *blk_ptr,
-                                 const int64_t *blk_idx, double *const *dBlockBufs, int nev, double *const *dEs, double *const *dCs) {
+                                 const int64_t *blk_idx, double *const *dBlockBufs, int nev, double *const *dEs, double *const *dCs,
+                                 bool f_from_finish) {
   EigWork &w = work_for(ctx);
   hipStream_t s = ctx->stream;
   const bool direct = dEs != nullptr;
@@ -1176,6 +1182,8 @@
                       w.sup_idx.size() == (size_t)N && std::equal(w.sup_idx.begin(), w.sup_idx.end(), blk_idx);
   if (!cached) {
     w.sup_S = nullptr;
+    w.fb_plan = false;
+    w.fb_src = nullptr;
     w.xc_have.clear();
     HFG_HIP_CHECK(hipStreamSynchronize(s));
     w.band_rows.clear();
@@ -1279,10 +1287,16 @@
   for (int f = 0; f < nF; f++)
     for (int ib = 0; ib < nblk; ib++)
       if (ib % ctx->shard_n == ctx->shard_rank) mine.push_back(f * nblk + ib);
-  DevBuf<double> &Fb = ctx->ws[5];
+  DevBuf<double> &Fb = w.Fb;
   DevBuf<double> &T1 = ctx->ws[0];
   DevBuf<double> &Xall = ctx->ws[4];
+  if (Fb.n < nmax * nmax * MAXB) w.fb_src = nullptr, w.fb_plan = false;
   Fb.resize(nmax * nmax * MAXB);
+  const bool one_direct = direct && nF == 1 && mine.size() <= (size_t)MAXB && cached && keep_x &&
+                          std::all_of(w.xc_have.begin(), w.xc_have.end(), [](char c) { return c != 0; });
+  const bool fb_filled = f_from_finish && one_direct && helfem::tuning_live().fock_blocks && w.fb_src && w.fb_src == dFs[0] &&
+                         w.fb_stamp == ctx->finish_count && w.fb_nmax == nmax;
+  bool band_fx_used = false;
   T1.resize(nmax * nmax * MAXB);
   Xall.resize(nmax * nmax * MAXB);
   for (size_t c0 = 0; c0 < mine.size(); c0 += MAXB) {
@@ -1367,7 +1381,11 @@
         low_tiles += t1 * (t1 + 1) / 2;
       }
       const bool band_fx = !fx.empty() && force_split < 0 && !gemm_prefers_128(ctx, full_tiles) && !tuning().mfma_4x4x4;
-      for (int k = 0; k < nb; k++) {
+      band_fx_used = band_fx;
+      const bool skip_gather = fb_filled && w.fb_src_band == band_fx;
+      if (!skip_gather) w.fb_src = nullptr;
+      for (int k = 0; k < nb && !skip_gather; k++) {
+        ProfScope pg(ctx, "k_gather_f");
         const int ib = mine[c0 + k] % nblk;
         const double *dF = dFs[mine[c0 + k] / nblk];
         int n = ns[k];
@@ -1469,7 +1487,35 @@
     } else
     check_status(ctx, w, nb);
   }
+  w.fb_plan = direct && nF == 1 && mine.size() <= (size_t)MAXB && keep_x && w.sup_S == dS;
+  w.fb_band = band_fx_used;
+  w.fb_nmax = nmax;
   HFG_HIP_CHECK(hipGetLastError());
+}
+
+bool eig_operand_target(hfg_ctx *ctx, int N, EigOperandTarget *tg) {
+  EigWork &w = work_for(ctx);
+  if (!w.fb_plan || !ctx->fixed_sinvh || w.sup_S != ctx->fixed_sinvh || w.sup_gen != ctx->fixed_gen || w.sup_N != N || !w.Fb.p) return false;
+  const int nblk = (int)w.sup_ptr.size() - 1;
+  if (nblk < 1 || nblk > MAXB || w.Fb.n < w.fb_nmax * w.fb_nmax * nblk) return false;
+  const bool want_band = ctx->band_state == 1 && ctx->band_node.size() == (size_t)N && helfem::tuning_live().eig_band;
+  if (want_band == w.band_rows.empty() || (w.fb_band && !want_band)) return false;
+  tg->Fb = w.Fb.p;
+  tg->stride = w.fb_nmax * w.fb_nmax;
+  tg->rows = (const int64_t *)w.idx.p;
+  tg->band_pos = w.fb_band ? (const int64_t *)w.band_pos_dev.p : nullptr;
+  tg->nblk = nblk;
+  tg->nmax = (int)w.fb_nmax;
+  tg->blk_ptr = w.sup_ptr.data();
+  tg->blk_idx = w.sup_idx.data();
+  return true;
+}
+
+void eig_operand_filled(hfg_ctx *ctx, const double *dF) {
+  EigWork &w = work_for(ctx);
+  w.fb_src = dF;
+  w.fb_src_band = w.fb_band;
+  w.fb_stamp = ctx->finish_count;
 }
 
 static void eig_assemble_sel_dev(hfg_ctx *ctx, int N, int nblk, const int64_t *blk_ptr, const int64_t *blk_idx, const double *dBlockBuf,
@@ -1525,13 +1571,13 @@
 }
 
 static void eig_gsym_sub_multi_dev(hfg_ctx *ctx, int N, int nF, const double *const *dFs, const double *dS, int nblk, const int64_t *blk_ptr,
-                                   const int64_t *blk_idx, int nev, double *const *dEs, double *const *dCs) {
+                                   const int64_t *blk_idx, int nev, double *const *dEs, double *const *dCs, bool f_from_finish = false) {
   int save_rank = ctx->shard_rank, save_n = ctx->shard_n;
   ctx->shard_rank = 0;
   ctx->shard_n = 1;
   try {
     if (helfem::tuning_live().eig_direct && nF * nblk <= MAXB) {
-      eig_blocks_multi_dev(ctx, N, nF, dFs, dS, nblk, blk_ptr, blk_idx, nullptr, nev, dEs, dCs);
+      eig_blocks_multi_dev(ctx, N, nF, dFs, dS, nblk, blk_ptr, blk_idx, nullptr, nev, dEs, dCs, f_from_finish);
     } else {
       const size_t sz = eig_block_buf_size(nblk, blk_ptr);
       DevBuf<double> &buf = ctx->ws[6];
@@ -1539,7 +1585,7 @@
       double *bufs[MAXB];
       if (nF > MAXB) throw std::logic_error("eig_gsym_sub: too many matrices in one call\n");
       for (int f = 0; f < nF; f++) bufs[f] = buf.p + f * sz;
-      eig_blocks_multi_dev(ctx, N, nF, dFs, dS, nblk, blk_ptr, blk_idx, bufs, nev);
+      eig_blocks_multi_dev(ctx, N, nF, dFs, dS, nblk, blk_ptr, blk_idx, bufs, nev, nullptr, nullptr, false);
       for (int f = 0; f < nF; f++) eig_assemble_sel_dev(ctx, N, nblk, blk_ptr, blk_idx, bufs[f], dEs[f], dCs[f], nev);
     }
   } catch (...) {
@@ -1552,8 +1598,8 @@
 }
 
 void eig_gsym_sub_dev(hfg_ctx *ctx, int N, const double *dF, const double *dS, int nblk, const int64_t *blk_ptr,
-                      const int64_t *blk_idx, double *dE, double *dC) {
-  eig_gsym_sub_multi_dev(ctx, N, 1, &dF, dS, nblk, blk_ptr, blk_idx, 0, &dE, &dC);
+                      const int64_t *blk_idx, double *dE, double *dC, bool f_from_finish) {
+  eig_gsym_sub_multi_dev(ctx, N, 1, &dF, dS, nblk, blk_ptr, blk_idx, 0, &dE, &dC, f_from_finish);
 }
 
 void eig_gsym_sub_sel_dev(hfg_ctx *ctx, int N, const double *dF, const double *dS, int nblk, const int64_t *blk_ptr,
diff --git a/helfem_amd/csrc/hip/fock.hip b/helfem_amd/csrc/hip/fock.hip
--- a/helfem_amd/csrc/hip/fock.hip
+++ b/helfem_amd/csrc/hip/fock.hip
@@ -192,6 +192,61 @@
   }
   outa[o] = va;
   outb[o] = vb;
+}
+
+template <int NS>
+__global__ __launch_bounds__(256) void k_fock_finish_blocks(const double *__restrict__ Xc, const double *__restrict__ Jc, size_t nc,
+                                                            const double *__restrict__ H0, int N, int A, int E, int p,
+                                                            const int *__restrict__ pure_shell, const int *__restrict__ pure_n,
+                                                            const int64_t *__restrict__ rows, const int *__restrict__ qblk,
+                                                            const int *__restrict__ bptr, double *__restrict__ outa,
+                                                            double *__restrict__ outb, double *__restrict__ Fb, size_t fb_stride,
+                                                            const int64_t *__restrict__ fb_pos) {
+  extern __shared__ double fin_sh[];
+  const int q = blockIdx.x, ib = qblk[q], lo = bptr[ib], n = bptr[ib + 1] - lo;
+  const int col = (int)rows[q];
+  const int y = pure_shell[col], m = pure_n[col];
+  const int pm = p - 1, pp = p * p, f1 = m / pm;
+  double *Fcol = Fb ? Fb + (size_t)ib * fb_stride + (size_t)(q - lo) * n : nullptr;
+  for (int t = threadIdx.x; t < n; t += blockDim.x) {
+    const int row = (int)rows[lo + t];
+    const size_t o = (size_t)col * N + row;
+    const int x = pure_shell[row], nn = pure_n[row];
+    const int e1 = nn / pm;
+    double va = H0 ? H0[o] : 0.0, vb = va;
+    const size_t base = (size_t)(x * A + y) * E * pp;
+    for (int ce = 0; ce < 2; ce++) {
+      int e = e1 - ce;
+      if (e < 0 || e >= E) continue;
+      int i = nn - e * pm;
+      if (i < 0 || i > pm) continue;
+      for (int cf = 0; cf < 2; cf++) {
+        int f = f1 - cf;
+        if (f != e) continue;
+        int j = m - f * pm;
+        if (j < 0 || j > pm) continue;
+        const size_t c = base + (size_t)e * pp + j * p + i;
+        double ta = Xc[c];
+        if (Jc) ta += Jc[c];
+        va += ta;
+        if (NS == 2) {
+          double tb = Xc[nc + c];
+          if (Jc) tb += Jc[nc + c];
+          vb += tb;
+        }
+      }
+    }
+    outa[o] = va;
+    if (NS == 2) outb[o] = vb;
+    if (Fcol) {
+      if (fb_pos) fin_sh[t] = va;
+      else Fcol[t] = va;
+    }
+  }
+  if (Fcol && fb_pos) {
+    __syncthreads();
+    for (int t = threadIdx.x; t < n; t += blockDim.x) Fcol[t] = fin_sh[fb_pos[lo + t]];
+  }
 }
 
 __global__ void k_coulomb_ket(const double *__restrict__ Pc, int A, int E, int pp, const int *__restrict__ lm_off,
@@ -1515,6 +1570,12 @@
   DevBuf<int> pure_shell, pure_n, lmpos;
   DevBuf<double> Pc, Jc, Pc2, Jc2, Pc3, Paux, Y, Jaux, D0, D1, D2, D3, V, Fo, GA, GB, GC, GL, partial, scal;
   DevBuf<int> on, gon, chan;
+  const int *blk_src = nullptr;
+  std::vector<int> h_blockid, h_blk_q, h_blk_p, h_tgt_q, h_tgt_p;
+  std::vector<int64_t> h_blk_rows;
+  DevBuf<int64_t> blk_rows;
+  DevBuf<int> blk_q, blk_p, tgt_q, tgt_p;
+  DevBuf<double> Fsum;
 };
 
 struct FockSkip {
@@ -2049,8 +2110,45 @@
   return (size_t)basis->Nang() * basis->Nang() * basis->Nel() * basis->max_Nprim() * basis->max_Nprim();
 }
 
+static void finish_block_lists(hfg_ctx *ctx, const hfg_dev_tables *t, FockAux &a, const int *dBlockId, bool again) {
+  const int N = t->N;
+  if (!again && a.blk_src == dBlockId && (int)a.h_blockid.size() == N) return;
+  HFG_HIP_CHECK(hipDeviceSynchronize());
+  a.blk_src = nullptr;
+  a.h_blockid.resize(N);
+  HFG_HIP_CHECK(hipMemcpy(a.h_blockid.data(), dBlockId, sizeof(int) * N, hipMemcpyDeviceToHost));
+  std::vector<int> ids(a.h_blockid);
+  std::sort(ids.begin(), ids.end());
+  ids.erase(std::unique(ids.begin(), ids.end()), ids.end());
+  const int nb = (int)ids.size();
+  std::vector<int> of(N);
+  a.h_blk_p.assign(nb + 1, 0);
+  for (int i = 0; i < N; i++) {
+    of[i] = (int)(std::lower_bound(ids.begin(), ids.end(), a.h_blockid[i]) - ids.begin());
+    a.h_blk_p[of[i] + 1]++;
+  }
+  for (int b = 0; b < nb; b++) a.h_blk_p[b + 1] += a.h_blk_p[b];
+  a.h_blk_rows.resize(N);
+  a.h_blk_q.resize(N);
+  std::vector<int> fill(a.h_blk_p.begin(), a.h_blk_p.end() - 1);
+  for (int i = 0; i < N; i++) {
+    a.h_blk_q[fill[of[i]]] = of[i];
+    a.h_blk_rows[fill[of[i]]++] = i;
+  }
+  a.blk_rows.upload(a.h_blk_rows, ctx->stream);
+  a.blk_q.upload(a.h_blk_q, ctx->stream);
+  a.blk_p.upload(a.h_blk_p, ctx->stream);
+  HFG_HIP_CHECK(hipStreamSynchronize(ctx->stream));
+  a.blk_src = dBlockId;
+}
+
 void set_fock_blocks(hfg_ctx *ctx, hfg_basis *basis, const int *dBlockId) {
   ctx->fock_need_tables = nullptr;
+  if (basis->dev && basis->dev_device == ctx->device) {
+    FockAux &a = aux_for(ctx, basis);
+    a.blk_src = nullptr;
+    if (dBlockId) finish_block_lists(ctx, basis->dev, a, dBlockId, true);
+  }
   if (!dBlockId) return;
   if (!basis->dev || basis->dev_device != ctx->device) throw std::logic_error("hfg_ctx_set_fock_blocks: the basis tables are not on this context's device\n");
   const hfg_dev_tables *t = basis->dev;
@@ -2081,9 +2179,16 @@
   ctx->fock_need_tables = t;
 }
 
+static void add_compact(hfg_ctx *ctx, double *dA, const double *dB, size_t nc) {
+  ProfScope pk(ctx, "k_add_inplace");
+  hipLaunchKernelGGL(k_add_inplace, dim3(2048), dim3(256), 0, ctx->stream, dA, dB, nc);
+}
+
 void fock_compact_dev(hfg_ctx *ctx, hfg_basis *basis, int x_func, int c_func, const double *dP, double *dFc,
-                      double *dScal, double thr) {
+                      double *dScal, double thr, const double **dXc) {
   hfg_dev_tables *t = tables_of(ctx, basis);
+  if (dXc) *dXc = nullptr;
+  const bool split = dXc && helfem::tuning_live().fock_blocks;
   FockAux &a = aux_for(ctx, basis);
   const size_t nc = fock_compact_size(basis);
   a.Pc.resize(nc);
@@ -2106,7 +2211,8 @@
     ProfScope ps(ctx, "xc");
     xc_compact(ctx, basis, x_func, c_func, a.Pc.p, a.Jc.p, dScal, thr, sk);
     HFG_HIP_CHECK(hipStreamWaitEvent(main, ctx->side_ev[1], 0));
-    hipLaunchKernelGGL(k_add_inplace, dim3(2048), dim3(256), 0, ctx->stream, dFc, a.Jc.p, nc);
+    if (split) *dXc = a.Jc.p;
+    else add_compact(ctx, dFc, a.Jc.p, nc);
     HFG_HIP_CHECK(hipGetLastError());
     return;
   }
@@ -2119,7 +2225,8 @@
   if (x_func > 0 || c_func > 0) {
     ProfScope ps(ctx, "xc");
     xc_compact(ctx, basis, x_func, c_func, a.Pc.p, a.Jc.p, dScal, thr, sk);
-    hipLaunchKernelGGL(k_add_inplace, dim3(2048), dim3(256), 0, ctx->stream, dFc, a.Jc.p, nc);
+    if (split) *dXc = a.Jc.p;
+    else add_compact(ctx, dFc, a.Jc.p, nc);
   } else {
     HFG_HIP_CHECK(hipMemsetAsync(dScal, 0, 3 * sizeof(double), ctx->stream));
   }
@@ -2131,7 +2238,9 @@
                      double *dF) {
   hfg_dev_tables *t = tables_of(ctx, basis);
   FockAux &a = aux_for(ctx, basis);
+  ctx->finish_count++;
   ProfScope ps(ctx, "scatter");
+  ProfScope pk(ctx, "k_fock_finish");
   dim3 grid((t->N + 63) / 64, (t->N + 3) / 4);
   hipLaunchKernelGGL(k_fock_finish, grid, dim3(256), 0, ctx->stream, dFc, dH0, dBlockId, t->N, t->A, t->R, t->E, t->p,
                      a.pure_shell.p, a.pure_n.p, dF);
@@ -2205,11 +2314,76 @@
                          double *dFa, double *dFb) {
   hfg_dev_tables *t = tables_of(ctx, basis);
   FockAux &a = aux_for(ctx, basis);
+  ctx->finish_count++;
   ProfScope ps(ctx, "scatter");
+  ProfScope pk(ctx, "k_fock_finish");
   dim3 grid((t->N + 63) / 64, (t->N + 3) / 4);
   hipLaunchKernelGGL(k_fock_finish_pol, grid, dim3(256), 0, ctx->stream, dFc, fock_compact_size(basis), dH0, dBlockId, t->N, t->A,
                      t->R, t->E, t->p, a.pure_shell.p, a.pure_n.p, dFa, dFb);
   HFG_HIP_CHECK(hipGetLastError());
 }
 
-}
+void fock_finish_blocks_dev(hfg_ctx *ctx, hfg_basis *basis, const double *dFc, const double *dJc, const double *dH0,
+                            const int *dBlockId, double *dF, double *dFb) {
+  hfg_dev_tables *t = tables_of(ctx, basis);
+  FockAux &a = aux_for(ctx, basis);
+  const size_t nc = fock_compact_size(basis), ns = dFb ? 2 : 1;
+  const int N = t->N;
+  if (!dBlockId || !helfem::tuning_live().fock_blocks) {
+    const double *sum = dFc;
+    if (dJc) {
+      a.Fsum.resize(ns * nc);
+      HFG_HIP_CHECK(hipMemcpyAsync(a.Fsum.p, dFc, ns * nc * sizeof(double), hipMemcpyDeviceToDevice, ctx->stream));
+      add_compact(ctx, a.Fsum.p, dJc, ns * nc);
+      sum = a.Fsum.p;
+    }
+    if (dFb) fock_finish_pol_dev(ctx, basis, sum, dH0, dBlockId, dF, dFb);
+    else fock_finish_dev(ctx, basis, sum, dH0, dBlockId, dF);
+    return;
+  }
+  finish_block_lists(ctx, t, a, dBlockId, false);
+  ctx->finish_count++;
+  const int64_t *rows = a.blk_rows.p;
+  const int *qblk = a.blk_q.p, *bptr = a.blk_p.p;
+  EigOperandTarget tg;
+  bool hand = !dFb && eig_operand_target(ctx, N, &tg) && (size_t)tg.nmax * sizeof(double) <= 64 * 1024;
+  if (hand) {
+    for (int ib = 0; ib < tg.nblk && hand; ib++) {
+      const int64_t lo = tg.blk_ptr[ib], hi = tg.blk_ptr[ib + 1];
+      if (tg.blk_idx[lo] < 0 || tg.blk_idx[lo] >= N) hand = false;
+      const int id = hand ? a.h_blockid[tg.blk_idx[lo]] : 0;
+      int64_t same = 0;
+      for (int64_t i = lo; i < hi && hand; i++)
+        if (tg.blk_idx[i] < 0 || tg.blk_idx[i] >= N || a.h_blockid[tg.blk_idx[i]] != id) hand = false;
+      for (int i = 0; i < N && hand; i++) same += a.h_blockid[i] == id;
+      if (same != hi - lo) hand = false;
+    }
+  }
+  if (hand) {
+    std::vector<int> q(N), p(tg.nblk + 1);
+    for (int ib = 0; ib <= tg.nblk; ib++) p[ib] = (int)tg.blk_ptr[ib];
+    for (int ib = 0; ib < tg.nblk; ib++)
+      for (int i = p[ib]; i < p[ib + 1]; i++) q[i] = ib;
+    upload_cached(a.tgt_q, a.h_tgt_q, q, ctx->stream);
+    upload_cached(a.tgt_p, a.h_tgt_p, p, ctx->stream);
+    rows = tg.rows;
+    qblk = a.tgt_q.p;
+    bptr = a.tgt_p.p;
+  }
+  {
+    ProfScope ps(ctx, "scatter");
+    ProfScope pk(ctx, "k_fock_finish_blocks");
+    const size_t lds = hand && tg.band_pos ? (size_t)tg.nmax * sizeof(double) : 0;
+    if (dFb)
+      hipLaunchKernelGGL(k_fock_finish_blocks<2>, dim3(N), dim3(256), 0, ctx->stream, dFc, dJc, nc, dH0, N, t->A, t->E, t->p,
+                         a.pure_shell.p, a.pure_n.p, rows, qblk, bptr, dF, dFb, (double *)nullptr, (size_t)0, (const int64_t *)nullptr);
+    else
+      hipLaunchKernelGGL(k_fock_finish_blocks<1>, dim3(N), dim3(256), lds, ctx->stream, dFc, dJc, nc, dH0, N, t->A, t->E, t->p,
+                         a.pure_shell.p, a.pure_n.p, rows, qblk, bptr, dF, (double *)nullptr, hand ? tg.Fb : (double *)nullptr,
+                         hand ? tg.stride : (size_t)0, hand ? tg.band_pos : (const int64_t *)nullptr);
+    HFG_HIP_CHECK(hipGetLastError());
+  }
+  if (hand) eig_operand_filled(ctx, dF);
+}
+
+}
diff --git a/helfem_amd/csrc/hip/internal.h b/helfem_amd/csrc/hip/internal.h
--- a/helfem_amd/csrc/hip/internal.h
+++ b/helfem_amd/csrc/hip/internal.h
@@ -36,13 +36,15 @@
 void set_fock_blocks(hfg_ctx *ctx, hfg_basis *basis, const int *dBlockId);
 size_t fock_compact_size(hfg_basis *basis);
 void fock_compact_dev(hfg_ctx *ctx, hfg_basis *basis, int x_func, int c_func, const double *dP, double *dFc, double *dScal,
-                      double thr);
+                      double thr, const double **dXc = nullptr);
 void fock_finish_dev(hfg_ctx *ctx, hfg_basis *basis, const double *dFc, const double *dH0, const int *dBlockId,
                      double *dF);
 void fock_compact_pol_dev(hfg_ctx *ctx, hfg_basis *basis, int x_func, int c_func, const double *dPa, const double *dPb,
                           double *dFc, double *dScal, double thr);
 void fock_finish_pol_dev(hfg_ctx *ctx, hfg_basis *basis, const double *dFc, const double *dH0, const int *dBlockId,
                          double *dFa, double *dFb);
+void fock_finish_blocks_dev(hfg_ctx *ctx, hfg_basis *basis, const double *dFc, const double *dJc, const double *dH0,
+                            const int *dBlockId, double *dF, double *dFb = nullptr);
 
 enum class ExTables { coulomb, screened, mix };
 hfg_dev_tables *exchange_tables(hfg_basis *basis, ExTables which);
@@ -64,7 +66,16 @@
 void eig_sym_dev(hfg_ctx *ctx, int n, const double *dA, double *dE, double *dC);
 void eig_gsym_dev(hfg_ctx *ctx, int N, int n, const double *dF, const double *dS, double *dE, double *dC);
 void eig_gsym_sub_dev(hfg_ctx *ctx, int N, const double *dF, const double *dS, int nblk, const int64_t *blk_ptr,
-                      const int64_t *blk_idx, double *dE, double *dC);
+                      const int64_t *blk_idx, double *dE, double *dC, bool f_from_finish = false);
+struct EigOperandTarget {
+  double *Fb;
+  size_t stride;
+  const int64_t *rows, *band_pos;
+  int nblk, nmax;
+  const int64_t *blk_ptr, *blk_idx;
+};
+bool eig_operand_target(hfg_ctx *ctx, int N, EigOperandTarget *tg);
+void eig_operand_filled(hfg_ctx *ctx, const double *dF);
 void eig_gsym_sub_pair_dev(hfg_ctx *ctx, int N, const double *dFa, const double *dFb, const double *dS, int nblk,
                            const int64_t *blk_ptr, const int64_t *blk_idx, double *dEa, double *dCa, double *dEb,
                            double *dCb);
diff --git a/helfem_amd/csrc/host/tuning.h b/helfem_amd/csrc/host/tuning.h
--- a/helfem_amd/csrc/host/tuning.h
+++ b/helfem_amd/csrc/host/tuning.h
@@ -23,6 +23,7 @@
   X(exl_mix, int, -1, "HELFEM_EXL_MIX", true, "int", atoi(e), "range-separated hybrids in the step objects: 0 = K from two builds, hfg_exchange_occ_dev and hfg_rs_exchange_dev, added on the device (checker); other non-negative = one build on the mixed-kernel table set (hfg_mix_exchange_tables); negative: by kernel kind as measured, the mixed set for both Yukawa and erfc") \
   X(fock_overlap, bool, true, "HELFEM_FOCK_OVERLAP", false, "off if 0", atoi(e) != 0, "Coulomb kernels on the side stream beside the XC kernels; off: one after the other on the main stream") \
   X(fock_skip, bool, true, "HELFEM_FOCK_SKIP", true, "off if 0", atoi(e) != 0, "Fock build skips shell pairs whose density block is zero and, after hfg_ctx_set_fock_blocks, pairs the caller does not read; off: every pair is computed (checker)") \
+  X(fock_blocks, bool, true, "HELFEM_FOCK_BLOCKS", true, "off if 0", atoi(e) != 0, "Fock finish of the step objects writes the entries inside the symmetry blocks alone, can take J and XC as two compact buffers and hands the blocks to the one-call eigensolve (hfg_fock_finish_blocks_devptr); off: k_add_inplace, k_fock_finish over the whole square and the eigensolve's gather (checker)") \
   X(xc_lds_limit, size_t, 150 * 1024, "HELFEM_XC_LDS_LIMIT", false, "int", (size_t)atol(e), "bytes of LDS the angular XC kernels plan with; smaller forces the chunked kernels (tests)") \
   X(coulomb_batch_chunk, int, 0, "HELFEM_COULOMB_BATCH_CHUNK", true, "int", std::max(0, atoi(e)), "densities per pass over the tables of the batched Coulomb build forced smaller than the LDS rule allows (tests; 0: the rule's own)") \
   X(exchange_batch_chunk, int, 0, "HELFEM_EXCHANGE_BATCH_CHUNK", true, "int", std::max(0, atoi(e)), "densities per pass over the tables of the batched exchange build at most (tests; 0: as many as fit the 64 factor columns of a pass)") \
diff --git a/include/helfem_gpu.h b/include/helfem_gpu.h
--- a/include/helfem_gpu.h
+++ b/include/helfem_gpu.h
@@ -208,6 +208,14 @@
 int hfg_fock_need_pairs(int nshell, const int *nfunc, const int *blockid, int *need);
 int hfg_eig_gsym_sub_dev(hfg_ctx *ctx, int64_t N, const double *dF, const double *dSinvh, int nblk,
                          const int64_t *blk_ptr, const int64_t *blk_idx, double *dE, double *dC);
+int hfg_fock_compact_parts_devptr(hfg_ctx *ctx, hfg_basis *basis, int x_func, int c_func, const double *dP, double *dFc,
+                                  double *dScal, double dens_thr, const double **dXc);
+int hfg_fock_finish_blocks_devptr(hfg_ctx *ctx, hfg_basis *basis, const double *dFc, const double *dJc, const double *dH0,
+                                  const int *dBlockId, double *dF);
+int hfg_fock_finish_blocks_pol_devptr(hfg_ctx *ctx, hfg_basis *basis, const double *dFc, const double *dJc, const double *dH0,
+                                      const int *dBlockId, double *dFa, double *dFb);
+int hfg_eig_gsym_sub_handoff_devptr(hfg_ctx *ctx, int64_t N, const double *dF, const double *dSinvh, int nblk,
+                                    const int64_t *blk_ptr, const int64_t *blk_idx, double *dE, double *dC, int f_from_finish);
 int hfg_eig_gsym_sub_sel_dev(hfg_ctx *ctx, int64_t N, const double *dF, const double *dSinvh, int nblk, const int64_t *blk_ptr,
                              const int64_t *blk_idx, int64_t nev, double *dE , double *dC );
 int64_t hfg_eig_block_buf_size(int nblk, const int64_t *blk_ptr);
```

Result: no change. 7.659 ms (median of 6 runs) (-0.6%).
